# initc3/HoneyBadgerMPC

Measured on AMD Instinct MI355X. Metric: shares reconstructed/sec (batch open, n=64 t=21), higher is better.
Workload: dtype u256 (integer mod p): exact int8 x int8 -> int32 byte-split GEMM on the matrix cores; the high half of every sum folded mod p on the matrix cores too, one-word Barrett quotient

## Files before the change

honeybadgermpc_amd/csrc/gen_mm8.py:

```python
#!/usr/bin/env python3
import os

NC = 47
MAXKB = 4
XB = 180
ABUF = [[196, 200], [204, 208]]
F_SETS = [212, 234]
F_KMIN = -2
CLOBBER_LO, CLOBBER_HI = 180, 255
HALF_RHOS = [(0, 1), (2, 3)]


def f(s, k, e):
    assert -2 <= k <= 8 and e in (0, 1)
    return F_SETS[s] + 2 * (k - F_KMIN) + e


def windows(rho):
    return [q for q in range(-2, 8) if -7 <= 4 * q + rho <= 31]


def cols_of(rho):
    return sorted({4 * q + rho + 7 + 8 * g for q in windows(rho) for g in (0, 1)})


def half_columns(half):
    return sorted(c for rho in HALF_RHOS[half] for c in cols_of(rho))


NCP = 39


def packed_columns(half):
    return sorted(4 * q + rho + 7 for rho in HALF_RHOS[half] for q in windows(rho))


def lds_loads(kb, xs_op, as_op, packed=False):
    a0, a1 = ABUF[kb & 1]
    out = []
    for e in (0, 1):
        for h in (0, 1):
            out.append(f"ds_read_b128 v[{XB + 8 * e + 4 * h}:{XB + 8 * e + 4 * h + 3}], {xs_op} offset:{((kb * 2 + e) * 2 + h) * 1024}")
    out.append(f"ds_read_b128 v[{a0}:{a0 + 3}], {as_op} offset:{(kb * 2) * 1024}")
    if not packed:
        out.append(f"ds_read_b128 v[{a1}:{a1 + 3}], {as_op} offset:{(kb * 2 + 1) * 1024}")
    return out


def interleave(mfmas, ops):
    out = []
    if not mfmas:
        return list(ops)
    n = len(mfmas)
    per = (len(ops) + max(n - 1, 1) - 1) // max(n - 1, 1)
    pi = 0
    for i, m in enumerate(mfmas):
        if i == n - 1:
            out += ops[pi:]
            pi = len(ops)
        out.append(m)
        if i < n - 1:
            out += ops[pi:pi + per]
            pi += per
    return out


def asm_half(half, nkb, skip=False, packed=False):
    assert not skip or nkb >= 2
    assert not (skip and packed)
    cols = packed_columns(half) if packed else half_columns(half)
    pos = {c: i for i, c in enumerate(cols)}
    ncol = len(cols)
    xs_op, as_op, bias = f"%{ncol}", f"%{ncol + 1}", f"%{ncol + 2}"
    L = []
    for s in range(2):
        for k in (-2, 8):
            for e in (0, 1):
                L.append(f"v_mov_b32 v{f(s, k, e)}, 0")
    L += lds_loads(0, xs_op, as_op, packed)[:(5 if skip else 6)]
    groups = [(kb, rho) for kb in range(nkb) for rho in HALF_RHOS[half]]

    def prep(gi):
        kb, rho = groups[gi]
        s = gi & 1
        ops = []
        if rho == HALF_RHOS[half][0]:
            ops.append("s_waitcnt lgkmcnt(0)")
            for e in (0, 1):
                for k in range(8):
                    ops.append(f"v_xor_b32 v{f(s, k, e)}, 0x80808080, v{XB + 8 * e + k}")
                ops.append(f"v_mov_b32 v{f(s, -1, e)}, 0")
            if rho != 0:
                for e in (0, 1):
                    for k in range(-1, 8):
                        ops.append(f"v_alignbyte_b32 v{f(s, k, e)}, v{f(s, k + 1, e)}, v{f(s, k, e)}, {rho}")
        else:
            for e in (0, 1):
                for k in range(-1, 8):
                    ops.append(f"v_alignbyte_b32 v{f(s, k, e)}, v{f(1 - s, k + 1, e)}, v{f(1 - s, k, e)}, 1")
        return ops

    started = set()

    def mfmas(gi):
        kb, rho = groups[gi]
        s = gi & 1
        out = []
        for q in windows(rho):
            r = f(s, q, 0)
            assert r % 2 == 0
            for grp in ((0,) if packed else (0, 1)):
                if skip and kb == 0 and grp == 1:
                    continue
                c = 4 * q + rho + 7 + 8 * grp
                ab = ABUF[kb & 1][grp]
                cin = f"%{pos[c]}"
                if c not in started:
                    assert kb == 0 or (skip and kb == 1)
                    cin = bias
                    started.add(c)
                out.append(f"v_mfma_i32_16x16x64_i8 %{pos[c]}, v[{ab}:{ab + 3}], v[{r}:{r + 3}], {cin}")
        return out

    L += prep(0) + ["s_nop 1"]
    for gi in range(len(groups)):
        nxt = gi + 1 < len(groups)
        kb, rho = groups[gi]
        if rho == HALF_RHOS[half][0] and kb + 1 < nkb:
            L += lds_loads(kb + 1, xs_op, as_op, packed)
        L += interleave(mfmas(gi), prep(gi + 1) if nxt else [])
        if nxt:
            L.append("s_nop 0")
    assert started == set(cols)
    L += ["s_nop 7", "s_nop 7"]
    return L, ncol


def emit():
    out = ["// GENERATED by gen_mm8.py -- do not edit", ""]
    out.append("// column held by accumulator i of each half (half 0: rho in {0,1}; half 1: rho in {2,3})")
    for half in range(2):
        cols = half_columns(half)
        out.append(f"// half {half}: {cols}")
    assert half_columns(0) == [c for c in range(NC) if c % 4 in (0, 3)] and half_columns(1) == [c for c in range(NC) if c % 4 in (1, 2)]
    out.append("template <int NKB, int HALF, bool SKIP = false> struct Mm8Phase;")
    clob = ", ".join(f'"v{r}"' for r in range(CLOBBER_LO, CLOBBER_HI + 1))
    for nkb, skip in [(k, False) for k in range(1, MAXKB + 1)] + [(k, True) for k in range(2, MAXKB + 1)]:
        for half in range(2):
            lines, ncol = asm_half(half, nkb, skip)
            out.append(f"template <> struct Mm8Phase<{nkb}, {half}, {'true' if skip else 'false'}> {{")
            out.append("    static __device__ __forceinline__ void run(v4i (&acc)[24], uint32_t xs_addr, uint32_t as_addr, v4i biasv) {")
            out.append("        asm volatile(")
            for ln in lines:
                out.append(f'            "{ln}\\n\\t"')
            outs = ", ".join(f'"=&v"(acc[{i}])' for i in range(ncol))
            out.append(f"            : {outs}")
            out.append('            : "v"(xs_addr), "v"(as_addr), "v"(biasv)')
            out.append(f'            : {clob}, "memory");')
            out.append("    }")
            out.append("};")
    assert packed_columns(0) == [c for c in range(NCP) if c % 4 in (0, 3)] and packed_columns(1) == [c for c in range(NCP) if c % 4 in (1, 2)]
    out.append("// packed phases: accumulator i of a half is the virtual column (one per window) of the same two lists cut at 38")
    out.append("template <int NKB, int HALF> struct Mm8PhasePacked;")
    for nkb in range(1, MAXKB + 1):
        for half in range(2):
            lines, ncol = asm_half(half, nkb, packed=True)
            assert sum("v_mfma" in ln for ln in lines) == len(windows(HALF_RHOS[half][0]) + windows(HALF_RHOS[half][1])) * nkb
            out.append(f"template <> struct Mm8PhasePacked<{nkb}, {half}> {{")
            out.append("    static __device__ __forceinline__ void run(v4i (&acc)[20], uint32_t xs_addr, uint32_t as_addr, v4i biasv) {")
            out.append("        asm volatile(")
            for ln in lines:
                out.append(f'            "{ln}\\n\\t"')
            outs = ", ".join(f'"=&v"(acc[{i}])' for i in range(ncol))
            out.append(f"            : {outs}")
            out.append('            : "v"(xs_addr), "v"(as_addr), "v"(biasv)')
            out.append(f'            : {clob}, "memory");')
            out.append("    }")
            out.append("};")
    return "\n".join(out) + "\n"


if __name__ == "__main__":
    here = os.path.dirname(os.path.abspath(__file__))
    text = emit()
    path = os.path.join(here, "hb_mm8_body.inc")
    old = open(path).read() if os.path.exists(path) else None
    if old != text:
        open(path, "w").write(text)
    print(path)
```

honeybadgermpc_amd/csrc/hb_common.hpp:

```cpp
#pragma once
#include <hip/hip_runtime.h>
#include <stdint.h>
#include <stdio.h>
#include <string.h>

#include <functional>
#include <map>
#include <mutex>
#include <string>
#include <vector>

#include "../../include/hbmpc_hip.h"
#include "fp29.hpp"

namespace hb {
struct FastMatrix;
struct Mm8Matrix;
struct Mm8wMatrix;
}
namespace hb {

struct Wide { static constexpr int NL = 9, NW = 8; };
struct Narrow { static constexpr int NL = 3, NW = 2; };

constexpr int OT = 4;

template <int NL, int NW>
__device__ __forceinline__ void eval_at_point_128(uint32_t (&r)[NL], const uint32_t *__restrict__ x_packed, const uint32_t *__restrict__ poly, int d,
                                                  const FpParams<NL> &P, uint32_t (*red)[NL]) {
    const int tid = threadIdx.x;
    uint32_t xd[NL], xm[NL], acc[NL];
    load_digits<NL, NW>(xd, x_packed);
    to_mont(xm, xd, P);
#pragma unroll
    for (int q = 0; q < NL; q++) acc[q] = 0;
    for (int l = tid; l < d; l += 128) {
        uint32_t pw[NL], cd[NL], m[NL];
        fp_pow_u32(pw, xm, (uint32_t)l, P);
        load_digits<NL, NW>(cd, poly + (size_t)l * NW);
        mont_mul(m, cd, pw, P);
        fp_add(acc, acc, m, P);
    }
#pragma unroll
    for (int q = 0; q < NL; q++) red[tid][q] = acc[q];
    __syncthreads();
    for (int w = 64; w >= 1; w >>= 1) {
        if (tid < w) {
            uint32_t a[NL], b[NL], t[NL];
#pragma unroll
            for (int q = 0; q < NL; q++) { a[q] = red[tid][q]; b[q] = red[tid + w][q]; }
            fp_add(t, a, b, P);
#pragma unroll
            for (int q = 0; q < NL; q++) red[tid][q] = t[q];
        }
        __syncthreads();
    }
#pragma unroll
    for (int q = 0; q < NL; q++) r[q] = red[0][q];
}

__host__ __device__ inline size_t m_index(int i, int l, int n_in, int nl, int q) {
    return (((size_t)((i / OT) * n_in + l) * (size_t)nl + (size_t)q) * OT) + (size_t)(i % OT);
}
inline int m_tiles(int n_out) { return (n_out + OT - 1) / OT; }

}

struct hb_matrix {
    hb_ctx *ctx;
    int n_out, n_in;
    uint32_t *dev;
    size_t words;
    bool cached;
    int refs;
    hb::Mm8wMatrix *wide;
    bool wide_tried;
};

namespace hb {
struct TlsError {
    static std::string &slot() { static thread_local std::string s; return s; }
    TlsError &operator=(const std::string &m) { slot() = m; return *this; }
    TlsError &operator=(const char *m) { slot() = m ? m : ""; return *this; }
    const char *c_str() const { return slot().c_str(); }
    void clear() { slot().clear(); }
    bool empty() const { return slot().empty(); }
};
struct PrescaleParams {
    uint32_t pbar[9];
    uint32_t pneg[8];
    uint32_t m0, m1;
};
}
namespace hb {
enum EnvHook {
    ENV_CACHE_CAP,
    ENV_GAO_PAIR,
    ENV_MM8W_FLAT,
    ENV_MM8W_RQ,
    ENV_MM8W_TILE16,
    ENV_MM8_NO_SKIP,
    ENV_NO_EVAL_FEW,
    ENV_NO_FUSED_MSCALE,
    ENV_NO_FUSED_PACK,
    ENV_NO_FUSED_SMALL,
    ENV_NO_FUSED_VALIDATE,
    ENV_NO_MFMA,
    ENV_NO_MFMA_DECODE,
    ENV_NO_MFMA_WIDE,
    ENV_NO_NARROW_FAST,
    ENV_NO_QUICK,
    ENV_NO_QUICK_PLAN,
    ENV_NTT_STAGE_LOOP,
    ENV_PROBE_WGS,
    ENV_QUICK_NO_CAND,
    ENV_UPLOAD_MODE,
    ENV_WB_NO_GAO,
    ENV_WB_NO_UNIFORM,
    ENV_COUNT
};
const char *env_hook(EnvHook h);
void env_reload();
}
struct hb_ctx {
    int device;
    int n_limbs;
    hb::FpParams<9> pw;
    hb::FpParams<3> pn;
    uint64_t p_limbs[4];
    std::recursive_mutex mu;
    int api_depth = 0;
    hb::TlsError err;
    std::map<std::string, hb_matrix *> mcache;
    std::map<std::vector<int32_t>, int32_t *> icache;
    std::map<std::string, void *> dcache;
    std::map<std::string, hb::FastMatrix *> fcache;
    std::map<std::string, hb::Mm8Matrix *> m8cache;
    struct CacheSlot { uint64_t tick; bool pinned; std::function<void()> drop; };
    std::map<std::string, CacheSlot> lru;
    uint64_t lru_clock = 0;
    size_t cache_cap = 192;
    int32_t *flag_dev;
    hb::PrescaleParams psc;
    int psc_state = 0;
    std::map<std::string, void *> ptcache;
    struct QuickSlot { void *buf = nullptr; size_t cap = 0; void *ev = nullptr; };
    std::vector<QuickSlot> qslots;
    unsigned qnext = 0;
    std::vector<void *> probe_pool, probe_host_pool;
    void *side_stream = nullptr;
    std::map<std::string, std::pair<void *, size_t>> scratch;
    void *fetch_host = nullptr, *fetch_dev = nullptr;
    int fetch_seq = 0;
    void *cand_host = nullptr, *cand_dev = nullptr;
    int32_t *cand_ticket = nullptr;
    int cand_seq = 0;
    void *after_event = nullptr;
    std::map<int, void *> wide_shared;
    std::map<std::string, std::vector<int>> wide_shapes;
    void *mm8_shared = nullptr;
    int elem_words() const { return n_limbs == 4 ? 8 : 2; }
    int nl() const { return n_limbs == 4 ? 9 : 3; }
};

struct hb_api_guard {
    hb_ctx *c;
    explicit hb_api_guard(hb_ctx *ctx) : c(ctx) { if (c) { c->mu.lock(); c->api_depth++; } }
    ~hb_api_guard() { if (c) { c->api_depth--; c->mu.unlock(); } }
    hb_api_guard(const hb_api_guard &) = delete;
    hb_api_guard &operator=(const hb_api_guard &) = delete;
};
#define HB_API_GUARD(ctxexpr) hb_api_guard hb_api_guard__(ctxexpr)

inline int ctx_scratch(hb_ctx *ctx, const char *slot, size_t bytes, void **out) {
    auto &e = ctx->scratch[slot];
    if (e.second < bytes || !e.first) {
        if (e.first) { (void)hipFree(e.first); e.first = nullptr; e.second = 0; }
        const size_t want = bytes ? bytes : 4;
        const hipError_t err = hipMalloc(&e.first, want);
        if (err != hipSuccess) { e.first = nullptr; ctx->err = std::string("scratch ") + slot + ": " + hipGetErrorString(err); return HB_ERR_HIP; }
        e.second = want;
    }
    *out = e.first;
    return HB_OK;
}
inline void ctx_scratch_free(hb_ctx *ctx) {
    for (auto &kv : ctx->scratch) if (kv.second.first) (void)hipFree(kv.second.first);
    ctx->scratch.clear();
}

#define HB_HIP(ctx, call)                                                                         \
    do {                                                                                          \
        hipError_t e__ = (call);                                                                  \
        if (e__ != hipSuccess) {                                                                  \
            (ctx)->err = std::string(#call) + ": " + hipGetErrorString(e__);                      \
            return HB_ERR_HIP;                                                                    \
        }                                                                                         \
    } while (0)

#define HB_LAUNCH_CHECK(ctx)                                                                      \
    do {                                                                                          \
        hipError_t e__ = hipGetLastError();                                                       \
        if (e__ != hipSuccess) {                                                                  \
            (ctx)->err = std::string("kernel launch: ") + hipGetErrorString(e__);                 \
            return HB_ERR_HIP;                                                                    \
        }                                                                                         \
    } while (0)

namespace hb {

inline int fail(hb_ctx *ctx, int code, const char *msg) {
    if (ctx) ctx->err = msg;
    return code;
}
inline int nsub_for(int d, int nl, int nw) {
    int shift = 29 * nl - 32 * nw;
    long per = 1L << shift;
    long n = (d + per - 1) / per;
    return n < 1 ? 1 : (int)n;
}
void fp_params_from_limbs(FpParams<9> &P, const uint64_t *p_limbs);
void fp_params_from_limbs(FpParams<3> &P, const uint64_t *p_limbs);
int get_int_array(hb_ctx *ctx, const int32_t *host, int n, int32_t **dev, hipStream_t s);
int own_int_array(hb_ctx *ctx, const int32_t *host, int n, int32_t **dev, hipStream_t s);
void cache_note(hb_ctx *ctx, const std::string &rk, std::function<void()> drop, bool pinned = false);
void cache_touch(hb_ctx *ctx, const std::string &rk);
void cache_trim(hb_ctx *ctx);
void matrix_unref(hb_matrix *m);
int alloc_matrix(hb_ctx *ctx, int n_out, int n_in, hb_matrix **out);
int upload_elems(hb_ctx *ctx, const uint64_t *host, size_t count, uint32_t **dev, hipStream_t s);
int upload_table(hb_ctx *ctx, void *dst_dev, const void *src_host, size_t bytes, hipStream_t s);
std::string table_key(const char *kind, hb_ctx *ctx, const uint64_t *x, int n, int d);
int pow_points_dev(hb_ctx *ctx, const uint64_t *base_host, const int32_t *exps_dev, int count, uint32_t **out_dev, hipStream_t s);
int vand_matrix_from_dev(hb_ctx *ctx, const std::string &key, const uint32_t *x_dev, int n, int d, hb_matrix **out, hipStream_t s);
int vinv_from_dev(hb_ctx *ctx, const std::string &key, const uint32_t *x_dev, int k, hb_matrix **out, hipStream_t s);
int gao_decode(hb_ctx *ctx, const uint64_t *x_host, int npts, int k, const uint64_t *ys_dev, int64_t C,
               uint64_t *coeffs_dev, uint64_t *errloc_dev, int32_t *errloc_len_dev, uint8_t *ok_dev, void *stream, int ys_stride = 0, const int32_t *sel_host = nullptr);
int launch_matvec(hb_ctx *ctx, const hb_matrix *m, const uint32_t *in, hb_view iv, const int32_t *in_rows_dev, int64_t in_count,
                  uint32_t *out, hb_view ov, int64_t out_count, const int32_t *check_mask_dev, int32_t *mismatch_dev,
                  int64_t C, hipStream_t s);
int launch_copy_view(hb_ctx *ctx, const uint32_t *src, hb_view sv, uint32_t *dst, hb_view dv, int64_t C, int L, int64_t dst_count, hipStream_t s);

int get_twiddles(hb_ctx *ctx, const uint64_t *omega_host, int n, uint32_t **tw, hipStream_t s);
int launch_ntt_lds(hb_ctx *ctx, const uint32_t *tw, int n, const uint32_t *in, hb_view iv, int64_t in_count, int d, int k,
                   uint32_t *out, hb_view ov, int64_t out_count, const int32_t *check_mask_dev, int32_t *mismatch_dev,
                   int64_t C, hipStream_t s, uint32_t *copy_dst = nullptr, hb_view cpv = hb_view{0, 0}, int64_t copy_count = 0, int copy_rows = 0);

struct FastMatrix {
    int n_out, n_in;
    int ot;
    uint32_t *M;
    int32_t *nd;
    int32_t *negrow;
    uint32_t *K;
    uint32_t *K2;
    uint32_t *K1;
    uint32_t *KT;
};
__host__ __device__ inline size_t mf_index(int i, int l, int n_in, int nl, int q, int ot) {
    return (((size_t)((i / ot) * n_in + l) * (size_t)nl + (size_t)q) * ot) + (size_t)(i % ot);
}
void fast_matrix_free(FastMatrix *m);
int fast_vand_create(hb_ctx *ctx, const uint32_t *x_dev, int n, int d, FastMatrix **out, hipStream_t s);
int fast_vinv_create(hb_ctx *ctx, const uint32_t *x_dev, int k, FastMatrix **out, hipStream_t s);
int launch_prescale(hb_ctx *ctx, const FastMatrix *m, const uint32_t *in, hb_view iv, const int32_t *rows_dev, int64_t in_count,
                    uint32_t *out_dg, int64_t C, hipStream_t s);
int launch_prescale_pk(hb_ctx *ctx, const FastMatrix *m, const uint32_t *in, hb_view iv, const int32_t *rows_dev, int64_t in_count,
                       uint32_t *out_pk, int64_t C, hipStream_t s);
int launch_matvec2(hb_ctx *ctx, const FastMatrix *m, const uint32_t *in_dg,
                   const uint32_t *in_pk, hb_view iv, const int32_t *in_rows_dev, int64_t in_count, uint32_t *scratch_dg,
                   uint32_t *out_pk, hb_view ov, int64_t out_count,
                   int pk_rows, int pk_from_mont, uint32_t *out_dg, const int32_t *check_mask_dev, int32_t *mismatch_dev,
                   int64_t C, hipStream_t s, int check_skip = 0, const uint32_t *K_override = nullptr);

int launch_decode_check(hb_ctx *ctx, const FastMatrix *dec, const FastMatrix *enc, const uint32_t *cols, hb_view cv,
                        const int32_t *z_dev, uint32_t *pk_dst, hb_view pv, int64_t pk_count, int pk_rows, uint32_t *coef_dg,
                        const int32_t *mask_dev, int32_t *mismatch_dev, int64_t C, hipStream_t s, int check_skip);

bool prescale_params(hb_ctx *ctx);
int mm8_from_fast(hb_ctx *ctx, const FastMatrix *f, Mm8Matrix **out, hipStream_t s, const int32_t *rows = nullptr, int n_rows = 0);
void mm8_free(Mm8Matrix *m);
int launch_mm8(hb_ctx *ctx, const Mm8Matrix *m, const uint32_t *in, hb_view iv, const int32_t *in_rows_dev, int64_t in_count,
               uint32_t *out, hb_view ov, int64_t out_count, const int32_t *check_mask_dev, int32_t *mismatch_dev,
               int64_t C, hipStream_t s, uint32_t *copy_dst = nullptr, hb_view cpv = hb_view{0, 0}, int64_t copy_count = 0,
               int copy_rows = 0, const int32_t *check_rows_dev = nullptr);

int mm8w_from_host(hb_ctx *ctx, const uint64_t *m_host, int n_out, int n_in, Mm8wMatrix **out, hipStream_t s);
void mm8w_free(Mm8wMatrix *m);
int mm8w_route(hb_ctx *ctx, const Mm8wMatrix *m, int64_t C, int32_t *out);
int launch_mm8w(hb_ctx *ctx, const Mm8wMatrix *m, const uint32_t *in, hb_view iv, const int32_t *in_rows_dev, int64_t in_count,
                uint32_t *out, hb_view ov, int64_t out_count, const int32_t *check_mask_dev, int32_t *mismatch_dev,
                int64_t C, hipStream_t s, const uint32_t *cmp = nullptr, hb_view cv = hb_view{0, 0}, int n_store = 0);
bool fold_tables(hb_ctx *ctx, int n_bytes, uint8_t *fold, uint32_t *top8, uint32_t *mu, uint32_t *shift8);
struct FsVerdict { unsigned long long word; unsigned long long pad; };
struct FsDone { int32_t *counter; FsVerdict *host; int32_t seq; };
constexpr int32_t FS_VERDICT_NONE = 0x3fffffff;
#ifdef __HIPCC__
__device__ __forceinline__ void fs_publish_verdict(int32_t *mismatch, int32_t *first_bad, int32_t *counter, FsVerdict *host, int32_t seq) {
    const int32_t fl = mismatch ? __hip_atomic_load(mismatch, __ATOMIC_RELAXED, __HIP_MEMORY_SCOPE_AGENT) : 0;
    const int32_t fb = first_bad ? __hip_atomic_load(first_bad, __ATOMIC_RELAXED, __HIP_MEMORY_SCOPE_AGENT) : INT32_MAX;
    const uint32_t low = ((fl & 1) ? 0x80000000u : 0u) | ((fl & 0x40000000) ? 0x40000000u : 0u) | (uint32_t)((fb < 0 || fb > FS_VERDICT_NONE) ? FS_VERDICT_NONE : fb);
    __hip_atomic_store(&host->word, ((unsigned long long)(uint32_t)seq << 32) | low, __ATOMIC_RELAXED, __HIP_MEMORY_SCOPE_SYSTEM);
    if (mismatch) __hip_atomic_store(mismatch, 0, __ATOMIC_RELAXED, __HIP_MEMORY_SCOPE_AGENT);
    if (first_bad) __hip_atomic_store(first_bad, INT32_MAX, __ATOMIC_RELAXED, __HIP_MEMORY_SCOPE_AGENT);
    if (counter) __hip_atomic_store(counter, 0, __ATOMIC_RELAXED, __HIP_MEMORY_SCOPE_AGENT);
}
__device__ __forceinline__ void fs_workgroup_done(const FsDone &done, int32_t *mismatch, int32_t *first_bad) {
    if (!done.counter) return;
    asm volatile("s_waitcnt vmcnt(0)" ::: "memory");
    __syncthreads();
    if (threadIdx.x == 0 && atomicAdd(done.counter, 1) == (int)gridDim.x - 1) fs_publish_verdict(mismatch, first_bad, done.counter, done.host, done.seq);
}
#endif
inline bool fs_verdict_is(const FsVerdict *host, int32_t seq) { return (int32_t)(*reinterpret_cast<const volatile unsigned long long *>(&host->word) >> 32) == seq; }
inline void fs_verdict_read(const FsVerdict *host, int32_t *flag, int32_t *first) {
    const uint32_t low = (uint32_t)*reinterpret_cast<const volatile unsigned long long *>(&host->word);
    *flag = ((low >> 31) ? 1 : 0) | ((low & 0x40000000u) ? 0x40000000 : 0);
    const int32_t f = (int32_t)(low & 0x3fffffffu);
    *first = f == FS_VERDICT_NONE ? INT32_MAX : f;
}
struct Mm8wShared { uint32_t bias; uint32_t c80r[9], biasmod[9]; void *wp; uint32_t *zero; };
int mm8w_geometry(int n_out, int d, int *tile_rows, int *n_rt, int *nkb, size_t *a8_bytes, size_t *crow_words);
int mm8w_shared(hb_ctx *ctx, int d, const Mm8wShared **out, hipStream_t s);
void mm8w_shared_free(hb_ctx *ctx);
int launch_mm8w_raw(hb_ctx *ctx, int n_out, int d, int tile_rows, const void *a8, const uint32_t *crow, const Mm8wShared *sh,
                    const uint32_t *in, hb_view iv, const int32_t *in_rows_dev, int64_t in_count, uint32_t *out, hb_view ov, int64_t out_count,
                    const int32_t *check_mask_dev, int32_t *mismatch_dev, int64_t C, hipStream_t s, const uint32_t *cmp, hb_view cv, int n_store,
                    int32_t *first_bad_dev, uint32_t *bad_map_dev = nullptr, const FsDone *done = nullptr);
void point_tables_free(hb_ctx *ctx);
void mm8_shared_free(hb_ctx *ctx);
struct PointTable {
    int n, S;
    uint32_t *xm, *inv, *pw;
    bool usable;
    int refs;
    bool small;
    std::vector<uint16_t> xs;
    uint16_t *xs_dev;
};
int point_table(hb_ctx *ctx, const uint64_t *x_host, int n, PointTable **out, hipStream_t s);
struct QuickLayout {
    int n, d, nc, n_coef, n_out, tile_rows, nkb;
    size_t o_a8, o_crow, o_wj, o_full, o_nraw, o_mcan, o_z, o_map, o_sync, need;
    size_t o_cand, o_cand_crow;
};
int quick_layout(hb_ctx *ctx, int n, int d, int nc, int n_coef, QuickLayout *L);
int quick_build(hb_ctx *ctx, const uint64_t *x_host, const int32_t *z, const int32_t *zc, const QuickLayout &L, uint8_t *base, const Mm8wShared **shared, hipStream_t s,
                int flags = 3 );
int quick_layout_cand(hb_ctx *ctx, QuickLayout *L);
int quick_launch(hb_ctx *ctx, const QuickLayout &L, const uint8_t *base, const Mm8wShared *sh, const uint32_t *cols, hb_view cv, uint32_t *out, hb_view ov,
                 int64_t out_count, int n_store, int32_t *mismatch_dev, int32_t *first_bad_dev, int64_t C, hipStream_t s, uint32_t *bad_map_dev = nullptr,
                 const FsDone *done = nullptr);
struct FsLayout {
    int n, d, nc, n_coef, n_out, n_rt, nkb;
    size_t o_a8, o_crow, o_kt, o_mode, o_z, o_cand, o_cand_crow, need;
    int pk_nm, pk_ns;
    uint8_t pk_single[8];
    size_t o_ms;
    int mscale;
};
constexpr int FS_BUILD_Z = 1, FS_BUILD_ZC = 2;
int fs_layout(hb_ctx *ctx, const PointTable *pt, int d, int nc, int n_coef, FsLayout *L);
int fs_build(hb_ctx *ctx, const PointTable *pt, const int32_t *z, const int32_t *zc, const FsLayout &L, uint8_t *base, int flags, int32_t *status_dev, hipStream_t s);
bool fs_pack(const PointTable *pt, const int32_t *z, FsLayout *L);
bool fs_mscale(FsLayout *L);
int fs_launch(hb_ctx *ctx, const FsLayout &L, const uint8_t *base, const uint32_t *cols, hb_view cv, uint32_t *out, hb_view ov, int64_t out_count,
              int32_t *mismatch_dev, int32_t *first_bad_dev, uint32_t *bad_map_dev, int64_t C, hipStream_t s, const FsDone *done = nullptr,
              const int32_t *pick_zc = nullptr);
int fs_build_cand(hb_ctx *ctx, PointTable *pt, const int32_t *z, const FsLayout &L, uint8_t *base, int32_t *status_dev, hipStream_t s, bool with_z = false);
struct Mv64Matrix;
int points_on_device(hb_ctx *ctx, const uint64_t *x_host, int n, uint32_t **out, hipStream_t s);
bool mv64_applies(const hb_ctx *ctx, int d);
bool mv64_matrix_cores(const hb_ctx *ctx, int d);
int mv64_from_host(hb_ctx *ctx, const uint64_t *m_host, int n_out, int d, const int32_t *mode_host, Mv64Matrix **out, hipStream_t s);
void mv64_free(Mv64Matrix *m);
int launch_mv64(hb_ctx *ctx, const Mv64Matrix *m, const uint64_t *in, hb_view iv, const int32_t *in_rows_dev, int64_t in_count, uint64_t *out, hb_view ov,
                int64_t out_count, int32_t *mismatch_dev, int32_t *first_bad_dev, int64_t C, hipStream_t s);
int mv64_plan_tables(hb_ctx *ctx, const uint64_t *x, int n, int d, const int32_t *z, const int32_t *zc, int nc, std::vector<uint64_t> &V, std::vector<uint64_t> &Vinv,
                     std::vector<uint64_t> &P);
int quick_dec_supported(hb_quick_dec *qd, int d, int nc, int n_coef);
const Mm8wMatrix *matrix_wide(hb_ctx *ctx, const hb_matrix *m, hipStream_t s);

#define HB_DISPATCH(ctx, EXPR_W, EXPR_N)                                                          \
    do {                                                                                          \
        if ((ctx)->n_limbs == 4) { EXPR_W; } else { EXPR_N; }                                     \
    } while (0)

}
```

honeybadgermpc_amd/csrc/hb_core.hip:

```cpp
#include <algorithm>

#include <mutex>
#include <string>

#include "hb_common.hpp"

using namespace hb;

namespace {

struct U320 { uint64_t l[5]; };
inline bool ge(const U320 &a, const U320 &b) {
    for (int i = 4; i >= 0; i--) if (a.l[i] != b.l[i]) return a.l[i] > b.l[i];
    return true;
}
inline void sub(U320 &a, const U320 &b) {
    unsigned __int128 br = 0;
    for (int i = 0; i < 5; i++) {
        unsigned __int128 d = (unsigned __int128)a.l[i] - b.l[i] - (uint64_t)br;
        a.l[i] = (uint64_t)d; br = (d >> 64) & 1;
    }
}
inline void dbl_mod(U320 &a, const U320 &p) {
    for (int i = 4; i > 0; i--) a.l[i] = (a.l[i] << 1) | (a.l[i - 1] >> 63);
// ... 122 lines not shown
    uint32_t d[NL], m[NL];
    load_digits<NL, NW>(d, src + (size_t)idx * NW);
    to_mont(m, d, P);
#pragma unroll
    for (int q = 0; q < NL; q++) M[m_index(i, l, n_in, NL, q)] = m[q];
}
template <int NL, int NW>
__global__ void k_matrix_export(const FpParams<NL> P, const uint32_t *__restrict__ M, int n_out, int n_in, uint32_t *__restrict__ dst) {
    int idx = blockIdx.x * blockDim.x + threadIdx.x;
    if (idx >= n_out * n_in) return;
    int i = idx / n_in, l = idx % n_in;
    uint32_t m[NL], d[NL];
#pragma unroll
    for (int q = 0; q < NL; q++) m[q] = M[m_index(i, l, n_in, NL, q)];
    from_mont(d, m, P);
    store_digits<NL, NW>(dst + (size_t)idx * NW, d);
}

template <int NL, int NW, bool CHECK>
__global__ void __launch_bounds__(256) k_matvec(const FpParams<NL> P, const uint32_t *__restrict__ M, int n_out, int n_in, int nsub,
                                                const uint32_t *__restrict__ in, int64_t in_sc, int64_t in_sl,
                                                const int32_t *__restrict__ in_rows, int64_t in_count,
                                                uint32_t *__restrict__ out, int64_t out_sc, int64_t out_sl, int64_t out_count,
                                                const int32_t *__restrict__ check_mask, int32_t *__restrict__ mismatch,
                                                int64_t C, int tiles, int64_t n_waves) {
    static_assert(OT == 4, "matrix tile is loaded as uint4 per digit");
    const int lane = threadIdx.x & 63;
    const int wib = __builtin_amdgcn_readfirstlane(threadIdx.x >> 6);
    const int64_t nb8 = gridDim.x >> 3;
    const int64_t vb = (int64_t)(blockIdx.x & 7) * nb8 + (blockIdx.x >> 3);
    const int64_t wave = vb * 4 + wib;
    if (wave >= n_waves) return;
    const int tile = (int)(wave % tiles);
    const int64_t g = wave / tiles;
    const int64_t c = g * 64 + lane;
    const bool active = c < C;
    const int64_t cc = active ? c : (C - 1);
    const int nv = min(OT, n_out - tile * OT);
    const uint4 *mt = reinterpret_cast<const uint4 *>(M) + (size_t)tile * n_in * NL;
    constexpr int GROUP = Lazy<NL>::GROUP;

    uint64_t col[OT][2 * NL];
#pragma unroll
    for (int o = 0; o < OT; o++) col_zero(col[o]);

#define HB_ROW_OF(l_) (in_rows ? in_rows[((l_) < n_in) ? (l_) : (n_in - 1)] : (((l_) < n_in) ? (l_) : (n_in - 1)))
#define HB_LOAD_M(dst_, l_)                                                              \
    _Pragma("unroll") for (int q = 0; q < NL; q++) dst_[q] = mt[(size_t)(l_) * NL + q];
#define HB_LOAD_X(w_, valid_, row_)                                                      \
    {                                                                                    \
        const int64_t idx_ = cc * in_sc + (int64_t)(row_) * in_sl;                       \
        valid_ = idx_ < in_count;                                                        \
        load_words<NW>(w_, in + (valid_ ? idx_ : 0) * NW);                               \
    }
#define HB_UNPACK_X(d_, w_, valid_)                                                      \
    {                                                                                    \
        unpack<NL, NW>(d_, w_);                                                          \
        _Pragma("unroll") for (int q = 0; q < NL; q++) d_[q] = valid_ ? d_[q] : 0u;      \
    }
    uint4 mc[NL], mn[NL];
    uint32_t wn[NW], xd[NL];
    bool vn;
    HB_LOAD_M(mc, 0)
    HB_LOAD_X(wn, vn, HB_ROW_OF(0))
    HB_UNPACK_X(xd, wn, vn)
    int row_n = HB_ROW_OF(1);
    int gcnt = 0;
    for (int l = 0; l < n_in; l++) {
        const int ln = (l + 1 < n_in) ? l + 1 : l;
        HB_LOAD_M(mn, ln)
        const int row_nn = HB_ROW_OF(l + 2);
        HB_LOAD_X(wn, vn, row_n)
        __builtin_amdgcn_sched_barrier(0);
        uint32_t xu[NL];
#pragma unroll
        for (int q = 0; q < NL; q++) { xu[q] = xd[q]; asm volatile("" : "+v"(xu[q])); }
#pragma unroll
        for (int o = 0; o < OT; o++) {
            if (o < nv) {
                uint32_t md[NL];
#pragma unroll
                for (int q = 0; q < NL; q++) md[q] = (o == 0) ? mc[q].x : (o == 1) ? mc[q].y : (o == 2) ? mc[q].z : mc[q].w;
                mac<NL>(col[o], md, xu);
            }
        }
        if (++gcnt == GROUP) {
            gcnt = 0;
#pragma unroll
            for (int o = 0; o < OT; o++) carry(col[o]);
        }
        __builtin_amdgcn_sched_barrier(0);
        HB_UNPACK_X(xd, wn, vn)
        row_n = row_nn;
#pragma unroll
        for (int q = 0; q < NL; q++) mc[q] = mn[q];
    }
#undef HB_ROW_OF
#undef HB_LOAD_M
#undef HB_LOAD_X
#undef HB_UNPACK_X
#pragma unroll
    for (int o = 0; o < OT; o++) {
        if (o < nv) {
            const int i = tile * OT + o;
            uint32_t r[NL];
            carry(col[o]);
            redc(r, col[o], P);
            for (int s = 0; s < nsub; s++) cond_sub_p(r, P);
            uint32_t w[NW];
            pack<NL, NW>(w, r);
            const int64_t oidx = cc * out_sc + (int64_t)i * out_sl;
            if constexpr (CHECK) {
                if (check_mask[i] && active) {
                    uint32_t e[NW];
                    load_words<NW>(e, out + oidx * NW);
                    uint32_t diff = 0;
#pragma unroll
                    for (int q = 0; q < NW; q++) diff |= e[q] ^ w[q];
                    if (diff) atomicOr(mismatch, 1);
                }
            } else {
                if (active && oidx < out_count) store_words<NW>(out + oidx * NW, w);
            }
        }
    }
}

template <int NW>
__global__ void k_copy_view(const uint32_t *__restrict__ src, int64_t s_sc, int64_t s_sl, uint32_t *__restrict__ dst, int64_t d_sc, int64_t d_sl,
                            int64_t C, int L, int64_t dst_count) {
    int64_t idx = (int64_t)blockIdx.x * blockDim.x + threadIdx.x;
    if (idx >= C * L) return;
    int64_t c = idx / L; int l = (int)(idx % L);
    int64_t di = c * d_sc + (int64_t)l * d_sl;
    if (di >= dst_count) return;
    uint32_t w[NW];
    load_words<NW>(w, src + (c * s_sc + (int64_t)l * s_sl) * NW);
    store_words<NW>(dst + di * NW, w);
}

template <int NL, int NW>
__global__ void k_reduce(const FpParams<NL> P, const uint32_t *__restrict__ src, uint32_t *__restrict__ dst, int64_t count,
                         int32_t *__restrict__ changed) {
    const int64_t i = (int64_t)blockIdx.x * blockDim.x + threadIdx.x;
    if (i >= count) return;
    uint32_t w[NW], d[NL], m[NL], o[NW];
    load_words<NW>(w, src + i * NW);
    unpack<NL, NW>(d, w);
    to_mont<NL>(m, d, P);
    from_mont<NL>(d, m, P);
    pack<NL, NW>(o, d);
    bool diff = false;
#pragma unroll
    for (int q = 0; q < NW; q++) diff |= o[q] != w[q];
    if (diff) {
        store_words<NW>(dst + i * NW, o);
        if (changed) atomicAdd(changed, 1);
    } else if (dst != src) {
        store_words<NW>(dst + i * NW, w);
    }
}

namespace hb {

void cache_note(hb_ctx *ctx, const std::string &rk, std::function<void()> drop, bool pinned) {
    ctx->lru[rk] = hb_ctx::CacheSlot{++ctx->lru_clock, pinned, std::move(drop)};
}
void cache_touch(hb_ctx *ctx, const std::string &rk) {
    auto it = ctx->lru.find(rk);
    if (it != ctx->lru.end()) it->second.tick = ++ctx->lru_clock;
}
static void cache_drop_down_to(hb_ctx *ctx, size_t keep) {
    std::vector<std::pair<uint64_t, std::string>> order;
    for (auto &kv : ctx->lru) if (!kv.second.pinned) order.emplace_back(kv.second.tick, kv.first);
    if (order.size() <= keep) return;
    std::sort(order.begin(), order.end());
    (void)hipDeviceSynchronize();
    for (size_t i = 0; i + keep < order.size(); i++) {
        auto it = ctx->lru.find(order[i].second);
        if (it == ctx->lru.end()) continue;
        auto drop = std::move(it->second.drop);
        ctx->lru.erase(it);
        drop();
    }
}
void cache_trim(hb_ctx *ctx) {
    if (ctx->api_depth > 1) return;
    size_t unpinned = 0;
    for (auto &kv : ctx->lru) if (!kv.second.pinned) unpinned++;
    if (unpinned > ctx->cache_cap) cache_drop_down_to(ctx, ctx->cache_cap / 2);
}
void matrix_unref(hb_matrix *m) {
    if (!m) return;
    if (--m->refs > 0) return;
    (void)hipFree(m->dev);
    mm8w_free(m->wide);
    delete m;
}

static std::string int_key(const int32_t *host, int n) {
    return std::string("i|") + std::string(reinterpret_cast<const char *>(host), (size_t)(n > 0 ? n : 0) * 4);
}
int own_int_array(hb_ctx *ctx, const int32_t *host, int n, int32_t **dev, hipStream_t s) {
    int32_t *d = nullptr;
    HB_HIP(ctx, hipMalloc(&d, sizeof(int32_t) * (size_t)(n > 0 ? n : 1)));
    const int rc = upload_table(ctx, d, host, sizeof(int32_t) * (size_t)(n > 0 ? n : 0), s);
    if (rc) { (void)hipFree(d); return rc; }
    *dev = d;
    return HB_OK;
}
int get_int_array(hb_ctx *ctx, const int32_t *host, int n, int32_t **dev, hipStream_t s) {
    std::vector<int32_t> key(host, host + n);
    const std::string rk = int_key(host, n);
    auto it = ctx->icache.find(key);
    if (it != ctx->icache.end()) { cache_touch(ctx, rk); *dev = it->second; return HB_OK; }
    int32_t *d = nullptr;
    int rc = own_int_array(ctx, host, n, &d, s); if (rc) return rc;
    ctx->icache[key] = d;
    cache_note(ctx, rk, [ctx, key]() { auto f = ctx->icache.find(key); if (f != ctx->icache.end()) { (void)hipFree(f->second); ctx->icache.erase(f); } });
    *dev = d;
    return HB_OK;
}

int alloc_matrix(hb_ctx *ctx, int n_out, int n_in, hb_matrix **out) {
    hb_matrix *m = new hb_matrix();
    m->ctx = ctx; m->n_out = n_out; m->n_in = n_in; m->cached = false; m->refs = 1; m->wide = nullptr; m->wide_tried = false;
    m->words = (size_t)m_tiles(n_out) * (size_t)n_in * OT * (size_t)ctx->nl();
    if (m->words == 0) m->words = 1;
    hipError_t e = hipMalloc(&m->dev, m->words * sizeof(uint32_t));
    if (e != hipSuccess) { delete m; ctx->err = std::string("hipMalloc: ") + hipGetErrorString(e); return HB_ERR_HIP; }
    *out = m;
    return HB_OK;
}

__global__ void k_upload_copy(const uint4 *__restrict__ src, uint4 *__restrict__ dst, size_t n16) {
    const size_t i = (size_t)blockIdx.x * blockDim.x + threadIdx.x;
    if (i < n16) dst[i] = src[i];
}
int upload_table(hb_ctx *ctx, void *dst_dev, const void *src_host, size_t bytes, hipStream_t s) {
    if (bytes == 0) return HB_OK;
    static const int legacy = [] { const char *e = env_hook(ENV_UPLOAD_MODE); return e && !strcmp(e, "memcpy") ? 1 : 0; }();
    if (legacy) {
        hipError_t e = hipMemcpyAsync(dst_dev, src_host, bytes, hipMemcpyHostToDevice, s);
        if (e == hipSuccess) e = hipStreamSynchronize(s);
        if (e != hipSuccess) { ctx->err = std::string("table upload: ") + hipGetErrorString(e); return HB_ERR_HIP; }
        return HB_OK;
    }
    const size_t n16 = (bytes + 15) / 16;
    void *stage = nullptr;
    HB_HIP(ctx, hipMalloc(&stage, n16 * 16));
    hipError_t e = hipMemcpy(stage, src_host, bytes, hipMemcpyHostToDevice);
    if (e == hipSuccess) {
        if (bytes % 16 == 0) k_upload_copy<<<(unsigned)((n16 + 255) / 256), 256, 0, s>>>((const uint4 *)stage, (uint4 *)dst_dev, n16);
        else e = hipMemcpyAsync(dst_dev, stage, bytes, hipMemcpyDeviceToDevice, s);
    }
    if (e == hipSuccess) e = hipGetLastError();
    if (e == hipSuccess) e = hipStreamSynchronize(s);
    (void)hipFree(stage);
    if (e != hipSuccess) { ctx->err = std::string("table upload: ") + hipGetErrorString(e); return HB_ERR_HIP; }
    return HB_OK;
}

int upload_elems(hb_ctx *ctx, const uint64_t *host, size_t count, uint32_t **dev, hipStream_t s) {
    size_t bytes = count * (size_t)ctx->elem_words() * 4;
    HB_HIP(ctx, hipMalloc(dev, bytes ? bytes : 4));
    const int rc = upload_table(ctx, *dev, host, bytes, s);
    if (rc) { (void)hipFree(*dev); *dev = nullptr; }
    return rc;
}

int points_on_device(hb_ctx *ctx, const uint64_t *x_host, int n, uint32_t **out, hipStream_t s) {
    std::string key = table_key("xs", ctx, x_host, n, 0);
    auto it = ctx->dcache.find(key);
    if (it != ctx->dcache.end()) { *out = (uint32_t *)it->second; cache_touch(ctx, "d|" + key); return HB_OK; }
    uint32_t *xd = nullptr;
    const int rc = upload_elems(ctx, x_host, (size_t)n, &xd, s); if (rc) return rc;
    ctx->dcache[key] = xd;
    cache_note(ctx, "d|" + key, [ctx, key]() { auto f = ctx->dcache.find(key); if (f != ctx->dcache.end()) { (void)hipFree(f->second); ctx->dcache.erase(f); } });
    *out = xd;
    return HB_OK;
}

std::string table_key(const char *kind, hb_ctx *ctx, const uint64_t *x, int n, int d) {
    std::string k(kind);
    k += ":" + std::to_string(n) + ":" + std::to_string(d) + ":";
    k.append(reinterpret_cast<const char *>(x), (size_t)n * ctx->n_limbs * 8);
    return k;
}

}

template <int NL, int NW>
__global__ void __launch_bounds__(128) k_eval_few(const FpParams<NL> P, const uint32_t *__restrict__ x, int n, const uint32_t *__restrict__ polys, int d,
                                                  uint32_t *__restrict__ out) {
    __shared__ uint32_t red[128][NL];
    const int c = blockIdx.x / n, i = blockIdx.x - c * n;
    uint32_t r[NL];
    eval_at_point_128<NL, NW>(r, x + (size_t)i * NW, polys + (size_t)c * d * NW, d, P, red);
    if (threadIdx.x == 0) store_digits<NL, NW>(out + ((size_t)c * n + i) * NW, r);
}


namespace hb {
static const char *const ENV_NAMES[ENV_COUNT] = {"HB_CACHE_CAP", "HB_GAO_PAIR", "HB_MM8W_FLAT", "HB_MM8W_RQ", "HB_MM8W_TILE16", "HB_MM8_NO_SKIP", "HB_NO_EVAL_FEW", "HB_NO_FUSED_MSCALE", "HB_NO_FUSED_PACK", "HB_NO_FUSED_SMALL", "HB_NO_FUSED_VALIDATE", "HB_NO_MFMA", "HB_NO_MFMA_DECODE", "HB_NO_MFMA_WIDE", "HB_NO_NARROW_FAST", "HB_NO_QUICK", "HB_NO_QUICK_PLAN", "HB_NTT_STAGE_LOOP", "HB_PROBE_WGS", "HB_QUICK_NO_CAND", "HB_UPLOAD_MODE", "HB_WB_NO_GAO", "HB_WB_NO_UNIFORM"};
static std::string g_env_val[ENV_COUNT];
static bool g_env_set[ENV_COUNT];
static std::once_flag g_env_once;
static std::mutex g_env_mu;
static void env_read() {
    for (int i = 0; i < ENV_COUNT; i++) {
        const char *e = ::getenv(ENV_NAMES[i]);
        g_env_set[i] = e != nullptr;
        g_env_val[i] = e ? e : "";
    }
}
const char *env_hook(EnvHook h) {
    std::call_once(g_env_once, env_read);
    return g_env_set[h] ? g_env_val[h].c_str() : nullptr;
}
void env_reload() {
    std::call_once(g_env_once, env_read);
    std::lock_guard<std::mutex> lk(g_env_mu);
    env_read();
}
}
extern "C" void hb_debug_reload_env() { hb::env_reload(); }

extern "C" {

int hb_version(void) { return 100; }

int hb_device_count(void) {
    int n = 0;
    if (hipGetDeviceCount(&n) != hipSuccess) return 0;
    return n;
}

int hb_ctx_create(hb_ctx **out, const uint64_t *p_limbs, int n_limbs, int device) {
    if (!out || !p_limbs) return HB_ERR_BAD_ARG;
    *out = nullptr;
    if (n_limbs != 1 && n_limbs != 4) return HB_ERR_BAD_ARG;
    if ((p_limbs[0] & 1) == 0) return HB_ERR_UNSUPPORTED;
    bool small = true; for (int i = 1; i < n_limbs; i++) if (p_limbs[i]) small = false;
    if (small && p_limbs[0] < 3) return HB_ERR_UNSUPPORTED;
    int ndev = 0;
    if (hipGetDeviceCount(&ndev) != hipSuccess || ndev == 0) return HB_ERR_NO_DEVICE;
    if (device < 0 || device >= ndev) return HB_ERR_NO_DEVICE;
    if (hipSetDevice(device) != hipSuccess) return HB_ERR_NO_DEVICE;
    hb_ctx *ctx = new hb_ctx();
    ctx->device = device; ctx->n_limbs = n_limbs;
    memset(ctx->p_limbs, 0, sizeof ctx->p_limbs);
    memcpy(ctx->p_limbs, p_limbs, (size_t)n_limbs * 8);
    if (n_limbs == 4) make_params<9>(ctx->pw, p_limbs, 4); else make_params<3>(ctx->pn, p_limbs, 1);
    if (const char *e = env_hook(ENV_CACHE_CAP)) { long v = atol(e); if (v >= 1) ctx->cache_cap = (size_t)v; }
    ctx->flag_dev = nullptr;
    if (hipMalloc(&ctx->flag_dev, 64 * sizeof(int32_t)) != hipSuccess) { delete ctx; return HB_ERR_HIP; }
    (void)hipMemset(ctx->flag_dev, 0, 64 * sizeof(int32_t));
    *out = ctx;
    return HB_OK;
}

void hb_ctx_destroy(hb_ctx *ctx) {
    if (!ctx) return;
    (void)hipSetDevice(ctx->device);
    ctx->lru.clear();
    for (auto &kv : ctx->mcache) matrix_unref(kv.second);
    for (auto &kv : ctx->icache) (void)hipFree(kv.second);
    for (auto &kv : ctx->dcache) (void)hipFree(kv.second);
    for (auto &kv : ctx->fcache) fast_matrix_free(kv.second);
    for (auto &kv : ctx->m8cache) mm8_free(kv.second);
    if (ctx->flag_dev) (void)hipFree(ctx->flag_dev);
    if (ctx->side_stream) (void)hipStreamDestroy((hipStream_t)ctx->side_stream);
    point_tables_free(ctx);
    mm8w_shared_free(ctx);
    mm8_shared_free(ctx);
    ctx_scratch_free(ctx);
    delete ctx;
}

const char *hb_last_error(const hb_ctx *ctx) { return ctx ? ctx->err.c_str() : "no context"; }
int hb_elem_bytes(const hb_ctx *ctx) { return ctx ? ctx->n_limbs * 8 : 0; }

int hb_malloc(hb_ctx *ctx, void **dptr, size_t bytes) { HB_API_GUARD(ctx); HB_HIP(ctx, hipMalloc(dptr, bytes ? bytes : 4)); return HB_OK; }
int hb_free(hb_ctx *ctx, void *dptr) { HB_API_GUARD(ctx); HB_HIP(ctx, hipFree(dptr)); return HB_OK; }
int hb_memcpy_h2d(hb_ctx *ctx, void *dst, const void *src, size_t bytes, void *stream) { HB_API_GUARD(ctx);
    HB_HIP(ctx, hipMemcpyAsync(dst, src, bytes, hipMemcpyHostToDevice, (hipStream_t)stream)); return HB_OK;
}
int hb_memcpy_d2h(hb_ctx *ctx, void *dst, const void *src, size_t bytes, void *stream) { HB_API_GUARD(ctx);
    HB_HIP(ctx, hipMemcpyAsync(dst, src, bytes, hipMemcpyDeviceToHost, (hipStream_t)stream));
    HB_HIP(ctx, hipStreamSynchronize((hipStream_t)stream)); return HB_OK;
}
int hb_stream_sync(hb_ctx *ctx, void *stream) { HB_API_GUARD(ctx); HB_HIP(ctx, hipStreamSynchronize((hipStream_t)stream)); return HB_OK; }

}

namespace hb {

template <int NL, int NW>
__global__ void k_pow_points(const FpParams<NL> P, const uint32_t *__restrict__ base, const int32_t *__restrict__ exps, int count,
                             uint32_t *__restrict__ out) {
    int i = blockIdx.x * blockDim.x + threadIdx.x;
    if (i >= count) return;
    uint32_t bd[NL], bm[NL], r[NL], c[NL];
    load_digits<NL, NW>(bd, base);
    to_mont(bm, bd, P);
    fp_pow_u32(r, bm, (uint32_t)(exps ? exps[i] : i), P);
    from_mont(c, r, P);
    store_digits<NL, NW>(out + (size_t)i * NW, c);
}

int pow_points_dev(hb_ctx *ctx, const uint64_t *base_host, const int32_t *exps_dev, int count, uint32_t **out_dev, hipStream_t s) {
    uint32_t *bd = nullptr;
    int rc = upload_elems(ctx, base_host, 1, &bd, s); if (rc) return rc;
    HB_HIP(ctx, hipMalloc(out_dev, (size_t)(count > 0 ? count : 1) * ctx->elem_words() * 4));
    if (count > 0) {
        HB_DISPATCH(ctx,
            (k_pow_points<9, 8><<<(count + 63) / 64, 64, 0, s>>>(ctx->pw, bd, exps_dev, count, *out_dev)),
            (k_pow_points<3, 2><<<(count + 63) / 64, 64, 0, s>>>(ctx->pn, bd, exps_dev, count, *out_dev)));
        HB_LAUNCH_CHECK(ctx);
    }
    HB_HIP(ctx, hipStreamSynchronize(s));
    HB_HIP(ctx, hipFree(bd));
    return HB_OK;
}

int vand_matrix_from_dev(hb_ctx *ctx, const std::string &key, const uint32_t *x_dev, int n, int d, hb_matrix **out, hipStream_t s) {
    hb_matrix *m = nullptr;
    int rc = alloc_matrix(ctx, n, d, &m); if (rc) return rc;
    HB_HIP(ctx, hipMemsetAsync(m->dev, 0, m->words * 4, s));
    if (n > 0 && d > 0) {
        HB_DISPATCH(ctx,
            (k_vand_table<9, 8><<<(n + 63) / 64, 64, 0, s>>>(ctx->pw, x_dev, n, d, m->dev)),
            (k_vand_table<3, 2><<<(n + 63) / 64, 64, 0, s>>>(ctx->pn, x_dev, n, d, m->dev)));
        HB_LAUNCH_CHECK(ctx);
        HB_HIP(ctx, hipStreamSynchronize(s));
    }
    m->cached = true; ctx->mcache[key] = m; *out = m;
    cache_note(ctx, "m|" + key, [ctx, key]() { auto f = ctx->mcache.find(key); if (f != ctx->mcache.end()) { hb_matrix *mm = f->second; ctx->mcache.erase(f); matrix_unref(mm); } });
    return HB_OK;
}

int vinv_from_dev(hb_ctx *ctx, const std::string &key, const uint32_t *x_dev, int k, hb_matrix **out, hipStream_t s) {
    if (k > 1023) return fail(ctx, HB_ERR_UNSUPPORTED, "vandermonde inverse: k > 1023");
    hb_matrix *m = nullptr;
    int rc = alloc_matrix(ctx, k, k, &m); if (rc) return rc;
    HB_HIP(ctx, hipMemsetAsync(m->dev, 0, m->words * 4, s));
    int singular = 0;
    if (k > 0) {
        HB_HIP(ctx, hipMemsetAsync(ctx->flag_dev, 0, sizeof(int32_t), s));
        int threads = ((k + 1 + 63) / 64) * 64;
        size_t lds = (size_t)(k + 2 * (k + 1)) * ctx->nl() * 4;
        if (ctx->n_limbs == 4) {
            HB_HIP(ctx, hipFuncSetAttribute(reinterpret_cast<const void *>(k_vinv_table<9, 8>), hipFuncAttributeMaxDynamicSharedMemorySize, (int)lds));
            k_vinv_table<9, 8><<<1, threads, lds, s>>>(ctx->pw, x_dev, k, m->dev, ctx->flag_dev);
        } else {
            HB_HIP(ctx, hipFuncSetAttribute(reinterpret_cast<const void *>(k_vinv_table<3, 2>), hipFuncAttributeMaxDynamicSharedMemorySize, (int)lds));
            k_vinv_table<3, 2><<<1, threads, lds, s>>>(ctx->pn, x_dev, k, m->dev, ctx->flag_dev);
        }
        HB_LAUNCH_CHECK(ctx);
        HB_HIP(ctx, hipMemcpyAsync(&singular, ctx->flag_dev, sizeof(int), hipMemcpyDeviceToHost, s));
        HB_HIP(ctx, hipStreamSynchronize(s));
    }
    if (singular) { m->refs = 1; matrix_unref(m); return fail(ctx, HB_ERR_SINGULAR, "Interpolation failed"); }
    m->cached = true; ctx->mcache[key] = m; *out = m;
    cache_note(ctx, "m|" + key, [ctx, key]() { auto f = ctx->mcache.find(key); if (f != ctx->mcache.end()) { hb_matrix *mm = f->second; ctx->mcache.erase(f); matrix_unref(mm); } });
    return HB_OK;
}

}

extern "C" {

int hb_vand_matrix_create(hb_ctx *ctx, const uint64_t *x_host, int n, int d, hb_matrix **out, void *stream) { HB_API_GUARD(ctx);
    if (!ctx || !out || n < 0 || d < 0) return HB_ERR_BAD_ARG;
    hipStream_t s = (hipStream_t)stream;
    cache_trim(ctx);
    std::string key = table_key("V", ctx, x_host, n, d);
    auto it = ctx->mcache.find(key);
    if (it != ctx->mcache.end()) { cache_touch(ctx, "m|" + key); it->second->refs++; *out = it->second; return HB_OK; }
    uint32_t *xd = nullptr;
    int rc = upload_elems(ctx, x_host, (size_t)n, &xd, s); if (rc) return rc;
    rc = vand_matrix_from_dev(ctx, key, xd, n, d, out, s);
    (void)hipStreamSynchronize(s);
    (void)hipFree(xd);
    if (!rc) (*out)->refs++;
    return rc;
}

int hb_vand_inverse_create(hb_ctx *ctx, const uint64_t *x_host, int k, hb_matrix **out, void *stream) { HB_API_GUARD(ctx);
    if (!ctx || !out || k < 0) return HB_ERR_BAD_ARG;
    hipStream_t s = (hipStream_t)stream;
    cache_trim(ctx);
    std::string key = table_key("Vinv", ctx, x_host, k, k);
    auto it = ctx->mcache.find(key);
    if (it != ctx->mcache.end()) { cache_touch(ctx, "m|" + key); it->second->refs++; *out = it->second; return HB_OK; }
    uint32_t *xd = nullptr;
    int rc = upload_elems(ctx, x_host, (size_t)k, &xd, s); if (rc) return rc;
    rc = vinv_from_dev(ctx, key, xd, k, out, s);
    (void)hipStreamSynchronize(s);
    (void)hipFree(xd);
    if (!rc) (*out)->refs++;
    return rc;
}

int hb_matrix_from_host(hb_ctx *ctx, const uint64_t *m_host, int n_out, int n_in, hb_matrix **out, void *stream) { HB_API_GUARD(ctx);
    if (!ctx || !out || n_out < 0 || n_in < 0) return HB_ERR_BAD_ARG;
    hipStream_t s = (hipStream_t)stream;
    hb_matrix *m = nullptr;
    int rc = alloc_matrix(ctx, n_out, n_in, &m); if (rc) return rc;
    HB_HIP(ctx, hipMemsetAsync(m->dev, 0, m->words * 4, s));
    if (n_out * n_in > 0) {
        uint32_t *src = nullptr;
        rc = upload_elems(ctx, m_host, (size_t)n_out * n_in, &src, s); if (rc) return rc;
        int tot = n_out * n_in;
        HB_DISPATCH(ctx,
            (k_matrix_import<9, 8><<<(tot + 127) / 128, 128, 0, s>>>(ctx->pw, src, n_out, n_in, m->dev)),
            (k_matrix_import<3, 2><<<(tot + 127) / 128, 128, 0, s>>>(ctx->pn, src, n_out, n_in, m->dev)));
        HB_LAUNCH_CHECK(ctx);
        HB_HIP(ctx, hipStreamSynchronize(s));
        HB_HIP(ctx, hipFree(src));
    }
    *out = m;
    return HB_OK;
}

int hb_matrix_to_host(hb_ctx *ctx, const hb_matrix *m, uint64_t *m_host, void *stream) { HB_API_GUARD(ctx);
    if (!ctx || !m || !m_host) return HB_ERR_BAD_ARG;
    hipStream_t s = (hipStream_t)stream;
    int tot = m->n_out * m->n_in;
    if (tot == 0) return HB_OK;
    uint32_t *dst = nullptr;
    size_t bytes = (size_t)tot * ctx->elem_words() * 4;
    HB_HIP(ctx, hipMalloc(&dst, bytes));
    HB_DISPATCH(ctx,
        (k_matrix_export<9, 8><<<(tot + 127) / 128, 128, 0, s>>>(ctx->pw, m->dev, m->n_out, m->n_in, dst)),
        (k_matrix_export<3, 2><<<(tot + 127) / 128, 128, 0, s>>>(ctx->pn, m->dev, m->n_out, m->n_in, dst)));
    HB_LAUNCH_CHECK(ctx);
    HB_HIP(ctx, hipMemcpyAsync(m_host, dst, bytes, hipMemcpyDeviceToHost, s));
    HB_HIP(ctx, hipStreamSynchronize(s));
    HB_HIP(ctx, hipFree(dst));
    return HB_OK;
}

void hb_matrix_destroy(hb_matrix *m) { HB_API_GUARD((m ? m->ctx : nullptr)); matrix_unref(m); }

}

namespace hb {

static const Mm8wMatrix *matvec_wide(hb_ctx *ctx, const hb_matrix *m, int64_t C, hipStream_t s) {
    return C >= 256 && m->n_in >= 4 && m->n_out >= 4 ? matrix_wide(ctx, m, s) : nullptr;
}

int launch_matvec(hb_ctx *ctx, const hb_matrix *m, const uint32_t *in, hb_view iv, const int32_t *in_rows_dev, int64_t in_count,
                  uint32_t *out, hb_view ov, int64_t out_count, const int32_t *check_mask_dev, int32_t *mismatch_dev,
                  int64_t C, hipStream_t s) {
    if (C <= 0 || m->n_out == 0) return HB_OK;
    if (const Mm8wMatrix *w = matvec_wide(ctx, m, C, s)) return launch_mm8w(ctx, w, in, iv, in_rows_dev, in_count, out, ov, out_count, check_mask_dev, mismatch_dev, C, s);
    const int tiles = m_tiles(m->n_out);
    const int64_t groups = (C + 63) / 64;
    const int64_t n_waves = groups * tiles;
    int64_t blocks = (n_waves + 3) / 4;
    blocks = ((blocks + 7) / 8) * 8;
    if (blocks > 0x7fffffffLL) return fail(ctx, HB_ERR_UNSUPPORTED, "matvec: batch too large for one launch");
    const int nsub = nsub_for(m->n_in, ctx->nl(), ctx->elem_words());
    if (nsub > 64) return fail(ctx, HB_ERR_UNSUPPORTED, "matvec: inner dimension too large");
    const bool check = check_mask_dev != nullptr;
    if (ctx->n_limbs == 4) {
        if (check) k_matvec<9, 8, true><<<(unsigned)blocks, 256, 0, s>>>(ctx->pw, m->dev, m->n_out, m->n_in, nsub, in, iv.stride_c, iv.stride_l, in_rows_dev, in_count, out, ov.stride_c, ov.stride_l, out_count, check_mask_dev, mismatch_dev, C, tiles, n_waves);
        else k_matvec<9, 8, false><<<(unsigned)blocks, 256, 0, s>>>(ctx->pw, m->dev, m->n_out, m->n_in, nsub, in, iv.stride_c, iv.stride_l, in_rows_dev, in_count, out, ov.stride_c, ov.stride_l, out_count, nullptr, nullptr, C, tiles, n_waves);
    } else {
        if (check) k_matvec<3, 2, true><<<(unsigned)blocks, 256, 0, s>>>(ctx->pn, m->dev, m->n_out, m->n_in, nsub, in, iv.stride_c, iv.stride_l, in_rows_dev, in_count, out, ov.stride_c, ov.stride_l, out_count, check_mask_dev, mismatch_dev, C, tiles, n_waves);
        else k_matvec<3, 2, false><<<(unsigned)blocks, 256, 0, s>>>(ctx->pn, m->dev, m->n_out, m->n_in, nsub, in, iv.stride_c, iv.stride_l, in_rows_dev, in_count, out, ov.stride_c, ov.stride_l, out_count, nullptr, nullptr, C, tiles, n_waves);
    }
    HB_LAUNCH_CHECK(ctx);
    return HB_OK;
}

const Mm8wMatrix *matrix_wide(hb_ctx *ctx, const hb_matrix *cm, hipStream_t s) {
    hb_matrix *m = const_cast<hb_matrix *>(cm);
    if (m->wide_tried) return m->wide;
    m->wide_tried = true;
    if (ctx->n_limbs != 4 || env_hook(ENV_NO_MFMA) || env_hook(ENV_NO_MFMA_WIDE)) return nullptr;
    std::vector<uint64_t> host((size_t)m->n_out * m->n_in * 4);
    if (hb_matrix_to_host(ctx, m, host.data(), (void *)s) != HB_OK) return nullptr;
    Mm8wMatrix *w = nullptr;
    if (mm8w_from_host(ctx, host.data(), m->n_out, m->n_in, &w, s) != HB_OK) return nullptr;
    m->wide = w;
    return w;
}

int launch_copy_view(hb_ctx *ctx, const uint32_t *src, hb_view sv, uint32_t *dst, hb_view dv, int64_t C, int L, int64_t dst_count, hipStream_t s) {
    int64_t tot = C * L;
    if (tot <= 0) return HB_OK;
    int64_t blocks = (tot + 255) / 256;
    if (ctx->n_limbs == 4) k_copy_view<8><<<(unsigned)blocks, 256, 0, s>>>(src, sv.stride_c, sv.stride_l, dst, dv.stride_c, dv.stride_l, C, L, dst_count);
    else k_copy_view<2><<<(unsigned)blocks, 256, 0, s>>>(src, sv.stride_c, sv.stride_l, dst, dv.stride_c, dv.stride_l, C, L, dst_count);
    HB_LAUNCH_CHECK(ctx);
    return HB_OK;
}

}

extern "C" int hb_debug_matvec_route(hb_ctx *ctx, const hb_matrix *m, int64_t C, int32_t *out) { HB_API_GUARD(ctx);
    if (!ctx || !m || !out) return HB_ERR_BAD_ARG;
    for (int j = 0; j < 8; j++) out[j] = 0;
    if (C <= 0 || m->n_out == 0) return HB_OK;
// ... 219 lines not shown
```

honeybadgermpc_amd/csrc/hb_mfma.hip:

```cpp
#include <atomic>

#include "hb_mm8.hpp"

namespace hb {

#include "hb_mm8_body.inc"

#ifdef HB_MM8_TIMING
__device__ unsigned long long g_mm8_t[2048 * 8];
#define MM8_T(k) do { const unsigned long long tn_ = __builtin_amdgcn_s_memtime(); tacc[k] += tn_ - tlast; tlast = tn_; } while (0)
#else
#define MM8_T(k) do { } while (0)
#endif
template <int NKB, bool CHECK, bool RAGGED, bool SKIP>
__global__ __launch_bounds__(256, 2) void k_mm8(const int4 *__restrict__ a8, const uint32_t *__restrict__ crowd,
                                                const uint32_t *__restrict__ zero_src,
                                                const uint32_t *__restrict__ in_pk, int64_t in_sc, int64_t in_sl,
                                                const int32_t *__restrict__ in_rows, int64_t in_count, int d,
                                                uint32_t *__restrict__ out_pk, int64_t out_sc, int64_t out_sl, int64_t out_count,
                                                const int32_t *__restrict__ check_mask, const int32_t *__restrict__ check_rows, int32_t *__restrict__ mismatch,
                                                uint32_t *__restrict__ copy_dst, int64_t copy_sc, int64_t copy_sl, int64_t copy_count, int copy_rows,
                                                int n_out, int n_rt, int tpw, int64_t n_chunks, int64_t n_units, BarrettParams bp) {
    extern __shared__ uint4 mm8_lds[];
    const int lane = threadIdx.x & 63, wave = __builtin_amdgcn_readfirstlane(threadIdx.x >> 6);
    const int n = lane & 15, g = lane >> 4;
    uint32_t *crl = reinterpret_cast<uint32_t *>(mm8_lds);
    int4 *abuf = reinterpret_cast<int4 *>(mm8_lds + n_rt * 64);
    uint4 *xbuf = mm8_lds + n_rt * 64 + n_rt * NKB * 2 * 64;
    const int bufsz = tpw * NKB * 4 * 64;

    const int n_pairs = tpw * n_rt;

    int32_t *rowl = reinterpret_cast<int32_t *>(xbuf + 2 * bufsz);
    uint32_t *rowoff = reinterpret_cast<uint32_t *>(rowl + 32);
    v4i *foldl = reinterpret_cast<v4i *>(rowl + 96 + 16 * n_rt);
    if (threadIdx.x < 32) {
        const int lc = (int)threadIdx.x < d ? (int)threadIdx.x : d - 1;
        const int row = in_rows ? in_rows[lc] : lc;
        rowl[threadIdx.x] = row;
        rowoff[threadIdx.x] = (uint32_t)((int64_t)row * in_sl * 32);
        int m = row;
        for (int o = 16; o > 0; o >>= 1) m = max(m, __shfl_xor(m, o, 32));
        if (threadIdx.x == 0) rowl[64] = m;
    }
    int32_t *maskl = rowl + 96;
    if constexpr (CHECK) {
        for (int i = threadIdx.x; i < n_rt * 16; i += 256) maskl[i] = (i < n_out && check_mask[i]) ? (check_rows ? check_rows[i] + 1 : i + 1) : 0;
    }
    __syncthreads();
    const int rowmax = __builtin_amdgcn_readfirstlane(rowl[64]);
    const bool fast_dma = in_sc >= 0 && in_sl >= 0 && in_count < (1ll << 27);
    const uint32_t lane_off = (uint32_t)((int64_t)n * in_sc * 32);
    const int n_slots = tpw * NKB * 4;
    auto issue_loads = [&](int64_t unit, int buf) {
        const int64_t c_last = (unit * tpw + tpw) * 16 - 1;
        if (fast_dma && c_last < n_chunks && c_last * in_sc + (int64_t)rowmax * in_sl < in_count) {
            for (int s = wave; s < n_slots; s += 4) {
                const int h = s & 1, e = (s >> 1) & 1, q = s >> 2, t = q / NKB, kb = q - t * NKB;
                const uint64_t sbase = (uint64_t)(uintptr_t)in_pk + (uint64_t)((unit * tpw + t) * 16 * in_sc) * 32 + h * 16;
                const uint32_t voff = lane_off + rowoff[8 * kb + 2 * g + e];
                const uint32_t lds_dst = __builtin_amdgcn_readfirstlane(
                    (uint32_t)(uintptr_t)(__attribute__((address_space(3))) void *)(xbuf + (size_t)buf * bufsz + s * 64));
                uint32_t keep;
                asm volatile("s_mov_b32 %0, m0\n\ts_mov_b32 m0, %3\n\ts_nop 0\n\tglobal_load_lds_dwordx4 %1, %2\n\ts_mov_b32 m0, %0"
                             : "=&s"(keep) : "v"(voff), "s"(sbase), "s"(lds_dst) : "memory");
            }
            return;
        }
        for (int s = wave; s < n_slots; s += 4) {
            const int h = s & 1, e = (s >> 1) & 1, q = s >> 2, t = q / NKB, kb = q - t * NKB;
            int64_t chunk = (unit * tpw + t) * 16 + n;
            if (chunk >= n_chunks) chunk = n_chunks - 1;
            const int64_t idx = chunk * in_sc + (int64_t)rowl[8 * kb + 2 * g + e] * in_sl;
            const uint4 *src = (idx < in_count) ? reinterpret_cast<const uint4 *>(in_pk) + idx * 2 + h
                                                : reinterpret_cast<const uint4 *>(zero_src) + h;
            const uint32_t lds_dst = __builtin_amdgcn_readfirstlane(
                (uint32_t)(uintptr_t)(__attribute__((address_space(3))) void *)(xbuf + (size_t)buf * bufsz + s * 64));
            uint32_t keep;
            asm volatile("s_mov_b32 %0, m0\n\ts_mov_b32 m0, %2\n\ts_nop 0\n\tglobal_load_lds_dwordx4 %1, off\n\ts_mov_b32 m0, %0"
                         : "=&s"(keep) : "v"(src), "s"(lds_dst) : "memory");
        }
    };
    const v4i biasv = v4i{MM8_BIAS, MM8_BIAS, MM8_BIAS, MM8_BIAS};
    uint32_t k256 = 256u, k16m = 1u << 24;
    int32_t s1 = 1, s256 = 256, s64k = 1 << 16, s16m = 1 << 24;
    uint32_t u1 = 1u;
    asm volatile("" : "+s"(k256), "+s"(k16m), "+s"(s1), "+s"(s256), "+s"(s64k), "+s"(s16m), "+s"(u1));

    int buf = 0;
    int64_t unit = blockIdx.x;
#ifdef HB_MM8_TIMING
    unsigned long long tacc[8] = {0, 0, 0, 0, 0, 0, 0, 0}, tlast = __builtin_amdgcn_s_memtime();
#endif
    if (unit < n_units) issue_loads(unit, 0);
    {
        const int n_cr = n_rt, n_blk = n_rt * (1 + 2 * NKB);
        for (int blk = wave; blk < n_blk; blk += 4) {
            const uint4 *src = (blk < n_cr ? reinterpret_cast<const uint4 *>(crowd) + blk * 64
                                           : reinterpret_cast<const uint4 *>(a8) + (blk - n_cr) * 64) + lane;
            const uint32_t lds_dst = __builtin_amdgcn_readfirstlane((uint32_t)(uintptr_t)(__attribute__((address_space(3))) void *)(mm8_lds + blk * 64));
            uint32_t keep;
            asm volatile("s_mov_b32 %0, m0\n\ts_mov_b32 m0, %2\n\ts_nop 0\n\tglobal_load_lds_dwordx4 %1, off\n\ts_mov_b32 m0, %0"
                         : "=&s"(keep) : "v"(src), "s"(lds_dst) : "memory");
        }
    }
    if (threadIdx.x < MM8_FOLD_Q) foldl[threadIdx.x] = reinterpret_cast<const v4i *>(crowd + (size_t)n_rt * 256)[threadIdx.x];
    asm volatile("s_waitcnt vmcnt(0) lgkmcnt(0)" ::: "memory");
    const v4i *fold_lane = reinterpret_cast<const v4i *>(reinterpret_cast<const char *>(foldl) + (g == (n >> 2) ? 16 * n : 256));
    MM8_T(0);
    for (; unit < n_units; unit += gridDim.x, buf ^= 1) {
        __builtin_amdgcn_s_barrier();
        MM8_T(1);
        if (unit + gridDim.x < n_units) issue_loads(unit + gridDim.x, buf ^ 1);
        MM8_T(2);
        if constexpr (CHECK) {
            if (copy_dst) {
                for (int e = wave; e < tpw * NKB * 2; e += 4) {
                    const int t = e / (NKB * 2), kb = (e >> 1) - t * NKB, l = 8 * kb + 2 * g + (e & 1);
                    const int64_t ch = (unit * tpw + t) * 16 + n;
                    const int64_t idx = ch * copy_sc + (int64_t)l * copy_sl;
                    if (l < copy_rows && l < d && ch < n_chunks && idx < copy_count) {
                        const uint4 *src = xbuf + (size_t)buf * bufsz + (size_t)e * 2 * 64 + lane;
                        uint4 *dst = reinterpret_cast<uint4 *>(copy_dst) + idx * 2;
                        dst[0] = src[0];
                        dst[1] = src[64];
                    }
                }
            }
        }
        if (wave >= n_pairs) asm volatile("s_waitcnt vmcnt(0)" ::: "memory");
        for (int pidx = wave; pidx < n_pairs; pidx += 4) {
            const int tl = pidx / n_rt, rt = pidx - tl * n_rt;
            const int64_t chunk = (unit * tpw + tl) * 16 + n;
            const uint4 *xs = xbuf + (size_t)buf * bufsz + (size_t)tl * NKB * 4 * 64 + lane;
            const int4 *as = abuf + (size_t)rt * NKB * 2 * 64 + lane;
            uint32_t eap[4][11], c0p[4];
            const int64_t obase = chunk * out_sc + (int64_t)(16 * rt + g) * out_sl, ostep = 4 * out_sl;
            const bool pair1 = !RAGGED || 16 * rt + 8 < n_out;
            const uint32_t xs_addr = (uint32_t)(uintptr_t)(__attribute__((address_space(3))) const void *)xs;
            const uint32_t as_addr = (uint32_t)(uintptr_t)(__attribute__((address_space(3))) const void *)as;
            {
                v4i acc[24];
                asm volatile("" ::: "memory");
                __builtin_amdgcn_sched_barrier(0);
                __builtin_amdgcn_s_setprio(0);
                Mm8Phase<NKB, 0, SKIP>::run(acc, xs_addr, as_addr, biasv);
                __builtin_amdgcn_s_setprio(2);
                __builtin_amdgcn_sched_barrier(0);
                MM8_T(3);
#pragma unroll
                for (int reg = 0; reg < 4; reg++) {
                    if (reg == 2 && !pair1) break;
                    c0p[reg] = (uint32_t)acc[0][reg];
#pragma unroll
                    for (int j = 0; j < 11; j++) eap[reg][j] = (uint32_t)acc[1 + 2 * j][reg] + ((uint32_t)acc[2 + 2 * j][reg] << 8);
                    asm volatile("" ::"v"(c0p[reg]), "v"(eap[reg][0]), "v"(eap[reg][1]), "v"(eap[reg][2]), "v"(eap[reg][3]), "v"(eap[reg][4]),
                                 "v"(eap[reg][5]), "v"(eap[reg][6]), "v"(eap[reg][7]), "v"(eap[reg][8]), "v"(eap[reg][9]), "v"(eap[reg][10]));
                    __builtin_amdgcn_sched_barrier(0);
                }
            }
            {
                v4i acc[24];
                asm volatile("" ::: "memory");
                __builtin_amdgcn_sched_barrier(0);
                MM8_T(4);
                __builtin_amdgcn_s_setprio(0);
                Mm8Phase<NKB, 1, SKIP>::run(acc, xs_addr, as_addr, biasv);
                __builtin_amdgcn_s_setprio(2);
                __builtin_amdgcn_sched_barrier(0);
                MM8_T(5);
                if (pidx + 4 >= n_pairs) asm volatile("s_waitcnt vmcnt(0)" ::: "memory");
                MM8_T(6);
#pragma unroll
                for (int reg = 0; reg < 4; reg++) {
                    if (reg == 2 && !pair1) break;
                    const int i = 16 * rt + 4 * reg + g;
                    uint32_t ew[8];
                    bool cmp = false;
                    if constexpr (CHECK) {
                        const int erow = maskl[i];
                        cmp = (chunk < n_chunks) && erow;
                        load_words<8>(ew, out_pk + (cmp ? (chunk * out_sc + (int64_t)(erow - 1) * out_sl) * 8 : 0));
                    }
                    (void)ew; (void)cmp;
                    uint64_t pw[8];
                    {
                        const uint4 *cr = reinterpret_cast<const uint4 *>(crl + (size_t)i * 16);
#pragma unroll
                        for (int k = 0; k < 4; k++) {
                            const uint4 c = cr[k];
                            pw[2 * k] = (uint64_t)c.x | ((uint64_t)c.y << 32);
                            pw[2 * k + 1] = (uint64_t)c.z | ((uint64_t)c.w << 32);
                        }
                    }
                    uint32_t glo[5], ghi[5];
#pragma unroll
                    for (int k = 0; k < 12; k++) {
                        const uint32_t f = (uint32_t)acc[2 * k][reg] + ((uint32_t)acc[2 * k + 1][reg] << 8);
                        uint64_t gk = (uint64_t)f * k256 + (k < 7 ? pw[k] : 0ull);
                        if (k < 11) gk += (uint64_t)eap[reg][k] * k16m;
                        if (k < 7) pw[k] = gk;
                        else { glo[k - 7] = (uint32_t)gk; ghi[k - 7] = (uint32_t)(gk >> 32); }
                    }
                    pw[0] += (uint64_t)c0p[reg] * u1;
                    pw[7] += (uint64_t)glo[0] * u1;
                    uint32_t hw[5];
                    {
                        unsigned cyw = 0;
#pragma unroll
                        for (int k = 0; k < 4; k++) hw[k] = __builtin_addc(glo[k + 1], ghi[k], cyw, &cyw);
                        hw[4] = ghi[4] + cyw;
                    }
                    v4i hb;
#pragma unroll
                    for (int k = 0; k < 4; k++) hb[k] = (int)(hw[k] ^ 0x80808080u);
                    v4i dcol[8];
#pragma unroll
                    for (int eb = 0; eb < 8; eb++)
                        dcol[eb] = __builtin_amdgcn_mfma_i32_16x16x64_i8(fold_lane[eb * (MM8_FOLD_ROW / 16)], hb, v4i{0, 0, 0, 0}, 0, 0, 0);
#pragma unroll
                    for (int k = 0; k < 8; k++) pw[k] += (uint64_t)hw[4] * bp.c384[k];
#pragma unroll
                    for (int k = 0; k < 8; k++) {
                        int64_t t = (int64_t)pw[k] + (int64_t)dcol[k][0] * s1;
                        t += (int64_t)dcol[k][1] * s256;
                        t += (int64_t)dcol[k][2] * s64k;
                        t += (int64_t)dcol[k][3] * s16m;
                        pw[k] = (uint64_t)t;
                    }
                    const uint64_t tq = pw[7] + (pw[6] >> 32);
                    const uint32_t qh = (uint32_t)(((uint64_t)(uint32_t)(tq >> 16) * bp.mu) >> 46);
#pragma unroll
                    for (int k = 0; k < 8; k++) pw[k] += (uint64_t)qh * bp.pneg[k];
                    uint32_t ow[8];
                    uint32_t top;
                    {
                        unsigned cy = 0;
                        ow[0] = (uint32_t)pw[0];
#pragma unroll
                        for (int k = 1; k < 8; k++) ow[k] = __builtin_addc((uint32_t)pw[k], (uint32_t)(pw[k - 1] >> 32), cy, &cy);
                        top = (uint32_t)(pw[7] >> 32) + cy - qh;
                    }
                    if (__builtin_amdgcn_ballot_w64(top != 0 || ow[7] >= ~bp.pneg[7]) != 0) {
                        uint32_t u[8];
                        unsigned cy2 = 0;
#pragma unroll
                        for (int k = 0; k < 8; k++) u[k] = __builtin_addc(ow[k], bp.pneg[k], cy2, &cy2);
                        const bool take = cy2 || top;
#pragma unroll
                        for (int k = 0; k < 8; k++) ow[k] = take ? u[k] : ow[k];
                    }
                    const int64_t oidx = obase + reg * ostep;
                    if constexpr (CHECK) {
                        uint32_t diff = 0;
#pragma unroll
                        for (int k = 0; k < 8; k++) diff |= ew[k] ^ ow[k];
                        asm volatile("" : "+v"(diff));
                        if (__builtin_amdgcn_ballot_w64(cmp && diff) != 0 && lane == 0 && *reinterpret_cast<volatile int32_t *>(mismatch) == 0) atomicOr(mismatch, 1);
                    } else {
                        asm volatile("" ::"v"(ow[0]), "v"(ow[1]), "v"(ow[2]), "v"(ow[3]), "v"(ow[4]), "v"(ow[5]), "v"(ow[6]), "v"(ow[7]));
                        if (chunk < n_chunks && i < n_out && oidx < out_count) {
                            bool stream_out = false;
                            if constexpr (SKIP && !RAGGED) stream_out = out_sc == 1;
                            if (stream_out) store_words_nt<8>(out_pk + oidx * 8, ow);
                            else store_words<8>(out_pk + oidx * 8, ow);
                        }
                    }
                    if (reg & 1) __builtin_amdgcn_sched_barrier(0);
                }
            }
            MM8_T(7);
        }
    }
#ifdef HB_MM8_TIMING
    if (lane == 0 && blockIdx.x < 512) for (int k = 0; k < 8; k++) g_mm8_t[(blockIdx.x * 4 + wave) * 8 + k] = tacc[k];
#endif
}

int64_t mm8_trimmed_grid(int64_t n_units, int64_t blocks) {
    if (blocks < 1 || n_units < 1) return blocks;
    const int64_t rounds = (n_units + blocks - 1) / blocks;
    return (n_units + rounds - 1) / rounds;
}

}

using namespace hb;

namespace {

constexpr size_t MM8_LDS_LIMIT = 78 * 1024;
size_t mm8_lds_bytes(int n_rt, int nkb, int tpw);
int mm8_tpw(int n_rt, int nkb) {
    int tpw = (n_rt == 1) ? 4 : (n_rt == 2) ? 2 : 1;
    return tpw;
}
size_t mm8_lds_bytes(int n_rt, int nkb, int tpw) {
    return ((size_t)n_rt * 64 + (size_t)n_rt * nkb * 2 * 64 + (size_t)2 * tpw * nkb * 4 * 64 + MM8_FOLD_Q) * 16 + 96 * 4 + (size_t)n_rt * 16 * 4;
}

int mm8_num_cus() {
    static int n = 0;
    if (!n) {
        int dev = 0;
        (void)hipGetDevice(&dev);
        if (hipDeviceGetAttribute(&n, hipDeviceAttributeMultiprocessorCount, dev) != hipSuccess || n <= 0) n = 256;
    }
    return n;
}

typedef std::vector<uint32_t> Big;
Big big_mul(const Big &a, const Big &b) {
    Big r(a.size() + b.size(), 0);
    for (size_t i = 0; i < a.size(); i++) {
        uint64_t cy = 0;
        for (size_t j = 0; j < b.size(); j++) {
            uint64_t t = (uint64_t)a[i] * b[j] + r[i + j] + cy;
            r[i + j] = (uint32_t)t; cy = t >> 32;
        }
        r[i + b.size()] = (uint32_t)cy;
    }
    return r;
}
bool big_ge(const Big &a, const Big &b) {
    for (size_t i = a.size(); i-- > 0;) if (a[i] != b[i]) return a[i] > b[i];
    return true;
}
void big_sub(Big &a, const Big &b) {
    int64_t br = 0;
    for (size_t i = 0; i < a.size(); i++) {
        int64_t t = (int64_t)a[i] - (i < b.size() ? b[i] : 0) + br;
        a[i] = (uint32_t)t; br = t >> 32;
    }
}
void big_add(Big &a, const Big &b) {
    uint64_t cy = 0;
    for (size_t i = 0; i < a.size(); i++) {
        uint64_t t = (uint64_t)a[i] + (i < b.size() ? b[i] : 0) + cy;
        a[i] = (uint32_t)t; cy = t >> 32;
    }
}
Big big_divmod(const Big &x, const Big &p, Big *q) {
    Big r(p.size() + 1, 0), pp(p); pp.push_back(0);
    if (q) q->assign(x.size(), 0);
    for (int bit = (int)x.size() * 32 - 1; bit >= 0; bit--) {
        uint32_t in = (x[bit >> 5] >> (bit & 31)) & 1u;
        for (size_t i = r.size(); i-- > 0;) r[i] = (r[i] << 1) | (i ? r[i - 1] >> 31 : in);
        if (big_ge(r, pp)) { big_sub(r, pp); if (q) (*q)[bit >> 5] |= 1u << (bit & 31); }
    }
    r.pop_back();
    return r;
}
Big big_shl(const Big &a, int bits, size_t words) {
    Big r(words, 0);
    for (size_t i = 0; i < a.size(); i++) {
        const size_t w = i + bits / 32; const int s = bits % 32;
        if (w < words) r[w] |= a[i] << s;
        if (s && w + 1 < words) r[w + 1] |= a[i] >> (32 - s);
    }
    return r;
}

}

namespace hb {

bool prescale_params(hb_ctx *ctx) {
    if (ctx->psc_state) return ctx->psc_state > 0;
    ctx->psc_state = -1;
    if (ctx->n_limbs != 4 || (ctx->p_limbs[3] >> 62) == 0) return false;
    Big p(8);
    for (int i = 0; i < 4; i++) { p[2 * i] = (uint32_t)ctx->p_limbs[i]; p[2 * i + 1] = (uint32_t)(ctx->p_limbs[i] >> 32); }
    Big pw9(p); pw9.push_back(0);
    Big pb(9, 0); pb[8] = 1u << 5;
    big_sub(pb, pw9);
    for (int k = 0; k < 9; k++) {
        const int bit = 29 * k, j = bit >> 5, sft = bit & 31;
        const uint64_t v = pb[j] | ((uint64_t)(j + 1 < 9 ? pb[j + 1] : 0) << 32);
        ctx->psc.pbar[k] = (uint32_t)(v >> sft) & DMASK;
    }
    Big pn(9, 0); pn[8] = 1;
    big_sub(pn, pw9);
    for (int k = 0; k < 8; k++) ctx->psc.pneg[k] = pn[k];
    Big two290(10, 0); two290[9] = 1u << 2;
    Big mu; big_divmod(two290, p, &mu);
    const uint64_t muv = mu[0] | ((uint64_t)mu[1] << 32);
    ctx->psc.m0 = (uint32_t)muv & DMASK;
    ctx->psc.m1 = (uint32_t)(muv >> LB);
    ctx->psc_state = 1;
    return true;
}

void mm8_free(Mm8Matrix *m) {
    if (!m) return;
    (void)hipFree(m->a8); (void)hipFree(m->crow); (void)hipFree(m->zero);
    delete m;
}

int mm8_shared(hb_ctx *ctx, const Mm8Shared **out, hipStream_t s) {
    if (ctx->mm8_shared) { *out = static_cast<const Mm8Shared *>(ctx->mm8_shared); return HB_OK; }
    if (ctx->n_limbs != 4 || (ctx->p_limbs[3] >> 62) == 0 || !prescale_params(ctx)) return fail(ctx, HB_ERR_UNSUPPORTED, "mm8: modulus");
    Mm8Shared *sh = new Mm8Shared();
    memset(sh, 0, sizeof *sh);
    Big p(8);
    for (int k = 0; k < 4; k++) { p[2 * k] = (uint32_t)ctx->p_limbs[k]; p[2 * k + 1] = (uint32_t)(ctx->p_limbs[k] >> 32); }
    uint32_t shift8[8];
    if (!fold_tables(ctx, 16, sh->fold_host, sh->bp.c384, &sh->bp.mu, shift8)) { delete sh; return fail(ctx, HB_ERR_UNSUPPORTED, "mm8: fold table"); }
    {
        Big pn(9, 0); pn[8] = 1;
        Big pw9(p); pw9.push_back(0);
        big_sub(pn, pw9);
        for (int k = 0; k < 8; k++) sh->bp.pneg[k] = pn[k];
    }
    auto digits9 = [](const Big &v, uint32_t *dg) {
        for (int k = 0; k < 9; k++) {
            const int bit = 29 * k, j = bit >> 5, sft = bit & 31;
            const uint64_t w = (uint64_t)(j < (int)v.size() ? v[j] : 0) | ((uint64_t)(j + 1 < (int)v.size() ? v[j + 1] : 0) << 32);
            dg[k] = (uint32_t)(w >> sft) & DMASK;
        }
    };
    Big biasmod;
    { Big bt(14, 0); for (int c = 0; c < MM8_NC; c++) { Big t(1, (uint32_t)MM8_BIAS); big_add(bt, big_shl(t, 8 * c, 14)); } biasmod = big_divmod(bt, p, nullptr); }
    { Big sft(shift8, shift8 + 8); if (!big_ge(biasmod, sft)) big_add(biasmod, p); big_sub(biasmod, sft); }
    digits9(biasmod, sh->biasmod);
    for (int merged = 0; merged < 2; merged++) {
        Big bt(14, 0);
        for (int c = 0; c < MM8_NCP; c++) {
            Big t(1, (uint32_t)MM8_BIAS_PACK);
            big_add(bt, big_shl(t, 8 * c, 14));
            if (merged) big_add(bt, big_shl(t, 8 * (c + 8), 14));
        }
        Big bm = big_divmod(bt, p, nullptr);
        Big sft(shift8, shift8 + 8);
        if (!big_ge(bm, sft)) big_add(bm, p);
        big_sub(bm, sft);
        digits9(bm, merged ? sh->biasmod_pm : sh->biasmod_ps);
    }
    {
        Big c80(8, 0x80808080u);
        Big r261(9, 0); r261[8] = 1u << 5;
        digits9(big_divmod(big_mul(c80, r261), p, nullptr), sh->c80r);
    }
    {
        digits9(big_divmod(Big(8, 0x80808080u), p, nullptr), sh->ms_c80);
        Big bt(10, 0);
        for (int c = 0; c < 32; c++) { Big t(1, 1u << 20); big_add(bt, big_shl(t, 8 * c, 10)); }
        digits9(big_divmod(bt, p, nullptr), sh->ms_bias);
    }
    if (hipMalloc(&sh->fold_dev, sizeof sh->fold_host) != hipSuccess) { delete sh; return fail(ctx, HB_ERR_HIP, "mm8: hipMalloc(fold table)"); }
    if (int rc = upload_table(ctx, sh->fold_dev, sh->fold_host, sizeof sh->fold_host, s)) { (void)hipFree(sh->fold_dev); delete sh; return rc; }
    ctx->mm8_shared = sh;
    *out = sh;
    return HB_OK;
}

void mm8_shared_free(hb_ctx *ctx) {
    Mm8Shared *sh = static_cast<Mm8Shared *>(ctx->mm8_shared);
    if (!sh) return;
    (void)hipFree(sh->fold_dev);
    delete sh;
    ctx->mm8_shared = nullptr;
}

int mm8_from_fast(hb_ctx *ctx, const FastMatrix *f, Mm8Matrix **out, hipStream_t s, const int32_t *rows, int n_rows) {
    *out = nullptr;
    if (env_hook(ENV_NO_MFMA)) return HB_ERR_UNSUPPORTED;
    if (ctx->n_limbs != 4 || f->n_in < 1 || f->n_in > 32 || f->n_out < 1) return HB_ERR_UNSUPPORTED;
    if ((ctx->p_limbs[3] >> 62) == 0) return HB_ERR_UNSUPPORTED;
    const int n_out = rows ? n_rows : f->n_out, d = f->n_in, nkb = (d + 7) / 8, n_rt = (n_out + 15) / 16;
    if (n_out < 1) return HB_ERR_UNSUPPORTED;
    if (mm8_lds_bytes(n_rt, nkb, (n_rt == 1) ? 4 : (n_rt == 2) ? 2 : 1) > MM8_LDS_LIMIT) return HB_ERR_UNSUPPORTED;
    const int tiles = (f->n_out + f->ot - 1) / f->ot;
    std::vector<uint32_t> Mh((size_t)tiles * d * f->ot * 9);
    std::vector<int32_t> neg((size_t)f->n_out, 0);
    HB_HIP(ctx, hipMemcpyAsync(Mh.data(), f->M, Mh.size() * 4, hipMemcpyDeviceToHost, s));
    if (f->negrow) HB_HIP(ctx, hipMemcpyAsync(neg.data(), f->negrow, neg.size() * 4, hipMemcpyDeviceToHost, s));
    HB_HIP(ctx, hipStreamSynchronize(s));

    Big p(8);
    for (int k = 0; k < 4; k++) { p[2 * k] = (uint32_t)ctx->p_limbs[k]; p[2 * k + 1] = (uint32_t)(ctx->p_limbs[k] >> 32); }
    Big c80(8, 0x80808080u);
    c80 = big_divmod(c80, p, nullptr);
    Big biasmod;
    { Big bt(14, 0); for (int c = 0; c < MM8_NC; c++) { Big t(1, (uint32_t)MM8_BIAS); big_add(bt, big_shl(t, 8 * c, 14)); } biasmod = big_divmod(bt, p, nullptr); }
    std::vector<uint8_t> foldtab((size_t)MM8_FOLD_Q * 16, 0);
    BarrettParams bpar;
    {
        uint32_t shift8[8];
        if (!fold_tables(ctx, 16, foldtab.data(), bpar.c384, &bpar.mu, shift8)) return HB_ERR_UNSUPPORTED;
        Big sh(shift8, shift8 + 8);
        if (!big_ge(biasmod, sh)) big_add(biasmod, p);
        big_sub(biasmod, sh);
    }

    std::vector<int8_t> a((size_t)n_rt * nkb * 2 * 64 * 16, 0);
    bool skip01 = nkb >= 2 && !env_hook(ENV_MM8_NO_SKIP);
    std::vector<uint32_t> cr((size_t)n_rt * 16 * 16 + (size_t)MM8_FOLD_Q * 4, 0);
    memcpy(&cr[(size_t)n_rt * 16 * 16], foldtab.data(), foldtab.size());
    for (size_t i = 0; i < (size_t)n_rt * 16; i++) for (int k = 0; k < 8; k++) { cr[i * 16 + 2 * k] = 0x10100000u; cr[i * 16 + 2 * k + 1] = 0x1010u; }
    for (int i = 0; i < n_out; i++) {
        Big pos(5, 0), ngs(5, 0);
        int64_t colsum = 0;
        const int src = rows ? rows[i] : i;
        if (src < 0 || src >= f->n_out) return HB_ERR_BAD_ARG;
        for (int l = 0; l < d; l++) {
            uint32_t dg[9], w8[8];
            for (int q = 0; q < 9; q++) dg[q] = Mh[mf_index(src, l, d, 9, q, f->ot)];
            pack<9, 8>(w8, dg);
            if (w8[4] | w8[5] | w8[6] | w8[7]) return HB_ERR_UNSUPPORTED;
            const int sgn = neg[src] ? -1 : 1;
            int carry = 0;
            const int lane_ = (4 * ((i % 16) % 4) + (i % 16) / 4) + 16 * ((l % 8) / 2), el = l & 1;
            for (int b = 0; b < 16; b++) {
                int t = sgn * (int)((w8[b >> 2] >> (8 * (b & 3))) & 0xffu) + carry;
                if (t > 127) { t -= 256; carry = 1; } else if (t < -128) { t += 256; carry = -1; } else carry = 0;
                const int grp = b >> 3, r7 = 7 - (b & 7), hi = r7 >> 2, bi = r7 & 3;
                a[((((size_t)(i / 16) * nkb + l / 8) * 2 + grp) * 64 + (size_t)lane_) * 16 + 4 * (2 * hi + el) + bi] = (int8_t)t;
                if (t != 0 && grp == 1 && l < 8) skip01 = false;
                colsum += (t < 0) ? -t : t;
            }
            if (carry) return HB_ERR_UNSUPPORTED;
            Big e(w8, w8 + 4);
            big_add(neg[src] ? ngs : pos, e);
        }
        if (colsum * 128 > MM8_BIAS) return HB_ERR_UNSUPPORTED;
        Big cp = big_divmod(big_mul(c80, pos), p, nullptr), cn = big_divmod(big_mul(c80, ngs), p, nullptr);
        if (!big_ge(cp, cn)) big_add(cp, p);
        big_sub(cp, cn);
        if (!big_ge(cp, biasmod)) big_add(cp, p);
        big_sub(cp, biasmod);
        for (int k = 0; k < 8; k++) {
            const uint64_t pair = (uint64_t)cp[k] + ((0x1010ull << 32) | 0x10100000ull);
            cr[(size_t)i * 16 + 2 * k] = (uint32_t)pair;
            cr[(size_t)i * 16 + 2 * k + 1] = (uint32_t)(pair >> 32);
        }
    }
    Mm8Matrix *m = new Mm8Matrix();
    m->n_out = n_out; m->d = d; m->nkb = nkb; m->n_rt = n_rt; m->skip01 = skip01; m->a8 = nullptr; m->crow = nullptr; m->zero = nullptr;
    m->bp = bpar;
    {
        Big pn(9, 0); pn[8] = 1;
        Big pw9(p); pw9.push_back(0);
        big_sub(pn, pw9);
        for (int k = 0; k < 8; k++) m->bp.pneg[k] = pn[k];
    }
    HB_HIP(ctx, hipMalloc(&m->a8, a.size()));
    HB_HIP(ctx, hipMalloc(&m->crow, cr.size() * 4));
    HB_HIP(ctx, hipMalloc(&m->zero, 64));
    {
        std::vector<uint8_t> zero64(64, 0);
        int rc = upload_table(ctx, m->a8, a.data(), a.size(), s);
        if (!rc) rc = upload_table(ctx, m->crow, cr.data(), cr.size() * 4, s);
        if (!rc) rc = upload_table(ctx, m->zero, zero64.data(), 64, s);
        if (rc) { mm8_free(m); return rc; }
    }
    *out = m;
    return HB_OK;
}

int launch_mm8(hb_ctx *ctx, const Mm8Matrix *m, const uint32_t *in, hb_view iv, const int32_t *in_rows_dev, int64_t in_count,
               uint32_t *out, hb_view ov, int64_t out_count, const int32_t *check_mask_dev, int32_t *mismatch_dev,
               int64_t C, hipStream_t s, uint32_t *copy_dst, hb_view cpv, int64_t copy_count, int copy_rows,
               const int32_t *check_rows_dev) {
    if (C <= 0) return HB_OK;
    const int tpw = mm8_tpw(m->n_rt, m->nkb);
    const int64_t n_tiles = (C + 15) / 16;
    const int64_t n_units = (n_tiles + tpw - 1) / tpw;
    int64_t blocks = 2 * (int64_t)mm8_num_cus();
    if (blocks > n_units) blocks = n_units;
    blocks = mm8_trimmed_grid(n_units, blocks);
    const size_t lds = mm8_lds_bytes(m->n_rt, m->nkb, tpw);
    const bool check = check_mask_dev != nullptr;
    const bool ragged = !check && (m->n_out % 16) >= 1 && (m->n_out % 16) <= 8;
#define MM8_LAUNCH_(NKB, CHK, RG, SK)                                                                                 \
    do {                                                                                                          \
        static std::atomic<unsigned long long> attr_done{0};                                                                               \
        if (!((attr_done.load() >> (ctx->device & 63)) & 1ull)) {                                                                                         \
            HB_HIP(ctx, hipFuncSetAttribute(reinterpret_cast<const void *>(k_mm8<NKB, CHK, RG, SK>), hipFuncAttributeMaxDynamicSharedMemorySize, 80 * 1024)); \
            attr_done.fetch_or(1ull << (ctx->device & 63));                                                                                     \
        }                                                                                                         \
        hipLaunchKernelGGL((k_mm8<NKB, CHK, RG, SK>), dim3((unsigned)blocks), dim3(256), lds, s, m->a8, m->crow, m->zero, in, iv.stride_c, \
                           iv.stride_l, in_rows_dev, in_count, m->d, out, ov.stride_c, ov.stride_l, out_count,   \
                           check_mask_dev, check_rows_dev, mismatch_dev, copy_dst, cpv.stride_c, cpv.stride_l, copy_count, copy_rows,         \
                           m->n_out, m->n_rt, tpw, C, n_units, m->bp);             \
    } while (0)
#define MM8_LAUNCH(NKB) do { if (check) MM8_LAUNCH_(NKB, true, false, false); else if (ragged) MM8_LAUNCH_(NKB, false, true, false); else MM8_LAUNCH_(NKB, false, false, false); } while (0)
#define MM8_LAUNCH_SK(NKB) do { if (check) MM8_LAUNCH_(NKB, true, false, true); else if (ragged) MM8_LAUNCH_(NKB, false, true, false); else MM8_LAUNCH_(NKB, false, false, true); } while (0)
    switch (m->nkb) {
        case 1: MM8_LAUNCH(1); break;
        case 2: if (m->skip01) MM8_LAUNCH_SK(2); else MM8_LAUNCH(2); break;
        case 3: if (m->skip01) MM8_LAUNCH_SK(3); else MM8_LAUNCH(3); break;
        case 4: if (m->skip01) MM8_LAUNCH_SK(4); else MM8_LAUNCH(4); break;
        default: return fail(ctx, HB_ERR_UNSUPPORTED, "mm8: more than 32 terms");
    }
#undef MM8_LAUNCH
#undef MM8_LAUNCH_SK
#undef MM8_LAUNCH_
    HB_LAUNCH_CHECK(ctx);
    return HB_OK;
}

}

extern "C" int hb_debug_mm8_create(hb_ctx *ctx, const uint64_t *x_host, int n, int d, void **out) { HB_API_GUARD(ctx);
    uint32_t *xd = nullptr;
    int rc = upload_elems(ctx, x_host, (size_t)n, &xd, 0);
    if (rc) return rc;
    FastMatrix *V = nullptr;
    rc = fast_vand_create(ctx, xd, n, d, &V, 0);
    (void)hipFree(xd);
    if (rc) return rc;
    Mm8Matrix *m = nullptr;
    rc = mm8_from_fast(ctx, V, &m, 0);
    fast_matrix_free(V);
    *out = m;
    return rc;
}
extern "C" int hb_debug_mm8_apply(hb_ctx *ctx, void *mat, const void *in_dev, int64_t in_sc, int64_t in_sl, int64_t in_count,
                                  void *out_dev, int64_t out_sc, int64_t out_sl, int64_t out_count, int64_t n_chunks,
                                  const int32_t *check_mask_dev, int32_t *mismatch_dev) { HB_API_GUARD(ctx);
    hb_view iv{in_sc, in_sl}, ov{out_sc, out_sl};
    return launch_mm8(ctx, (const Mm8Matrix *)mat, (const uint32_t *)in_dev, iv, nullptr, in_count, (uint32_t *)out_dev, ov, out_count,
                      check_mask_dev, mismatch_dev, n_chunks, 0, nullptr, hb_view{0, 0}, 0, 0, nullptr);
}

#ifdef HB_MM8_TIMING
extern "C" int hb_debug_mm8_timing(unsigned long long *out, int count) {
    return hipMemcpyFromSymbol(out, HIP_SYMBOL(hb::g_mm8_t), sizeof(unsigned long long) * (size_t)count) == hipSuccess ? 0 : 1;
}
#endif
```

honeybadgermpc_amd/csrc/hb_mfma_fused.hip:

```cpp
#include <math.h>

#include <algorithm>
#include <atomic>
#include <type_traits>

#include "hb_mm8.hpp"

namespace hb {

#include "hb_mm8_body.inc"

constexpr int FS_WAVES = 8, FS_TPW = 4;
#ifdef HB_MM8_TIMING
__device__ unsigned long long g_fs_t[256 * 8 * 8];
#define FS_T(k) do { const unsigned long long tn_ = __builtin_amdgcn_s_memtime(); tacc[k] += tn_ - tlast; tlast = tn_; } while (0)
#else
#define FS_T(k) do { } while (0)
#endif
constexpr int FS_MAXD = 24, FS_MAXC = 104;
constexpr size_t FS_LDS_LIMIT = 156 * 1024;

struct FsIdx { uint16_t z[FS_MAXD], xz[FS_MAXD], zc[FS_MAXC], xzc[FS_MAXC]; };
struct FsPick { const uint4 *cand; const uint32_t *cand_crow; int n_coef, nc; uint16_t zc[FS_MAXC]; };
struct FsSplit { uint32_t terms[FS_WAVES]; };
struct FsPack { int nm, ns; uint8_t single[8]; };
__host__ __device__ inline int fs_slot(const FsPack &pk, int i, int n_out, int &kind) {
    kind = 0;
    if (!(pk.nm | pk.ns)) return i;
    const int base = 16 * ((n_out + 15) / 16 - 1);
    int before = 0;
    for (int k = 0; k < pk.ns; k++) {
        if (pk.single[k] == i) { kind = 2; return base + 4 + (k & 3) + 8 * (k >> 2); }
        before += pk.single[k] < i;
    }
    const int pos = i - before;
    if (pos >= base) kind = 1;
    return pos;
}
static bool fs_pack_decide(int d, int n_coef, int nc, const uint8_t *small, FsPack *pk) {
    memset(pk, 0, sizeof *pk);
    const int n_out = n_coef + nc, rem = n_out - 16 * ((n_out + 15) / 16 - 1);
    if ((int64_t)d * 8 * 128 * 128 > MM8_BIAS_PACK) return false;
    if (rem <= 8) { pk->nm = rem; return true; }
    if (rem == 16) return false;
    int ns = 0;
    for (int i = n_coef - 1; i >= 0 && ns < 8; i--)
        if (small[i]) pk->single[ns++] = (uint8_t)i;
    std::reverse(pk->single, pk->single + ns);
    if (rem - ns > 4) { memset(pk, 0, sizeof *pk); return false; }
    pk->nm = rem - ns; pk->ns = ns;
    return true;
}
constexpr int FS_CAND_MAXN = 128;

__host__ __device__ inline int fs_ms_q(int d) { return d * 64 + d * 8; }
__host__ __device__ inline size_t fs_lds_bytes(int n_rt, int nkb, int ms_d = 0) {
    return ((size_t)n_rt * 64 + (size_t)n_rt * nkb * 2 * 64 + (size_t)2 * FS_TPW * nkb * 4 * 64 + MM8_FOLD_Q + (ms_d ? fs_ms_q(ms_d) : 0)) * 16 +
           (size_t)(32 + 16 * n_rt) * 4;
}

#define FS_REDUCE(I_, F_, E_, C0_) \
    do { \
        const int i = (I_); \
        const int md = maskl[i]; \
        const bool live = chunk < n_chunks; \
        const bool cmp = live && md > 0, st = live && md < 0; \
        uint32_t ew[8]; \
        load_words<8>(ew, in_pk + (cmp ? (chunk * in_sc + (int64_t)(md - 1) * in_sl) * 8 : 0)); \
        uint64_t pw[8]; \
        { \
            const uint4 *cr = reinterpret_cast<const uint4 *>(crl + (size_t)i * 16); \
        _Pragma("unroll") \
            for (int k = 0; k < 4; k++) { \
                const uint4 c = cr[k]; \
                pw[2 * k] = (uint64_t)c.x | ((uint64_t)c.y << 32); \
                pw[2 * k + 1] = (uint64_t)c.z | ((uint64_t)c.w << 32); \
            } \
        } \
        uint32_t glo[5], ghi[5]; \
        _Pragma("unroll") \
        for (int k = 0; k < 12; k++) { \
            uint64_t gk = (uint64_t)F_(k) * k256 + (k < 7 ? pw[k] : 0ull); \
            if (k < 11) gk += (uint64_t)E_(k) * k16m; \
            if (k < 7) pw[k] = gk; \
            else { glo[k - 7] = (uint32_t)gk; ghi[k - 7] = (uint32_t)(gk >> 32); } \
        } \
        pw[0] += (uint64_t)(C0_) * u1; \
        pw[7] += (uint64_t)glo[0] * u1; \
        uint32_t hw[5]; \
        { \
            unsigned cyw = 0; \
        _Pragma("unroll") \
            for (int k = 0; k < 4; k++) hw[k] = __builtin_addc(glo[k + 1], ghi[k], cyw, &cyw); \
            hw[4] = ghi[4] + cyw; \
        } \
        v4i hb; \
        _Pragma("unroll") \
        for (int k = 0; k < 4; k++) hb[k] = (int)(hw[k] ^ 0x80808080u); \
        v4i dcol[8]; \
        _Pragma("unroll") \
        for (int eb = 0; eb < 8; eb++) \
            dcol[eb] = __builtin_amdgcn_mfma_i32_16x16x64_i8(fold_lane[eb * (MM8_FOLD_ROW / 16)], hb, v4i{0, 0, 0, 0}, 0, 0, 0); \
        _Pragma("unroll") \
        for (int k = 0; k < 8; k++) pw[k] += (uint64_t)hw[4] * bp.c384[k]; \
        _Pragma("unroll") \
        for (int k = 0; k < 8; k++) { \
            int64_t tt = (int64_t)pw[k] + (int64_t)dcol[k][0] * s1; \
            tt += (int64_t)dcol[k][1] * s256; \
            tt += (int64_t)dcol[k][2] * s64k; \
            tt += (int64_t)dcol[k][3] * s16m; \
            pw[k] = (uint64_t)tt; \
        } \
        const uint64_t tq = pw[7] + (pw[6] >> 32); \
        const uint32_t qh = (uint32_t)(((uint64_t)(uint32_t)(tq >> 16) * bp.mu) >> 46); \
        _Pragma("unroll") \
        for (int k = 0; k < 8; k++) pw[k] += (uint64_t)qh * bp.pneg[k]; \
        uint32_t ow[8]; \
        uint32_t top; \
        { \
            unsigned cy = 0; \
            ow[0] = (uint32_t)pw[0]; \
        _Pragma("unroll") \
            for (int k = 1; k < 8; k++) ow[k] = __builtin_addc((uint32_t)pw[k], (uint32_t)(pw[k - 1] >> 32), cy, &cy); \
            top = (uint32_t)(pw[7] >> 32) + cy - qh; \
        } \
        if (__builtin_amdgcn_ballot_w64(top != 0 || ow[7] >= ~bp.pneg[7]) != 0) { \
            uint32_t u[8]; \
            unsigned cy2 = 0; \
        _Pragma("unroll") \
            for (int k = 0; k < 8; k++) u[k] = __builtin_addc(ow[k], bp.pneg[k], cy2, &cy2); \
            const bool take = cy2 || top; \
        _Pragma("unroll") \
            for (int k = 0; k < 8; k++) ow[k] = take ? u[k] : ow[k]; \
        } \
        uint32_t diff = 0; \
        _Pragma("unroll") \
        for (int k = 0; k < 8; k++) diff |= ew[k] ^ ow[k]; \
        asm volatile("" : "+v"(diff), "+v"(ow[0]), "+v"(ow[1]), "+v"(ow[2]), "+v"(ow[3]), "+v"(ow[4]), "+v"(ow[5]), "+v"(ow[6]), "+v"(ow[7])); \
        const unsigned long long bad_lanes = __builtin_amdgcn_ballot_w64(cmp && diff); \
        if (bad_lanes) { \
            const uint32_t bits16 = (uint32_t)((bad_lanes | (bad_lanes >> 16) | (bad_lanes >> 32) | (bad_lanes >> 48)) & 0xffffull); \
            if (lane == 0) { \
                const int64_t tile_base = chunk - n; \
                const int32_t cmin = (int32_t)tile_base + __builtin_ctz(bits16); \
                if (*reinterpret_cast<volatile int32_t *>(mismatch) == 0) atomicOr(mismatch, 1); \
                if (first_bad && *reinterpret_cast<volatile int32_t *>(first_bad) > cmin) atomicMin(first_bad, cmin); \
                if (bad_map) atomicOr(bad_map + (tile_base >> 5), bits16 << (tile_base & 31)); \
            } \
        } \
        const int64_t oidx = chunk * out_sc + (int64_t)(-md - 1) * out_sl; \
        if (st && oidx < out_count) store_words<8>(out_pk + oidx * 8, ow); \
    } while (0)

template <int NKB, int PK, bool MSC>
__global__ __launch_bounds__(64 * FS_WAVES, 2) void k_mm8f(const int4 *__restrict__ a8, const uint32_t *__restrict__ crowd, const v4i *__restrict__ foldg,
                                                          const uint32_t *__restrict__ KT, const PrescaleParams PP,
                                                          const uint32_t *__restrict__ in_pk, int64_t in_sc, int64_t in_sl, const int32_t *__restrict__ in_rows,
                                                          int64_t in_count, int d, const int32_t *__restrict__ rowmode,
                                                          uint32_t *__restrict__ out_pk, int64_t out_sc, int64_t out_sl, int64_t out_count,
                                                          int32_t *__restrict__ mismatch, int32_t *__restrict__ first_bad, uint32_t *__restrict__ bad_map,
                                                          int n_out, int n_rt, int64_t n_chunks, int64_t n_units, BarrettParams bp, const FsDone done, const FsPick pick,
                                                          const FsSplit split, const v4i *__restrict__ MS) {
    constexpr bool PACKED = PK != 0;
    const int n_slots = PACKED ? 16 * n_rt : n_out;
    constexpr int NT = 64 * FS_WAVES, NL = 9, NW = 8;
    extern __shared__ uint4 fs_lds[];
    const int lane = threadIdx.x & 63, wave = __builtin_amdgcn_readfirstlane(threadIdx.x >> 6);
    const int n = lane & 15, g = lane >> 4;
    uint32_t *crl = reinterpret_cast<uint32_t *>(fs_lds);
    int4 *abuf = reinterpret_cast<int4 *>(fs_lds + n_rt * 64);
    uint4 *xbuf = fs_lds + n_rt * 64 + n_rt * NKB * 2 * 64;
    constexpr int bufsz = FS_TPW * NKB * 4 * 64;
    int32_t *rowl = reinterpret_cast<int32_t *>(xbuf + 2 * bufsz);
    int32_t *maskl = rowl + 32;
    v4i *foldl = reinterpret_cast<v4i *>(maskl + 16 * n_rt);
    v4i *msl = foldl + MM8_FOLD_Q;

#ifdef HB_MM8_TIMING
    unsigned long long tacc[8] = {0, 0, 0, 0, 0, 0, 0, 0}, tlast = __builtin_amdgcn_s_memtime();
#endif
    auto unit_chunk = [&](int64_t unit) {
        const int64_t chunk = unit * 64 + lane;
        return chunk >= n_chunks ? n_chunks - 1 : chunk;
    };
    auto fetch_halves = [&](int64_t unit, int row, uint32_t (&w)[NW], bool &okk) {
        const int r = lane & 31, h = lane >> 5;
        bool oks[2];
#pragma unroll
        for (int s = 0; s < 2; s++) {
            int64_t chunk = unit * 64 + 32 * s + r;
            chunk = chunk >= n_chunks ? n_chunks - 1 : chunk;
            const int64_t idx = chunk * in_sc + (int64_t)row * in_sl;
            oks[s] = idx < in_count;
            const uint4 v = *reinterpret_cast<const uint4 *>(in_pk + (oks[s] ? idx : 0) * NW + 4 * h);
            w[4 * s] = v.x; w[4 * s + 1] = v.y; w[4 * s + 2] = v.z; w[4 * s + 3] = v.w;
        }
        okk = h ? oks[1] : oks[0];
    };
    auto fetch_row = [&](int64_t chunk, int row, uint32_t (&w)[NW], bool &okk) {
        const int64_t idx = chunk * in_sc + (int64_t)row * in_sl;
        okk = idx < in_count;
        load_words<NW>(w, in_pk + (okk ? idx : 0) * NW);
    };
    const uint32_t first_terms = (0x01010101u << wave) & (d < 32 ? (1u << d) - 1u : ~0u);
    uint32_t x_first[NW] = {0, 0, 0, 0, 0, 0, 0, 0};
    bool ok_first = false;
    uint32_t xf[MSC ? NKB : 1][NW];
    bool okf[MSC ? NKB : 1];
    if (!MSC && first_terms) {
        const int l0 = __builtin_ctz(first_terms);
        fetch_row(unit_chunk(blockIdx.x), in_rows ? in_rows[l0] : l0, x_first, ok_first);
    }
    uint4 pk_piece = make_uint4(0, 0, 0, 0), pk_crow = make_uint4(0, 0, 0, 0);
    const int pk_e = threadIdx.x;
    const bool pk_has_piece = !PACKED && pick.cand && pk_e < pick.nc * NKB * 8, pk_has_crow = !PACKED && pick.cand && pk_e < pick.nc * 4;
    if (pk_has_piece) {
        const int j = pk_e / (NKB * 8), pc = pk_e - j * (NKB * 8);
        pk_piece = pick.cand[(size_t)pick.zc[j] * (NKB * 8) + pc];
    }
    if (pk_has_crow) pk_crow = reinterpret_cast<const uint4 *>(pick.cand_crow)[(size_t)pick.zc[pk_e >> 2] * 4 + (pk_e & 3)];
    {
        const int tid = threadIdx.x, n_mask = n_rt * 16, n_crow = n_rt * 64, n_img = n_rt * NKB * 2 * 64;
        const int lc = tid < d ? tid : d - 1;
        int32_t rw = in_rows ? in_rows[lc] : lc;
        int32_t mk = rowmode[tid < n_slots ? tid : 0];
        v4i cr = reinterpret_cast<const v4i *>(crowd)[tid < n_crow ? tid : 0];
        v4i fo = foldg[tid < MM8_FOLD_Q ? tid : 0];
        v4i img[3];
#pragma unroll
        for (int k = 0; k < 3; k++) img[k] = reinterpret_cast<const v4i *>(a8)[tid + k * NT < n_img ? tid + k * NT : 0];
        const int ms_lj = wave + 8 * (lane >> 3), ms_cq = d * 64 + (ms_lj < d ? ms_lj : d - 1) * 8 + (lane & 7);
        v4i msv[MSC ? NKB + 1 : 1];
        if constexpr (MSC) {
#pragma unroll
            for (int j = 0; j < NKB; j++) {
                const int l = wave + 8 * j, lc = l < d ? l : d - 1;
                msv[j] = MS[lc * 64 + lane];
            }
            msv[NKB] = MS[ms_cq];
#pragma unroll
            for (int j = 0; j < NKB; j++) {
                const int l = wave + 8 * j, lc = l < d ? l : d - 1;
                fetch_halves(blockIdx.x, in_rows ? in_rows[lc] : lc, xf[j], okf[j]);
                okf[j] = okf[j] && l < d;
            }
        }
        asm volatile("" : "+v"(rw), "+v"(mk), "+v"(cr), "+v"(fo), "+v"(img[0]), "+v"(img[1]), "+v"(img[2]));
        if constexpr (MSC) {
#pragma unroll
            for (int j = 0; j <= NKB; j++) asm volatile("" : "+v"(msv[j]));
        }
        if (tid < 32) rowl[tid] = rw;
        if (tid < n_mask) maskl[tid] = tid < n_slots ? mk : 0;
        if (tid < n_crow) reinterpret_cast<v4i *>(fs_lds)[tid] = cr;
        if (tid < MM8_FOLD_Q) foldl[tid] = fo;
#pragma unroll
        for (int k = 0; k < 3; k++)
            if (tid + k * NT < n_img) reinterpret_cast<v4i *>(abuf)[tid + k * NT] = img[k];
        if constexpr (MSC) {
#pragma unroll
            for (int j = 0; j < NKB; j++) {
                const int l = wave + 8 * j, lc = l < d ? l : d - 1;
                msl[lc * 64 + lane] = msv[j];
            }
            if (lane < 8 * NKB) msl[ms_cq] = msv[NKB];
        }
        for (int i = tid + NT; i < n_mask; i += NT) maskl[i] = i < n_slots ? rowmode[i] : 0;
        for (int i = tid + NT; i < n_crow; i += NT) fs_lds[i] = reinterpret_cast<const uint4 *>(crowd)[i];
        for (int i = tid + 3 * NT; i < n_img; i += NT) abuf[i] = a8[i];
    }
    for (int i = threadIdx.x; i < (8 * NKB - d) * 256; i += NT) {
        const int l = d + (i >> 8), b = (i >> 7) & 1, t = (i >> 5) & 3, h = (i >> 4) & 1, c = i & 15;
        const int kb = l >> 3, gg = (l & 7) >> 1, e = l & 1;
        xbuf[(size_t)b * bufsz + (size_t)((((t * NKB + kb) * 2 + e) * 2 + h) * 64) + (c + 16 * gg)] = make_uint4(0, 0, 0, 0);
    }
    const int n_pairs = FS_TPW * n_rt;
    const uint32_t my_terms = (uint32_t)__builtin_amdgcn_readfirstlane((int)split.terms[wave]);

    uint32_t ms64k = 1u << 16;
    if constexpr (MSC) asm volatile("" : "+s"(ms64k));
    typedef int v16i __attribute__((ext_vector_type(16)));
    const v4i *ms_al = msl + lane, *ms_cl = msl + d * 64 + 4 * (lane >> 5);
    auto ms_products = [&](int l, const uint32_t (&x)[NW], v16i &acc0, v16i &acc1) __attribute__((always_inline)) {
        const v4i a = ms_al[l * 64];
        const v4i *cl = ms_cl + l * 8;
        v16i c;
#pragma unroll
        for (int q = 0; q < 4; q++) {
            const v4i cq = cl[q];
#pragma unroll
            for (int k = 0; k < 4; k++) c[4 * q + k] = cq[k];
        }
        const v4i b0 = v4i{(int)(x[0] ^ 0x80808080u), (int)(x[1] ^ 0x80808080u), (int)(x[2] ^ 0x80808080u), (int)(x[3] ^ 0x80808080u)};
        const v4i b1 = v4i{(int)(x[4] ^ 0x80808080u), (int)(x[5] ^ 0x80808080u), (int)(x[6] ^ 0x80808080u), (int)(x[7] ^ 0x80808080u)};
        acc0 = __builtin_amdgcn_mfma_i32_32x32x32_i8(a, b0, c, 0, 0, 0);
        acc1 = __builtin_amdgcn_mfma_i32_32x32x32_i8(a, b1, c, 0, 0, 0);
    };
    auto ms_words = [&](const v16i &acc0, const v16i &acc1, uint64_t (&mw)[8]) __attribute__((always_inline)) {
#pragma unroll
        for (int q = 0; q < 4; q++) {
            uint64_t ad[2];
#pragma unroll
            for (int s = 0; s < 2; s++) {
                const v16i &m = s ? acc1 : acc0;
                const uint32_t lo = (uint32_t)m[4 * q] + ((uint32_t)m[4 * q + 1] << 8), hi = (uint32_t)m[4 * q + 2] + ((uint32_t)m[4 * q + 3] << 8);
                ad[s] = (uint64_t)hi * ms64k + lo;
            }
            const auto slo = __builtin_amdgcn_permlane32_swap((uint32_t)ad[0], (uint32_t)ad[1], false, false);
            const auto shi = __builtin_amdgcn_permlane32_swap((uint32_t)(ad[0] >> 32), (uint32_t)(ad[1] >> 32), false, false);
            mw[2 * q] = (uint64_t)slo[0] | ((uint64_t)shi[0] << 32);
            mw[2 * q + 1] = (uint64_t)slo[1] | ((uint64_t)shi[1] << 32);
        }
    };
    auto scale_unit = [&](auto first, int64_t unit, uint4 *dst, uint32_t terms) {
        constexpr bool FIRST = decltype(first)::value;
        const int64_t chunk = unit_chunk(unit);
        const int t = lane >> 4;
        uint32_t xw[NW];
        bool ok = false;
        auto fetch = [&](int l, uint32_t (&w)[NW], bool &okk) {
            if constexpr (MSC) fetch_halves(unit, rowl[l], w, okk);
            else fetch_row(chunk, FIRST ? (in_rows ? in_rows[l] : l) : rowl[l], w, okk);
        };
        terms &= d < 32 ? (1u << d) - 1u : ~0u;
        int l = terms ? __builtin_ctz(terms) : d;
        if constexpr (FIRST) {
#pragma unroll
            for (int k = 0; k < NW; k++) xw[k] = x_first[k];
            ok = ok_first;
        } else if (l < d) fetch(l, xw, ok);
        while (l < d) {
            terms &= terms - 1u;
            const int ln = terms ? __builtin_ctz(terms) : d;
            uint32_t xn[NW];
            bool okn = false;
            fetch(ln < d ? ln : l, xn, okn);
            uint32_t w[NW];
            bool over;
            if constexpr (MSC) {
                static_assert(!FIRST, "the first unit's matrix-core tasks are the block at the call site");
                v16i acc0, acc1;
                ms_products(l, xw, acc0, acc1);
                uint64_t mw[8];
                ms_words(acc0, acc1, mw);
                const uint64_t tq = mw[7] + (mw[6] >> 32);
                const uint32_t mq = (uint32_t)(((uint64_t)(uint32_t)(tq >> 16) * bp.mu) >> 46);
#pragma unroll
                for (int k = 0; k < 8; k++) mw[k] += (uint64_t)mq * bp.pneg[k];
                unsigned cyw = 0;
                w[0] = (uint32_t)mw[0];
#pragma unroll
                for (int k = 1; k < 8; k++) w[k] = __builtin_addc((uint32_t)mw[k], (uint32_t)(mw[k - 1] >> 32), cyw, &cyw);
                over = (uint32_t)(mw[7] >> 32) + cyw != mq;
            } else {
                const uint32_t *__restrict__ T = KT + (size_t)l * (NL * NL);
                uint32_t xd[NL];
                unpack<NL, NW>(xd, xw);
                uint64_t col[NL + 1];
#pragma unroll
                for (int j = 0; j <= NL; j++) col[j] = 0;
#pragma unroll
                for (int q = 0; q < NL; q++)
#pragma unroll
                    for (int j = 0; j < NL; j++) col[j] += (uint64_t)xd[q] * T[q * NL + j];
                uint32_t v[NL + 1];
#pragma unroll
                for (int k = 0; k < NL; k++) { v[k] = (uint32_t)col[k] & DMASK; col[k + 1] += col[k] >> LB; }
                v[NL] = (uint32_t)col[NL];
                const uint64_t mid = (uint64_t)v[9] * PP.m0 + (uint64_t)v[8] * PP.m1 + (((uint64_t)v[8] * PP.m0) >> LB);
                const uint64_t qh = (uint64_t)v[9] * PP.m1 + (mid >> LB);
                const uint32_t q0 = (uint32_t)qh & DMASK, q1 = (uint32_t)(qh >> LB);
                uint64_t dc[NL];
#pragma unroll
                for (int k = 0; k < NL; k++) {
                    dc[k] = v[k] + (uint64_t)q0 * PP.pbar[k];
                    if (k > 0) dc[k] += (uint64_t)q1 * PP.pbar[k - 1];
                }
                uint32_t r[NL];
#pragma unroll
                for (int k = 0; k < NL; k++) {
                    r[k] = (uint32_t)dc[k] & DMASK;
                    if (k < NL - 1) dc[k + 1] += dc[k] >> LB;
                }
                pack<NL, NW>(w, r);
                over = (r[NL - 1] >> 24) != 0;
            }
            const uint32_t *pneg = MSC ? bp.pneg : PP.pneg;
            if (pneg[NW - 1] >> 31) {
#pragma unroll
                for (int k = 0; k < NW; k++) w[k] = ok ? w[k] : 0u;
            } else {
                uint32_t u[NW];
                unsigned cy = 0;
#pragma unroll
                for (int k = 0; k < NW; k++) u[k] = __builtin_addc(w[k], pneg[k], cy, &cy);
                const bool take = cy || over;
#pragma unroll
                for (int k = 0; k < NW; k++) w[k] = ok ? (take ? u[k] : w[k]) : 0u;
            }
            const int kb = l >> 3, gg = (l & 7) >> 1, e = l & 1;
            uint4 *slot = dst + (size_t)(((t * NKB + kb) * 2 + e) * 2) * 64 + (n + 16 * gg);
            slot[0] = make_uint4(w[0], w[1], w[2], w[3]);
            slot[64] = make_uint4(w[4], w[5], w[6], w[7]);
#pragma unroll
            for (int k = 0; k < NW; k++) xw[k] = xn[k];
            ok = okn;
            l = ln;
        }
    };

    if constexpr (MSC) {
        const int t = lane >> 4;
        auto first_block = [&](auto canon_c) __attribute__((always_inline)) {
            constexpr bool CANON = decltype(canon_c)::value;
            v16i mc[NKB][2];
#pragma unroll
            for (int s = 0; s <= NKB; s++) {
                if (s < NKB) {
                    const int j = s, l = wave + 8 * j, lc = l < d ? l : d - 1;
                    ms_products(lc, xf[j], mc[j][0], mc[j][1]);
                }
                if (s > 0) {
                    const int j = s - 1, l = wave + 8 * j;
                    uint64_t mw[8];
                    ms_words(mc[j][0], mc[j][1], mw);
                    const uint64_t tq = mw[7] + (mw[6] >> 32);
                    const uint32_t mq = (uint32_t)(((uint64_t)(uint32_t)(tq >> 16) * bp.mu) >> 46);
#pragma unroll
                    for (int k = 0; k < 8; k++) mw[k] += (uint64_t)mq * bp.pneg[k];
                    uint32_t w[NW];
                    unsigned cyw = 0;
                    w[0] = (uint32_t)mw[0];
#pragma unroll
                    for (int k = 1; k < 8; k++) w[k] = __builtin_addc((uint32_t)mw[k], (uint32_t)(mw[k - 1] >> 32), cyw, &cyw);
                    if constexpr (CANON) {
                        const bool over = (uint32_t)(mw[7] >> 32) + cyw != mq;
                        uint32_t u[NW];
                        unsigned cy = 0;
#pragma unroll
                        for (int k = 0; k < NW; k++) u[k] = __builtin_addc(w[k], bp.pneg[k], cy, &cy);
                        const bool take = cy || over;
#pragma unroll
                        for (int k = 0; k < NW; k++) w[k] = okf[j] ? (take ? u[k] : w[k]) : 0u;
                    } else {
#pragma unroll
                        for (int k = 0; k < NW; k++) w[k] = okf[j] ? w[k] : 0u;
                    }
                    const int gg = (l & 7) >> 1, e = l & 1;
                    uint4 *slot = xbuf + (size_t)(((t * NKB + j) * 2 + e) * 2) * 64 + (n + 16 * gg);
                    slot[0] = make_uint4(w[0], w[1], w[2], w[3]);
                    slot[64] = make_uint4(w[4], w[5], w[6], w[7]);
                }
                __builtin_amdgcn_sched_barrier(0);
            }
        };
        if (bp.pneg[NW - 1] >> 31) first_block(std::false_type{});
        else first_block(std::true_type{});
    } else
        scale_unit(std::true_type{}, blockIdx.x, xbuf, first_terms);
    if (!PACKED && pick.cand) {
        __syncthreads();
        auto put = [&](int e, const uint4 &v) {
            const int j = e / (NKB * 8), pc = e - j * (NKB * 8);
            const int ri = pick.n_coef + j, rt = ri >> 4, r16 = ri & 15, r = 4 * (r16 & 3) + (r16 >> 2);
            const int kb = pc >> 3, grp = (pc >> 2) & 1, gg = pc & 3;
            reinterpret_cast<uint4 *>(abuf)[((rt * NKB + kb) * 2 + grp) * 64 + r + 16 * gg] = v;
        };
        if (pk_has_piece) put(pk_e, pk_piece);
        for (int e = pk_e + NT; e < pick.nc * NKB * 8; e += NT) {
            const int j = e / (NKB * 8), pc = e - j * (NKB * 8);
            put(e, pick.cand[(size_t)pick.zc[j] * (NKB * 8) + pc]);
        }
        if (pk_has_crow) fs_lds[(pick.n_coef + (pk_e >> 2)) * 4 + (pk_e & 3)] = pk_crow;
        for (int j = threadIdx.x; j < pick.nc; j += NT) maskl[pick.n_coef + j] = (int32_t)pick.zc[j] + 1;
    }

    const v4i biasv = v4i{MM8_BIAS, MM8_BIAS, MM8_BIAS, MM8_BIAS};
    uint32_t k256 = 256u, k16m = 1u << 24;
    int32_t s1 = 1, s256 = 256, s64k = 1 << 16, s16m = 1 << 24;
    uint32_t u1 = 1u;
    asm volatile("" : "+s"(k256), "+s"(k16m), "+s"(s1), "+s"(s256), "+s"(s64k), "+s"(s16m), "+s"(u1));
    const v4i *fold_lane = reinterpret_cast<const v4i *>(reinterpret_cast<const char *>(foldl) + (g == (n >> 2) ? 16 * n : 256));

    int buf = 0;
    int64_t unit = blockIdx.x;
    FS_T(0);
    for (; unit < n_units; unit += gridDim.x, buf ^= 1) {
        asm volatile("s_waitcnt lgkmcnt(0)" ::: "memory");
        FS_T(7);
        __builtin_amdgcn_s_barrier();
        FS_T(1);
        if (my_terms && unit + gridDim.x < n_units) scale_unit(std::false_type{}, unit + gridDim.x, xbuf + (size_t)(buf ^ 1) * bufsz, my_terms);
        FS_T(2);
        for (int pidx = wave; pidx < n_pairs; pidx += FS_WAVES) {
            const int tl = n_rt == 2 ? (pidx >> 1) : pidx / n_rt;
            const int rt = n_rt == 2 ? ((pidx ^ (pidx >> 2)) & 1) : pidx - tl * n_rt;
            const int64_t chunk = (unit * FS_TPW + tl) * 16 + n;
            const uint4 *xs = xbuf + (size_t)buf * bufsz + (size_t)tl * NKB * 4 * 64 + lane;
            const int4 *as = abuf + (size_t)rt * NKB * 2 * 64 + lane;
            uint32_t eap[4][11], c0p[4];
            const int rows_here = n_out - 16 * rt < 16 ? n_out - 16 * rt : 16;
            const int nreg = PACKED ? 4 : (rows_here + 3) >> 2;
            const uint32_t xs_addr = (uint32_t)(uintptr_t)(__attribute__((address_space(3))) const void *)xs;
            const uint32_t as_addr = (uint32_t)(uintptr_t)(__attribute__((address_space(3))) const void *)as;
            if (PACKED && rt == n_rt - 1) {
                const v4i biaspv = v4i{MM8_BIAS_PACK, MM8_BIAS_PACK, MM8_BIAS_PACK, MM8_BIAS_PACK};
                auto park_merged = [&](auto rc, const v4i (&acc)[20]) __attribute__((always_inline)) {
                    constexpr int r = decltype(rc)::value;
                    c0p[r] = (uint32_t)acc[0][r];
#pragma unroll
                    for (int j = 0; j < 11; j++) {
                        uint32_t lo = 0, hi = 0;
                        if (j < 9) { lo = (uint32_t)acc[1 + 2 * j][r]; hi = (uint32_t)acc[2 + 2 * j][r]; }
                        if (j >= 2) { lo += (uint32_t)acc[2 * j - 3][r + 2]; hi += (uint32_t)acc[2 * j - 2][r + 2]; }
                        if (j == 1) hi += (uint32_t)acc[0][r + 2];
                        eap[r][j] = lo + (hi << 8);
                    }
                };
                auto park_single = [&](auto rc, const v4i (&acc)[20]) __attribute__((always_inline)) {
                    constexpr int r = decltype(rc)::value;
                    c0p[r] = (uint32_t)acc[0][r];
#pragma unroll
                    for (int j = 0; j < 11; j++) eap[r][j] = j < 9 ? (uint32_t)acc[1 + 2 * j][r] + ((uint32_t)acc[2 + 2 * j][r] << 8) : 0u;
                };
                auto keep = [&](auto rc) __attribute__((always_inline)) {
                    constexpr int r = decltype(rc)::value;
                    asm volatile("" ::"v"(c0p[r]), "v"(eap[r][0]), "v"(eap[r][1]), "v"(eap[r][2]), "v"(eap[r][3]), "v"(eap[r][4]), "v"(eap[r][5]),
                                 "v"(eap[r][6]), "v"(eap[r][7]), "v"(eap[r][8]), "v"(eap[r][9]), "v"(eap[r][10]));
                    __builtin_amdgcn_sched_barrier(0);
                };
                {
                    v4i acc[20];
                    asm volatile("" ::: "memory");
                    __builtin_amdgcn_sched_barrier(0);
                    __builtin_amdgcn_s_setprio(0);
                    Mm8PhasePacked<NKB, 0>::run(acc, xs_addr, as_addr, biaspv);
                    __builtin_amdgcn_s_setprio(2);
                    __builtin_amdgcn_sched_barrier(0);
                    FS_T(3);
                    park_merged(std::integral_constant<int, 0>{}, acc);
                    keep(std::integral_constant<int, 0>{});
                    if constexpr (PK == 1) park_merged(std::integral_constant<int, 1>{}, acc);
                    else park_single(std::integral_constant<int, 1>{}, acc);
                    keep(std::integral_constant<int, 1>{});
                    if constexpr (PK == 2) {
                        park_single(std::integral_constant<int, 3>{}, acc);
                        keep(std::integral_constant<int, 3>{});
                    }
                }
                {
                    v4i acc[20];
                    asm volatile("" ::: "memory");
                    __builtin_amdgcn_sched_barrier(0);
                    FS_T(4);
                    __builtin_amdgcn_s_setprio(0);
                    Mm8PhasePacked<NKB, 1>::run(acc, xs_addr, as_addr, biaspv);
                    __builtin_amdgcn_s_setprio(2);
                    __builtin_amdgcn_sched_barrier(0);
                    FS_T(5);
                    auto pair_merged = [&](auto rc, int k) __attribute__((always_inline)) {
                        constexpr int r = decltype(rc)::value;
                        uint32_t lo = 0, hi = 0;
                        if (k < 10) { lo = (uint32_t)acc[2 * k][r]; hi = (uint32_t)acc[2 * k + 1][r]; }
                        if (k >= 2) { lo += (uint32_t)acc[2 * k - 4][r + 2]; hi += (uint32_t)acc[2 * k - 3][r + 2]; }
                        return lo + (hi << 8);
                    };
                    auto pair_single = [&](auto rc, int k) __attribute__((always_inline)) {
                        constexpr int r = decltype(rc)::value;
                        return k < 10 ? (uint32_t)acc[2 * k][r] + ((uint32_t)acc[2 * k + 1][r] << 8) : 0u;
                    };
#define FS_FM0(k) pair_merged(std::integral_constant<int, 0>{}, k)
#define FS_FM1(k) pair_merged(std::integral_constant<int, 1>{}, k)
#define FS_FS1(k) pair_single(std::integral_constant<int, 1>{}, k)
#define FS_FS3(k) pair_single(std::integral_constant<int, 3>{}, k)
#define FS_E0(k) eap[0][k]
#define FS_E1(k) eap[1][k]
#define FS_E3(k) eap[3][k]
                    if constexpr (PK == 2) { FS_REDUCE(16 * rt + 12 + g, FS_FS3, FS_E3, c0p[3]); __builtin_amdgcn_sched_barrier(0); }
                    FS_REDUCE(16 * rt + g, FS_FM0, FS_E0, c0p[0]);
                    if constexpr (PK == 1) FS_REDUCE(16 * rt + 4 + g, FS_FM1, FS_E1, c0p[1]);
                    else FS_REDUCE(16 * rt + 4 + g, FS_FS1, FS_E1, c0p[1]);
#undef FS_FM0
#undef FS_FM1
#undef FS_FS1
#undef FS_FS3
#undef FS_E0
#undef FS_E1
#undef FS_E3
                }
                FS_T(6);
                continue;
            }
            {
                v4i acc[24];
                asm volatile("" ::: "memory");
                __builtin_amdgcn_sched_barrier(0);
                __builtin_amdgcn_s_setprio(0);
                Mm8Phase<NKB, 0, false>::run(acc, xs_addr, as_addr, biasv);
                __builtin_amdgcn_s_setprio(2);
                __builtin_amdgcn_sched_barrier(0);
                FS_T(3);
#pragma unroll
                for (int reg = 0; reg < 4; reg++) {
                    if (reg >= 2 && reg >= nreg) break;
                    c0p[reg] = (uint32_t)acc[0][reg];
#pragma unroll
                    for (int j = 0; j < 11; j++) eap[reg][j] = (uint32_t)acc[1 + 2 * j][reg] + ((uint32_t)acc[2 + 2 * j][reg] << 8);
                    asm volatile("" ::"v"(c0p[reg]), "v"(eap[reg][0]), "v"(eap[reg][1]), "v"(eap[reg][2]), "v"(eap[reg][3]), "v"(eap[reg][4]),
                                 "v"(eap[reg][5]), "v"(eap[reg][6]), "v"(eap[reg][7]), "v"(eap[reg][8]), "v"(eap[reg][9]), "v"(eap[reg][10]));
                    __builtin_amdgcn_sched_barrier(0);
                }
            }
            {
                v4i acc[24];
                asm volatile("" ::: "memory");
                __builtin_amdgcn_sched_barrier(0);
                FS_T(4);
                __builtin_amdgcn_s_setprio(0);
                Mm8Phase<NKB, 1, false>::run(acc, xs_addr, as_addr, biasv);
                __builtin_amdgcn_s_setprio(2);
                __builtin_amdgcn_sched_barrier(0);
                FS_T(5);
#pragma unroll
                for (int reg = 0; reg < 4; reg++) {
                    if (reg >= 2 && reg >= nreg) break;
#define FS_F(k) ((uint32_t)acc[2 * (k)][reg] + ((uint32_t)acc[2 * (k) + 1][reg] << 8))
#define FS_E(k) eap[reg][k]
                    FS_REDUCE(16 * rt + 4 * reg + g, FS_F, FS_E, c0p[reg]);
#undef FS_F
#undef FS_E
                    if (reg & 1) __builtin_amdgcn_sched_barrier(0);
                }
            }
            FS_T(6);
        }
    }
#ifdef HB_MM8_TIMING
    if (lane == 0 && blockIdx.x < 256) for (int k = 0; k < 8; k++) g_fs_t[(blockIdx.x * 8 + wave) * 8 + k] = tacc[k];
#endif
    fs_workgroup_done(done, mismatch, first_bad);
}

typedef __int128 i128;

struct FsConsts {
    uint32_t c80r[9], biasmod[9], biasmod_pm[9], biasmod_ps[9];
    uint32_t ms_c80[9], ms_bias[9], pneg[8];
};
constexpr int FS_MS_BIAS = 1 << 20;
constexpr int32_t FS_OVERFLOW = 0x40000000;

__device__ __forceinline__ size_t fs_digit_addr(int i, int l, int b, int nkb) {
    const int lane_ = (4 * ((i % 16) % 4) + (i % 16) / 4) + 16 * ((l % 8) / 2), el = l & 1;
    const int grp = b >> 3, r7 = 7 - (b & 7), hi = r7 >> 2, bi = r7 & 3;
    return ((((size_t)(i / 16) * nkb + l / 8) * 2 + grp) * 64 + (size_t)lane_) * 16 + 4 * (2 * hi + el) + bi;
}

__device__ __forceinline__ void fs_row_constant(const FpParams<9> &P, const FsConsts &cs, const i128 *row, int d, uint32_t *dst16, int kind = 0) {
    constexpr int NL = 9, NW = 8;
    uint32_t s5[5] = {0, 0, 0, 0, 0};
    for (int l = 0; l < d; l++) {
        const i128 v = row[l];
        const uint32_t vw[5] = {(uint32_t)v, (uint32_t)(v >> 32), (uint32_t)(v >> 64), (uint32_t)(v >> 96), (uint32_t)(v >> 127 >> 1)};
        unsigned cy = 0;
#pragma unroll
        for (int k = 0; k < 5; k++) s5[k] = __builtin_addc(s5[k], vw[k], cy, &cy);
    }
    const bool negs = (s5[4] >> 31) != 0;
    if (negs) {
        unsigned cy = 1;
#pragma unroll
        for (int k = 0; k < 5; k++) s5[k] = __builtin_addc(~s5[k], 0u, cy, &cy);
    }
    uint32_t w8[NW] = {s5[0], s5[1], s5[2], s5[3], s5[4], 0, 0, 0}, fe[NL], prod[NL], corr[NL], k80[NL], bm[NL];
    unpack<NL, NW>(fe, w8);
    if (negs) fp_neg(fe, fe, P);
#pragma unroll
    for (int k = 0; k < NL; k++) { k80[k] = cs.c80r[k]; bm[k] = kind == 0 ? cs.biasmod[k] : kind == 1 ? cs.biasmod_pm[k] : cs.biasmod_ps[k]; }
    mont_mul(prod, fe, k80, P);
    fp_sub(corr, prod, bm, P);
    uint32_t cw[NW];
    pack<NL, NW>(cw, corr);
#pragma unroll
    for (int k = 0; k < 8; k++) {
        const uint64_t pair = (uint64_t)cw[k] + ((0x1010ull << 32) | 0x10100000ull);
        dst16[2 * k] = (uint32_t)pair;
        dst16[2 * k + 1] = (uint32_t)(pair >> 32);
    }
}

__device__ __forceinline__ void fs_build_body(uint8_t *fb_lds, const FpParams<9> &P, const uint32_t *__restrict__ inv, int n, const FsIdx &ix, int d, int nc, int n_coef,
                                              int flags, const FsConsts &cs, uint8_t *__restrict__ a8, uint32_t *__restrict__ crow, uint32_t *__restrict__ KT,
                                              int32_t *__restrict__ rowmode, int32_t *__restrict__ z_dev, int32_t *__restrict__ status, const FsPack &pk,
                                              uint8_t *__restrict__ ms = nullptr) {
    constexpr int NL = 9, NW = 8;
    const int n_out = n_coef + nc, nkb = (d + 7) / 8, n_rt = (n_out + 15) / 16;
    i128 *ent = reinterpret_cast<i128 *>(fb_lds);
    i128 *Ac = ent + (size_t)n_out * d;
    uint32_t *wj = reinterpret_cast<uint32_t *>(Ac + (d + 1));
    uint32_t *part = wj + (size_t)d * NL;
    const int tid = threadIdx.x;
    const bool do_z = flags & FS_BUILD_Z, do_zc = flags & FS_BUILD_ZC;
    if (do_z) {
        const size_t img = (size_t)n_rt * nkb * 2 * 64 * 16;
        for (size_t i = tid; i < img / 16; i += 1024) reinterpret_cast<uint4 *>(a8)[i] = make_uint4(0, 0, 0, 0);
        for (int i = tid; i < n_rt * 16 * 8; i += 1024) { crow[2 * i] = 0x10100000u; crow[2 * i + 1] = 0x1010u; }
        for (int i = tid; i < n_rt * 16; i += 1024) rowmode[i] = 0;
        if (tid < d) z_dev[tid] = ix.z[tid];
    }
    if (do_z && tid < 64) {
        if (tid <= d) Ac[tid] = tid == 0 ? 1 : 0;
        __builtin_amdgcn_fence(__ATOMIC_RELEASE, "wavefront");
        __builtin_amdgcn_wave_barrier();
        for (int q = 0; q < d; q++) {
            i128 nv = 0;
            const bool act = tid <= q + 1 && tid <= d;
            if (act) nv = (tid > 0 ? Ac[tid - 1] : (i128)0) - (i128)ix.xz[q] * Ac[tid];
            __builtin_amdgcn_fence(__ATOMIC_ACQ_REL, "wavefront");
            __builtin_amdgcn_wave_barrier();
            if (act) Ac[tid] = nv;
            __builtin_amdgcn_fence(__ATOMIC_ACQ_REL, "wavefront");
            __builtin_amdgcn_wave_barrier();
        }
        if (tid < d) {
            const i128 xj = ix.xz[tid];
            i128 cur = 1;
            for (int m = d - 1; m >= 0; m--) {
                if (m < n_coef) ent[(size_t)m * d + tid] = cur;
                if (m > 0) cur = Ac[m] + xj * cur;
            }
        }
    } else if (do_z && tid < 64 + 4 * FS_MAXD + 32) {
        const int j = (tid - 64) >> 2, pq = (tid - 64) & 3;
        if (j < d) {
            uint32_t w[NL];
            fp_set(w, P.one);
            const uint32_t *row = inv + (size_t)ix.z[j] * n * NL;
            for (int q = pq; q < d; q += 4) {
                if (q == j) continue;
                uint32_t f[NL];
#pragma unroll
                for (int k = 0; k < NL; k++) f[k] = row[(size_t)ix.z[q] * NL + k];
                mont_mul(w, w, f, P);
            }
#pragma unroll
            for (int k = 0; k < NL; k++) part[((size_t)j * 4 + pq) * NL + k] = w[k];
        }
    } else if (do_zc && tid >= 256) {
        for (int e = tid - 256; e < nc * d; e += 1024 - 256) {
            const int i = e / d, j = e - i * d;
            const int64_t xi = ix.xzc[i];
            i128 v = 1;
            for (int q = 0; q < d; q++)
                if (q != j) v *= (i128)(xi - (int64_t)ix.xz[q]);
            ent[(size_t)(n_coef + i) * d + j] = v;
        }
    }
    __syncthreads();
    if (do_z && tid < d) {
        uint32_t a[NL], b[NL], c[NL];
#pragma unroll
        for (int k = 0; k < NL; k++) { a[k] = part[((size_t)tid * 4) * NL + k]; b[k] = part[((size_t)tid * 4 + 1) * NL + k]; }
        mont_mul(c, a, b, P);
#pragma unroll
        for (int k = 0; k < NL; k++) { a[k] = part[((size_t)tid * 4 + 2) * NL + k]; b[k] = part[((size_t)tid * 4 + 3) * NL + k]; }
        mont_mul(a, a, b, P);
        mont_mul(c, c, a, P);
#pragma unroll
        for (int k = 0; k < NL; k++) wj[(size_t)tid * NL + k] = c[k];
    }
    __syncthreads();
    const int row_lo = do_z ? 0 : n_coef, row_hi = do_zc ? n_out : n_coef;
    for (int e = tid + row_lo * d; e < row_hi * d; e += 1024) {
        const int i = e / d, l = e - i * d;
        i128 v = ent[e];
        const bool negv = v < 0;
        int carry = 0, kind;
        const int sl = fs_slot(pk, i, n_out, kind);
        bool lost = false;
#pragma unroll
        for (int b = 0; b < 16; b++) {
            int t = (int)((uint32_t)(v >> (8 * b)) & 0xffu) + carry;
            if (t > 127) { t -= 256; carry = 1; } else carry = 0;
            if (kind == 0) a8[fs_digit_addr(sl, l, b, nkb)] = (uint8_t)(int8_t)t;
            else if (b < 8 || kind == 1) a8[fs_digit_addr(sl + (b < 8 ? 0 : 8), l, b & 7, nkb)] = (uint8_t)(int8_t)t;
            else lost |= t != 0;
        }
        if ((lost || carry != (negv ? 1 : 0)) && status) atomicOr(status, FS_OVERFLOW);
    }
    for (int i = tid + row_lo; i < row_hi; i += 1024) {
        int kind;
        const int sl = fs_slot(pk, i, n_out, kind);
        fs_row_constant(P, cs, ent + (size_t)i * d, d, crow + (size_t)sl * 16, kind);
        rowmode[sl] = i < n_coef ? -(i + 1) : (int32_t)ix.zc[i - n_coef] + 1;
    }
    if (do_z) {
        for (int e = tid; e < d * NL; e += 1024) {
            const int l = e / NL, q = e - l * NL;
            uint32_t w[NL], two[NL], tq[NL];
#pragma unroll
            for (int k = 0; k < NL; k++) { w[k] = wj[(size_t)l * NL + k]; two[k] = (k == q) ? 1u : 0u; }
            mont_mul(tq, w, two, P);
#pragma unroll
            for (int k = 0; k < NL; k++) KT[((size_t)l * NL + q) * NL + k] = tq[k];
        }
    }
    if (do_z && ms) {
        for (int e = tid; e < d * 32; e += 1024) {
            const int l = e >> 5, b = e & 31;
            uint32_t w[NL], two[NL], u[NL], uw[NW];
#pragma unroll
            for (int k = 0; k < NL; k++) { w[k] = wj[(size_t)l * NL + k]; two[k] = (k == (8 * b) / LB) ? 1u << ((8 * b) % LB) : 0u; }
            mont_mul(u, w, two, P);
            pack<NL, NW>(uw, u);
            int8_t dg[32];
            int carry = 0;
            for (int pass = 0; pass < 2; pass++) {
                carry = 0;
                for (int c = 0; c < 32; c++) {
                    int t = (int)((uw[c >> 2] >> (8 * (c & 3))) & 0xffu) + carry;
                    if (t > 127) { t -= 256; carry = 1; } else carry = 0;
                    dg[c] = (int8_t)t;
                }
                if (carry == pass) break;
                if (pass == 0) {
                    unsigned cy = 0;
#pragma unroll
                    for (int k = 0; k < NW; k++) uw[k] = __builtin_addc(uw[k], cs.pneg[k], cy, &cy);
                } else if (status) atomicOr(status, FS_OVERFLOW);
            }
            for (int c = 0; c < 32; c++) ms[(size_t)((l * 2 + (b >> 4)) * 32 + c) * 16 + (b & 15)] = (uint8_t)dg[c];
        }
        for (int l = tid; l < d; l += 1024) {
            uint32_t w[NL], c80[NL], bm[NL], prod[NL], kk[NL], kw[NW];
#pragma unroll
            for (int k = 0; k < NL; k++) { w[k] = wj[(size_t)l * NL + k]; c80[k] = cs.ms_c80[k]; bm[k] = cs.ms_bias[k]; }
            mont_mul(prod, w, c80, P);
            fp_sub(kk, prod, bm, P);
            pack<NL, NW>(kw, kk);
            int32_t *ci = reinterpret_cast<int32_t *>(ms + (size_t)d * 1024) + l * 32;
            for (int c = 0; c < 32; c++) ci[16 * ((c >> 2) & 1) + 4 * (c >> 3) + (c & 3)] = FS_MS_BIAS + (int32_t)((kw[c >> 2] >> (8 * (c & 3))) & 0xffu);
        }
    }
}

__device__ __forceinline__ void fs_cand_body(uint8_t *fc_lds, const FpParams<9> &P, int n, const uint16_t *__restrict__ xs, const FsIdx &ix, int d, const FsConsts &cs,
                                             uint8_t *__restrict__ cand, uint32_t *__restrict__ cand_crow, int32_t *__restrict__ status) {
    i128 *ent = reinterpret_cast<i128 *>(fc_lds);
    const int tid = threadIdx.x, nkb = (d + 7) / 8;
    const size_t row_bytes = (size_t)nkb * 8 * 16;
    for (size_t i = tid; i < (size_t)n * row_bytes / 16; i += 1024) reinterpret_cast<uint4 *>(cand)[i] = make_uint4(0, 0, 0, 0);
    for (int e = tid; e < n * d; e += 1024) {
        const int i = e / d, j = e - i * d;
        const int64_t xi = xs[i];
        i128 v = 1;
        for (int q = 0; q < d; q++)
            if (q != j) v *= (i128)(xi - (int64_t)ix.xz[q]);
        ent[e] = v;
    }
    __syncthreads();
    for (int e = tid; e < n * d; e += 1024) {
        const int i = e / d, l = e - i * d;
        const i128 v = ent[e];
        const bool negv = v < 0;
        const int kb = l >> 3, gg = (l & 7) >> 1, el = l & 1;
        int carry = 0;
#pragma unroll
        for (int b = 0; b < 16; b++) {
            int t = (int)((uint32_t)(v >> (8 * b)) & 0xffu) + carry;
            if (t > 127) { t -= 256; carry = 1; } else carry = 0;
            const int grp = b >> 3, r7 = 7 - (b & 7), hi = r7 >> 2, bi = r7 & 3;
            cand[(size_t)i * row_bytes + (size_t)(((kb * 2 + grp) * 4 + gg) * 16) + 4 * (2 * hi + el) + bi] = (uint8_t)(int8_t)t;
        }
        if (carry != (negv ? 1 : 0) && status) atomicOr(status, FS_OVERFLOW);
    }
    for (int i = tid; i < n; i += 1024) fs_row_constant(P, cs, ent + (size_t)i * d, d, cand_crow + (size_t)i * 16);
}

__global__ void __launch_bounds__(1024) k_fs_build(const FpParams<9> P, const uint32_t *__restrict__ inv, int n, const FsIdx ix, int d, int nc, int n_coef,
                                                   int flags, const FsConsts cs, uint8_t *__restrict__ a8, uint32_t *__restrict__ crow, uint32_t *__restrict__ KT,
                                                   int32_t *__restrict__ rowmode, int32_t *__restrict__ z_dev, int32_t *__restrict__ status, const FsPack pk,
                                                   uint8_t *__restrict__ ms) {
    extern __shared__ __attribute__((aligned(16))) uint8_t fs_b_lds[];
    fs_build_body(fs_b_lds, P, inv, n, ix, d, nc, n_coef, flags, cs, a8, crow, KT, rowmode, z_dev, status, pk, ms);
}

__global__ void __launch_bounds__(1024) k_fs_cand(const FpParams<9> P, int n, const uint16_t *__restrict__ xs, const FsIdx ix, int d, const FsConsts cs,
                                                  uint8_t *__restrict__ cand, uint32_t *__restrict__ cand_crow, int32_t *__restrict__ status) {
    extern __shared__ __attribute__((aligned(16))) uint8_t fs_c_lds[];
    fs_cand_body(fs_c_lds, P, n, xs, ix, d, cs, cand, cand_crow, status);
}

__global__ void __launch_bounds__(1024) k_fs_build_z_cand(const FpParams<9> P, const uint32_t *__restrict__ inv, int n, const uint16_t *__restrict__ xs, const FsIdx ix, int d, int nc,
                                                          int n_coef, const FsConsts cs, uint8_t *__restrict__ a8, uint32_t *__restrict__ crow, uint32_t *__restrict__ KT,
                                                          int32_t *__restrict__ rowmode, int32_t *__restrict__ z_dev, uint8_t *__restrict__ cand, uint32_t *__restrict__ cand_crow,
                                                          int32_t *__restrict__ status) {
    extern __shared__ __attribute__((aligned(16))) uint8_t fs_zc_lds[];
    if (blockIdx.x == 0) fs_build_body(fs_zc_lds, P, inv, n, ix, d, nc, n_coef, FS_BUILD_Z, cs, a8, crow, KT, rowmode, z_dev, status, FsPack{});
    else fs_cand_body(fs_zc_lds, P, n, xs, ix, d, cs, cand, cand_crow, status);
}

static int fs_num_cus() {
    static int n = 0;
    if (!n) {
        int dev = 0;
        (void)hipGetDevice(&dev);
        if (hipDeviceGetAttribute(&n, hipDeviceAttributeMultiprocessorCount, dev) != hipSuccess || n <= 0) n = 256;
    }
    return n;
}

int fs_layout(hb_ctx *ctx, const PointTable *pt, int d, int nc, int n_coef, FsLayout *L) {
    if (ctx->n_limbs != 4 || !pt || !pt->usable || !pt->small) return HB_ERR_UNSUPPORTED;
    if (d < 4 || d > 22 || nc < 0 || nc > FS_MAXC || n_coef < 1 || n_coef > d) return HB_ERR_UNSUPPORTED;
    if (env_hook(ENV_NO_MFMA) || env_hook(ENV_NO_FUSED_SMALL) || env_hook(ENV_NO_QUICK) || !prescale_params(ctx)) return HB_ERR_UNSUPPORTED;
    if ((int64_t)d * 16 * 128 * 128 > MM8_BIAS) return HB_ERR_UNSUPPORTED;
    std::vector<uint16_t> xs(pt->xs);
    std::sort(xs.begin(), xs.end());
    double bits_n = 0.0, bits_p = 0.0;
    for (int k = 0; k < d - 1 && k < (int)xs.size(); k++) bits_n += log2(1.0 + xs[xs.size() - 1 - k]);
    const int R = xs.empty() ? 0 : xs.back() - xs.front();
    for (int k = 0; k < d - 1; k++) { const int dist = R - k / 2; if (dist < 1) break; bits_p += log2((double)dist); }
// ... 257 lines not shown
```

honeybadgermpc_amd/csrc/hb_mm8.hpp:

```cpp
#pragma once
#include "hb_common.hpp"

namespace hb {

typedef int v4i __attribute__((ext_vector_type(4)));

constexpr int MM8_NC = 47;
constexpr int MM8_CW = 13;
constexpr int MM8_FOLD_ROW = 272;
constexpr int MM8_FOLD_Q = 8 * MM8_FOLD_ROW / 16;
constexpr int MM8_BIAS = 5800000;
constexpr int MM8_NCP = 39;
constexpr int MM8_BIAS_PACK = MM8_BIAS / 2;

struct BarrettParams {
    uint32_t pneg[8];
    uint32_t c384[8];
    uint32_t mu;
};

struct Mm8Matrix {
    int n_out, d, nkb, n_rt;
    bool skip01;
    int4 *a8;
    uint32_t *crow;
    uint32_t *zero;
    BarrettParams bp;
};

struct Mm8Shared {
    BarrettParams bp;
    uint32_t c80r[9], biasmod[9];
    uint32_t biasmod_pm[9], biasmod_ps[9];
    uint32_t ms_c80[9], ms_bias[9];
    uint8_t fold_host[MM8_FOLD_Q * 16];
    v4i *fold_dev;
};
int mm8_shared(hb_ctx *ctx, const Mm8Shared **out, hipStream_t s);
int64_t mm8_trimmed_grid(int64_t n_units, int64_t blocks);
void mm8_shared_free(hb_ctx *ctx);

}
```

Before: 9.862 billion.

## Pre-bias element bytes in LDS with interleaved granule layout to drop in-phase XORs

Adds pre-biased MFMA phase variants (Mm8PhaseB / Mm8PhasePackedB) that expect the element buffer to already hold bytes XORed with 0x80808080, stored in an interleaved granule layout. In the plain mm8 kernel a prebias pass runs on the next buffer after the current unit. In the fused kernel the bias is applied at the point the elements are stored to LDS. This removes the per-phase v_xor instructions and frees some reserved VGPRs from the inline asm. The cost is an extra LDS read-modify-write pass in k_mm8 and a changed LDS load layout. A generator-side symbolic checker verifies that the new schedules are equivalent to the old ones, and an env switch can turn the path off.

After: 10.04 billion (median of 6 runs). 1.02x the previous value.

```diff
diff --git a/honeybadgermpc_amd/csrc/gen_mm8.py b/honeybadgermpc_amd/csrc/gen_mm8.py
--- a/honeybadgermpc_amd/csrc/gen_mm8.py
+++ b/honeybadgermpc_amd/csrc/gen_mm8.py
@@ -1,5 +1,6 @@
 #!/usr/bin/env python3
 import os
+import re
 
 NC = 47
 MAXKB = 4
@@ -136,6 +137,241 @@
     return L, ncol
 
 
+CLOBBER_LO_B = 196
+
+
+def lds_loads_b(kb, xs_op, as_op, packed=False):
+    a0, a1 = ABUF[kb & 1]
+    out = []
+    for j in range(4):
+        r = f(0, 2 * j, 0)
+        out.append(f"ds_read_b128 v[{r}:{r + 3}], {xs_op} offset:{(kb * 4 + j) * 1024}")
+    out.append(f"ds_read_b128 v[{a0}:{a0 + 3}], {as_op} offset:{(kb * 2) * 1024}")
+    if not packed:
+        out.append(f"ds_read_b128 v[{a1}:{a1 + 3}], {as_op} offset:{(kb * 2 + 1) * 1024}")
+    return out
+
+
+def asm_half_b(half, nkb, skip=False, packed=False):
+    assert not skip or nkb >= 2
+    assert not (skip and packed)
+    cols = packed_columns(half) if packed else half_columns(half)
+    pos = {c: i for i, c in enumerate(cols)}
+    ncol = len(cols)
+    xs_op, as_op, bias = f"%{ncol}", f"%{ncol + 1}", f"%{ncol + 2}"
+    rho0 = HALF_RHOS[half][0]
+    L = []
+    for s in range(2):
+        for k in (-2, 8):
+            for e in (0, 1):
+                L.append(f"v_mov_b32 v{f(s, k, e)}, 0")
+    for e in (0, 1):
+        L.append(f"v_mov_b32 v{f(0, -1, e)}, 0")
+    groups = [(kb, rho) for kb in range(nkb) for rho in HALF_RHOS[half]]
+
+    def fetch(kb):
+        ops = lds_loads_b(kb, xs_op, as_op, packed)
+        return ops[:5] if skip and kb == 0 else ops
+
+    def prep(gi):
+        kb, rho = groups[gi]
+        s = gi & 1
+        ops = []
+        if rho == rho0:
+            assert s == 0
+            ops.append("s_waitcnt lgkmcnt(0)")
+            if rho != 0:
+                for e in (0, 1):
+                    ops.append(f"v_alignbyte_b32 v{f(0, -1, e)}, v{f(0, 0, e)}, 0, {rho}")
+                    for k in range(0, 8):
+                        ops.append(f"v_alignbyte_b32 v{f(0, k, e)}, v{f(0, k + 1, e)}, v{f(0, k, e)}, {rho}")
+        else:
+            assert s == 1
+            for e in (0, 1):
+                for k in range(-1, 8):
+                    ops.append(f"v_alignbyte_b32 v{f(1, k, e)}, v{f(0, k + 1, e)}, v{f(0, k, e)}, 1")
+        return ops
+
+    started = set()
+
+    def mfmas(gi):
+        kb, rho = groups[gi]
+        s = gi & 1
+        out = []
+        for q in windows(rho):
+            r = f(s, q, 0)
+            assert r % 2 == 0
+            for grp in ((0,) if packed else (0, 1)):
+                if skip and kb == 0 and grp == 1:
+                    continue
+                c = 4 * q + rho + 7 + 8 * grp
+                ab = ABUF[kb & 1][grp]
+                cin = f"%{pos[c]}"
+                if c not in started:
+                    assert kb == 0 or (skip and kb == 1)
+                    cin = bias
+                    started.add(c)
+                out.append(f"v_mfma_i32_16x16x64_i8 %{pos[c]}, v[{ab}:{ab + 3}], v[{r}:{r + 3}], {cin}")
+        return out
+
+    L += fetch(0) + prep(0) + ["s_nop 1"]
+    for gi in range(len(groups)):
+        nxt = gi + 1 < len(groups)
+        kb, rho = groups[gi]
+        mm = mfmas(gi)
+        if not nxt:
+            L += mm
+        elif rho == rho0:
+            L += interleave(mm, prep(gi + 1)) + ["s_nop 0"]
+        else:
+            hold = len(mm) - 2 if rho0 == 0 else len(mm) // 2
+            L += fetch(kb + 1) + mm[:hold] + interleave(mm[hold:], prep(gi + 1)) + ["s_nop 0"]
+    assert started == set(cols)
+    L += ["s_nop 7", "s_nop 7"]
+    return L, ncol
+
+
+def check_phase(lines, half, nkb, skip, packed, prebiased):
+    cols = packed_columns(half) if packed else half_columns(half)
+    ncol = len(cols)
+    reg = {}
+    pending = {}
+    valu_age = {}
+    done = set()
+    n_mfma = 0
+
+    def outside(k, rho):
+        return 4 * k + rho + 3 < 0 or 4 * k + rho >= 32
+
+    def tick(n):
+        for r in list(valu_age):
+            valu_age[r] += n
+            if valu_age[r] > 8:
+                del valu_age[r]
+
+    def rd(r):
+        assert r not in pending, f"v{r} read while its LDS read is in flight"
+        return reg.get(r)
+
+    def wr(r, v):
+        assert r not in pending, f"v{r} written while its LDS read is in flight"
+        assert CLOBBER_LO_B <= r <= CLOBBER_HI if prebiased else CLOBBER_LO <= r <= CLOBBER_HI, f"v{r} outside the reserved range"
+        reg[r] = v
+        valu_age[r] = 0
+
+    def num(tok):
+        return int(tok.strip().rstrip(",").lstrip("v"))
+
+    for ln in lines:
+        t = ln.replace(",", " ").split()
+        op = t[0]
+        if op == "s_nop":
+            tick(int(t[1]) + 1)
+            continue
+        if op == "s_waitcnt":
+            assert t[1] == "lgkmcnt(0)"
+            for r, v in pending.items():
+                reg[r] = v
+            pending.clear()
+            tick(1)
+            continue
+        tick(1)
+        if op == "v_mov_b32":
+            assert t[2] == "0"
+            wr(num(t[1]), "z")
+        elif op == "v_xor_b32":
+            assert not prebiased and t[2] == "0x80808080"
+            v = rd(num(t[3]))
+            assert v is not None and v != "z"
+            wr(num(t[1]), v)
+        elif op == "v_alignbyte_b32":
+            d, n = num(t[1]), int(t[4])
+            hi = rd(num(t[2]))
+            lo = "z" if t[3] == "0" else rd(num(t[3]))
+            assert hi is not None and lo is not None, ln
+            if hi == "z" and lo == "z":
+                wr(d, "z")
+                continue
+            ref = lo if lo != "z" else hi
+            _, kb, k, rho, e = ref
+            if lo == "z":
+                k -= 1
+            assert lo == ("x", kb, k, rho, e) or (lo == "z" and outside(k, rho)), ln
+            assert hi == ("x", kb, k + 1, rho, e) or (hi == "z" and outside(k + 1, rho)), ln
+            assert rho + n <= 3
+            wr(d, ("x", kb, k, rho + n, e))
+        elif op == "ds_read_b128":
+            m = re.match(r"v\[(\d+):(\d+)\]", t[1])
+            lo_r, hi_r = int(m.group(1)), int(m.group(2))
+            assert hi_r == lo_r + 3 and (CLOBBER_LO_B if prebiased else CLOBBER_LO) <= lo_r and hi_r <= CLOBBER_HI
+            slot, rem = divmod(int(t[3].split(":")[1]), 1024)
+            assert rem == 0
+            for i in range(4):
+                if t[2] == f"%{ncol}":
+                    if prebiased:
+                        kb, j = divmod(slot, 4)
+                        v = ("x", kb, 2 * j + (i >> 1), 0, i & 1)
+                    else:
+                        kb, eh = divmod(slot, 4)
+                        v = ("x", kb, 4 * (eh & 1) + i, 0, eh >> 1)
+                else:
+                    assert t[2] == f"%{ncol + 1}"
+                    v = ("a", slot >> 1, slot & 1, i)
+                assert lo_r + i not in pending
+                pending[lo_r + i] = v
+                reg.pop(lo_r + i, None)
+                valu_age.pop(lo_r + i, None)
+        elif op == "v_mfma_i32_16x16x64_i8":
+            n_mfma += 1
+            acc = int(t[1].lstrip("%"))
+            ma, mb = re.match(r"v\[(\d+):(\d+)\]", t[2]), re.match(r"v\[(\d+):(\d+)\]", t[3])
+            a0, b0 = int(ma.group(1)), int(mb.group(1))
+            for r in list(range(a0, a0 + 4)) + list(range(b0, b0 + 4)):
+                assert valu_age.get(r, 99) > 2, f"v{r}: VALU write {valu_age[r]} wait states before the MFMA that reads it"
+            av = [rd(a0 + i) for i in range(4)]
+            assert av[0] is not None and av[0][0] == "a"
+            _, kb, grp, _ = av[0]
+            assert av == [("a", kb, grp, i) for i in range(4)], ln
+            bv = [rd(b0 + i) for i in range(4)]
+            ref = next(v for v in bv if v not in (None, "z"))
+            _, kbx, k, rho, e = ref
+            q = k - bv.index(ref) // 2
+            for i in range(4):
+                kk, ee = q + (i >> 1), i & 1
+                assert bv[i] == ("x", kb, kk, rho, ee) or (bv[i] == "z" and outside(kk, rho)), (ln, bv)
+            assert kbx == kb and rho in HALF_RHOS[half]
+            c = 4 * q + rho + 7 + 8 * grp
+            assert not packed or grp == 0
+            assert cols[acc] == c, ln
+            cin = t[4]
+            first = not any(dc == c for dc, _, _ in done)
+            assert cin == (f"%{ncol + 2}" if first else f"%{acc}"), ln
+            assert (c, kb, grp) not in done
+            done.add((c, kb, grp))
+        else:
+            raise AssertionError(ln)
+    assert not pending
+    want = set()
+    for rho in HALF_RHOS[half]:
+        for q in windows(rho):
+            for grp in ((0,) if packed else (0, 1)):
+                for kb in range(nkb):
+                    if not (skip and kb == 0 and grp == 1):
+                        want.add((4 * q + rho + 7 + 8 * grp, kb, grp))
+    assert done == want and n_mfma == len(want)
+    assert lines[-2:] == ["s_nop 7", "s_nop 7"]
+    return n_mfma, {c for c, _, _ in done}
+
+
+def variants():
+    out = []
+    for nkb, skip in [(k, False) for k in range(1, MAXKB + 1)] + [(k, True) for k in range(2, MAXKB + 1)]:
+        out += [(nkb, half, skip, False) for half in range(2)]
+    for nkb in range(1, MAXKB + 1):
+        out += [(nkb, half, False, True) for half in range(2)]
+    return out
+
+
 def emit():
     out = ["// GENERATED by gen_mm8.py -- do not edit", ""]
     out.append("// column held by accumulator i of each half (half 0: rho in {0,1}; half 1: rho in {2,3})")
@@ -148,6 +384,7 @@
     for nkb, skip in [(k, False) for k in range(1, MAXKB + 1)] + [(k, True) for k in range(2, MAXKB + 1)]:
         for half in range(2):
             lines, ncol = asm_half(half, nkb, skip)
+            check_phase(lines, half, nkb, skip, False, False)
             out.append(f"template <> struct Mm8Phase<{nkb}, {half}, {'true' if skip else 'false'}> {{")
             out.append("    static __device__ __forceinline__ void run(v4i (&acc)[24], uint32_t xs_addr, uint32_t as_addr, v4i biasv) {")
             out.append("        asm volatile(")
@@ -165,6 +402,7 @@
     for nkb in range(1, MAXKB + 1):
         for half in range(2):
             lines, ncol = asm_half(half, nkb, packed=True)
+            check_phase(lines, half, nkb, False, True, False)
             assert sum("v_mfma" in ln for ln in lines) == len(windows(HALF_RHOS[half][0]) + windows(HALF_RHOS[half][1])) * nkb
             out.append(f"template <> struct Mm8PhasePacked<{nkb}, {half}> {{")
             out.append("    static __device__ __forceinline__ void run(v4i (&acc)[20], uint32_t xs_addr, uint32_t as_addr, v4i biasv) {")
@@ -177,6 +415,29 @@
             out.append(f'            : {clob}, "memory");')
             out.append("    }")
             out.append("};")
+    out.append("// pre-biased phases: the element buffer holds biased bytes in interleaved granules (gen_mm8.py); accumulators as above")
+    out.append("template <int NKB, int HALF, bool SKIP = false> struct Mm8PhaseB;")
+    out.append("template <int NKB, int HALF> struct Mm8PhasePackedB;")
+    clob_b = ", ".join(f'"v{r}"' for r in range(CLOBBER_LO_B, CLOBBER_HI + 1))
+    for nkb, half, skip, packed in variants():
+        lines, ncol = asm_half_b(half, nkb, skip, packed)
+        old_lines, _ = asm_half(half, nkb, skip, packed)
+        assert check_phase(lines, half, nkb, skip, packed, True) == check_phase(old_lines, half, nkb, skip, packed, False)
+        assert not any("0x80808080" in ln or "v_xor" in ln for ln in lines)
+        if packed:
+            out.append(f"template <> struct Mm8PhasePackedB<{nkb}, {half}> {{")
+        else:
+            out.append(f"template <> struct Mm8PhaseB<{nkb}, {half}, {'true' if skip else 'false'}> {{")
+        out.append(f"    static __device__ __forceinline__ void run(v4i (&acc)[{20 if packed else 24}], uint32_t xs_addr, uint32_t as_addr, v4i biasv) {{")
+        out.append("        asm volatile(")
+        for ln in lines:
+            out.append(f'            "{ln}\\n\\t"')
+        outs = ", ".join(f'"=&v"(acc[{i}])' for i in range(ncol))
+        out.append(f"            : {outs}")
+        out.append('            : "v"(xs_addr), "v"(as_addr), "v"(biasv)')
+        out.append(f'            : {clob_b}, "memory");')
+        out.append("    }")
+        out.append("};")
     return "\n".join(out) + "\n"
 
 
diff --git a/honeybadgermpc_amd/csrc/hb_common.hpp b/honeybadgermpc_amd/csrc/hb_common.hpp
--- a/honeybadgermpc_amd/csrc/hb_common.hpp
+++ b/honeybadgermpc_amd/csrc/hb_common.hpp
@@ -99,6 +99,7 @@
     ENV_MM8W_FLAT,
     ENV_MM8W_RQ,
     ENV_MM8W_TILE16,
+    ENV_MM8_NO_PREBIAS,
     ENV_MM8_NO_SKIP,
     ENV_NO_EVAL_FEW,
     ENV_NO_FUSED_MSCALE,
diff --git a/honeybadgermpc_amd/csrc/hb_core.hip b/honeybadgermpc_amd/csrc/hb_core.hip
--- a/honeybadgermpc_amd/csrc/hb_core.hip
+++ b/honeybadgermpc_amd/csrc/hb_core.hip
@@ -448,7 +448,7 @@
 
 
 namespace hb {
-static const char *const ENV_NAMES[ENV_COUNT] = {"HB_CACHE_CAP", "HB_GAO_PAIR", "HB_MM8W_FLAT", "HB_MM8W_RQ", "HB_MM8W_TILE16", "HB_MM8_NO_SKIP", "HB_NO_EVAL_FEW", "HB_NO_FUSED_MSCALE", "HB_NO_FUSED_PACK", "HB_NO_FUSED_SMALL", "HB_NO_FUSED_VALIDATE", "HB_NO_MFMA", "HB_NO_MFMA_DECODE", "HB_NO_MFMA_WIDE", "HB_NO_NARROW_FAST", "HB_NO_QUICK", "HB_NO_QUICK_PLAN", "HB_NTT_STAGE_LOOP", "HB_PROBE_WGS", "HB_QUICK_NO_CAND", "HB_UPLOAD_MODE", "HB_WB_NO_GAO", "HB_WB_NO_UNIFORM"};
+static const char *const ENV_NAMES[ENV_COUNT] = {"HB_CACHE_CAP", "HB_GAO_PAIR", "HB_MM8W_FLAT", "HB_MM8W_RQ", "HB_MM8W_TILE16", "HB_MM8_NO_PREBIAS", "HB_MM8_NO_SKIP", "HB_NO_EVAL_FEW", "HB_NO_FUSED_MSCALE", "HB_NO_FUSED_PACK", "HB_NO_FUSED_SMALL", "HB_NO_FUSED_VALIDATE", "HB_NO_MFMA", "HB_NO_MFMA_DECODE", "HB_NO_MFMA_WIDE", "HB_NO_NARROW_FAST", "HB_NO_QUICK", "HB_NO_QUICK_PLAN", "HB_NTT_STAGE_LOOP", "HB_PROBE_WGS", "HB_QUICK_NO_CAND", "HB_UPLOAD_MODE", "HB_WB_NO_GAO", "HB_WB_NO_UNIFORM"};
 static std::string g_env_val[ENV_COUNT];
 static bool g_env_set[ENV_COUNT];
 static std::once_flag g_env_once;
diff --git a/honeybadgermpc_amd/csrc/hb_mfma.hip b/honeybadgermpc_amd/csrc/hb_mfma.hip
--- a/honeybadgermpc_amd/csrc/hb_mfma.hip
+++ b/honeybadgermpc_amd/csrc/hb_mfma.hip
@@ -12,7 +12,7 @@
 #else
 #define MM8_T(k) do { } while (0)
 #endif
-template <int NKB, bool CHECK, bool RAGGED, bool SKIP>
+template <int NKB, bool CHECK, bool RAGGED, bool SKIP, bool PB = false>
 __global__ __launch_bounds__(256, 2) void k_mm8(const int4 *__restrict__ a8, const uint32_t *__restrict__ crowd,
                                                 const uint32_t *__restrict__ zero_src,
                                                 const uint32_t *__restrict__ in_pk, int64_t in_sc, int64_t in_sl,
@@ -54,6 +54,41 @@
     const int n_slots = tpw * NKB * 4;
     auto issue_loads = [&](int64_t unit, int buf) {
         const int64_t c_last = (unit * tpw + tpw) * 16 - 1;
+        if constexpr (PB) {
+            static_assert(!PB || !CHECK, "CHECK reads raw elements out of xbuf");
+            const bool fast = fast_dma && c_last < n_chunks && c_last * in_sc + (int64_t)rowmax * in_sl < in_count;
+#pragma nounroll
+            for (int q = wave; q < tpw * NKB; q += 4) {
+                const int t = q / NKB, kb = q - t * NKB;
+                const uint32_t lds_dst = __builtin_amdgcn_readfirstlane(
+                    (uint32_t)(uintptr_t)(__attribute__((address_space(3))) void *)(xbuf + (size_t)buf * bufsz + q * 4 * 64));
+                if (fast) {
+                    const uint64_t sbase = (uint64_t)(uintptr_t)in_pk + (uint64_t)((unit * tpw + t) * 16 * in_sc) * 32;
+                    const uint2 ro = *reinterpret_cast<const uint2 *>(rowoff + 8 * kb + 2 * g);
+                    const uint32_t voff0 = lane_off + ro.x, voff1 = lane_off + ro.y, voff0h = voff0 + 16, voff1h = voff1 + 16;
+                    uint32_t keep;
+                    asm volatile("s_mov_b32 %0, m0\n\ts_mov_b32 m0, %6\n\ts_nop 0\n\tglobal_load_lds_dwordx4 %1, %5\n\t"
+                                 "s_add_u32 m0, m0, 0x400\n\ts_nop 0\n\tglobal_load_lds_dwordx4 %2, %5\n\t"
+                                 "s_add_u32 m0, m0, 0x400\n\ts_nop 0\n\tglobal_load_lds_dwordx4 %3, %5\n\t"
+                                 "s_add_u32 m0, m0, 0x400\n\ts_nop 0\n\tglobal_load_lds_dwordx4 %4, %5\n\ts_mov_b32 m0, %0"
+                                 : "=&s"(keep) : "v"(voff0), "v"(voff0h), "v"(voff1), "v"(voff1h), "s"(sbase), "s"(lds_dst) : "memory", "scc");
+                    continue;
+                }
+                int64_t chunk = (unit * tpw + t) * 16 + n;
+                if (chunk >= n_chunks) chunk = n_chunks - 1;
+#pragma nounroll
+                for (int eh = 0; eh < 4; eh++) {
+                    const int64_t idx = chunk * in_sc + (int64_t)rowl[8 * kb + 2 * g + (eh >> 1)] * in_sl;
+                    const uint4 *src = (idx < in_count) ? reinterpret_cast<const uint4 *>(in_pk) + idx * 2 + (eh & 1)
+                                                        : reinterpret_cast<const uint4 *>(zero_src) + (eh & 1);
+                    const uint32_t dst = lds_dst + eh * 1024;
+                    uint32_t keep;
+                    asm volatile("s_mov_b32 %0, m0\n\ts_mov_b32 m0, %2\n\ts_nop 0\n\tglobal_load_lds_dwordx4 %1, off\n\ts_mov_b32 m0, %0"
+                                 : "=&s"(keep) : "v"(src), "s"(dst) : "memory");
+                }
+            }
+            return;
+        }
         if (fast_dma && c_last < n_chunks && c_last * in_sc + (int64_t)rowmax * in_sl < in_count) {
             for (int s = wave; s < n_slots; s += 4) {
                 const int h = s & 1, e = (s >> 1) & 1, q = s >> 2, t = q / NKB, kb = q - t * NKB;
@@ -80,6 +115,19 @@
             asm volatile("s_mov_b32 %0, m0\n\ts_mov_b32 m0, %2\n\ts_nop 0\n\tglobal_load_lds_dwordx4 %1, off\n\ts_mov_b32 m0, %0"
                          : "=&s"(keep) : "v"(src), "s"(lds_dst) : "memory");
         }
+    };
+    auto prebias = [&](int b) {
+#pragma clang loop vectorize(disable) interleave(disable) unroll(disable)
+        for (int q = wave; q < tpw * NKB; q += 4) {
+            uint4 *p = xbuf + (size_t)b * bufsz + (size_t)q * 4 * 64 + lane;
+            const uint4 a0 = p[0], a1 = p[64], c0 = p[128], c1 = p[192];
+            const uint32_t m = 0x80808080u;
+            p[0] = make_uint4(a0.x ^ m, c0.x ^ m, a0.y ^ m, c0.y ^ m);
+            p[64] = make_uint4(a0.z ^ m, c0.z ^ m, a0.w ^ m, c0.w ^ m);
+            p[128] = make_uint4(a1.x ^ m, c1.x ^ m, a1.y ^ m, c1.y ^ m);
+            p[192] = make_uint4(a1.z ^ m, c1.z ^ m, a1.w ^ m, c1.w ^ m);
+        }
+        asm volatile("s_waitcnt lgkmcnt(0)" ::: "memory");
     };
     const v4i biasv = v4i{MM8_BIAS, MM8_BIAS, MM8_BIAS, MM8_BIAS};
     uint32_t k256 = 256u, k16m = 1u << 24;
@@ -106,6 +154,7 @@
     }
     if (threadIdx.x < MM8_FOLD_Q) foldl[threadIdx.x] = reinterpret_cast<const v4i *>(crowd + (size_t)n_rt * 256)[threadIdx.x];
     asm volatile("s_waitcnt vmcnt(0) lgkmcnt(0)" ::: "memory");
+    if constexpr (PB) { if (unit < n_units) prebias(0); }
     const v4i *fold_lane = reinterpret_cast<const v4i *>(reinterpret_cast<const char *>(foldl) + (g == (n >> 2) ? 16 * n : 256));
     MM8_T(0);
     for (; unit < n_units; unit += gridDim.x, buf ^= 1) {
@@ -144,7 +193,8 @@
                 asm volatile("" ::: "memory");
                 __builtin_amdgcn_sched_barrier(0);
                 __builtin_amdgcn_s_setprio(0);
-                Mm8Phase<NKB, 0, SKIP>::run(acc, xs_addr, as_addr, biasv);
+                if constexpr (PB) Mm8PhaseB<NKB, 0, SKIP>::run(acc, xs_addr, as_addr, biasv);
+                else Mm8Phase<NKB, 0, SKIP>::run(acc, xs_addr, as_addr, biasv);
                 __builtin_amdgcn_s_setprio(2);
                 __builtin_amdgcn_sched_barrier(0);
                 MM8_T(3);
@@ -165,7 +215,8 @@
                 __builtin_amdgcn_sched_barrier(0);
                 MM8_T(4);
                 __builtin_amdgcn_s_setprio(0);
-                Mm8Phase<NKB, 1, SKIP>::run(acc, xs_addr, as_addr, biasv);
+                if constexpr (PB) Mm8PhaseB<NKB, 1, SKIP>::run(acc, xs_addr, as_addr, biasv);
+                else Mm8Phase<NKB, 1, SKIP>::run(acc, xs_addr, as_addr, biasv);
                 __builtin_amdgcn_s_setprio(2);
                 __builtin_amdgcn_sched_barrier(0);
                 MM8_T(5);
@@ -271,6 +322,8 @@
             }
             MM8_T(7);
         }
+        if constexpr (PB) { if (unit + gridDim.x < n_units) prebias(buf ^ 1); }
+        MM8_T(6);
     }
 #ifdef HB_MM8_TIMING
     if (lane == 0 && blockIdx.x < 512) for (int k = 0; k < 8; k++) g_mm8_t[(blockIdx.x * 4 + wave) * 8 + k] = tacc[k];
@@ -536,7 +589,7 @@
         }
     }
     Mm8Matrix *m = new Mm8Matrix();
-    m->n_out = n_out; m->d = d; m->nkb = nkb; m->n_rt = n_rt; m->skip01 = skip01; m->a8 = nullptr; m->crow = nullptr; m->zero = nullptr;
+    m->n_out = n_out; m->d = d; m->nkb = nkb; m->n_rt = n_rt; m->skip01 = skip01; m->prebias = !env_hook(ENV_MM8_NO_PREBIAS); m->a8 = nullptr; m->crow = nullptr; m->zero = nullptr;
     m->bp = bpar;
     {
         Big pn(9, 0); pn[8] = 1;
@@ -572,14 +625,15 @@
     const size_t lds = mm8_lds_bytes(m->n_rt, m->nkb, tpw);
     const bool check = check_mask_dev != nullptr;
     const bool ragged = !check && (m->n_out % 16) >= 1 && (m->n_out % 16) <= 8;
-#define MM8_LAUNCH_(NKB, CHK, RG, SK)                                                                                 \
+#define MM8_LAUNCH_(NKB, CHK, RG, SK) do { if (!(CHK) && m->prebias) MM8_LAUNCH__(NKB, CHK, RG, SK, !(CHK)); else MM8_LAUNCH__(NKB, CHK, RG, SK, false); } while (0)
+#define MM8_LAUNCH__(NKB, CHK, RG, SK, PB)                                                                                 \
     do {                                                                                                          \
         static std::atomic<unsigned long long> attr_done{0};                                                                               \
         if (!((attr_done.load() >> (ctx->device & 63)) & 1ull)) {                                                                                         \
-            HB_HIP(ctx, hipFuncSetAttribute(reinterpret_cast<const void *>(k_mm8<NKB, CHK, RG, SK>), hipFuncAttributeMaxDynamicSharedMemorySize, 80 * 1024)); \
+            HB_HIP(ctx, hipFuncSetAttribute(reinterpret_cast<const void *>(k_mm8<NKB, CHK, RG, SK, PB>), hipFuncAttributeMaxDynamicSharedMemorySize, 80 * 1024)); \
             attr_done.fetch_or(1ull << (ctx->device & 63));                                                                                     \
         }                                                                                                         \
-        hipLaunchKernelGGL((k_mm8<NKB, CHK, RG, SK>), dim3((unsigned)blocks), dim3(256), lds, s, m->a8, m->crow, m->zero, in, iv.stride_c, \
+        hipLaunchKernelGGL((k_mm8<NKB, CHK, RG, SK, PB>), dim3((unsigned)blocks), dim3(256), lds, s, m->a8, m->crow, m->zero, in, iv.stride_c, \
                            iv.stride_l, in_rows_dev, in_count, m->d, out, ov.stride_c, ov.stride_l, out_count,   \
                            check_mask_dev, check_rows_dev, mismatch_dev, copy_dst, cpv.stride_c, cpv.stride_l, copy_count, copy_rows,         \
                            m->n_out, m->n_rt, tpw, C, n_units, m->bp);             \
@@ -596,6 +650,7 @@
 #undef MM8_LAUNCH
 #undef MM8_LAUNCH_SK
 #undef MM8_LAUNCH_
+#undef MM8_LAUNCH__
     HB_LAUNCH_CHECK(ctx);
     return HB_OK;
 }
diff --git a/honeybadgermpc_amd/csrc/hb_mfma_fused.hip b/honeybadgermpc_amd/csrc/hb_mfma_fused.hip
--- a/honeybadgermpc_amd/csrc/hb_mfma_fused.hip
+++ b/honeybadgermpc_amd/csrc/hb_mfma_fused.hip
@@ -272,8 +272,20 @@
     for (int i = threadIdx.x; i < (8 * NKB - d) * 256; i += NT) {
         const int l = d + (i >> 8), b = (i >> 7) & 1, t = (i >> 5) & 3, h = (i >> 4) & 1, c = i & 15;
         const int kb = l >> 3, gg = (l & 7) >> 1, e = l & 1;
-        xbuf[(size_t)b * bufsz + (size_t)((((t * NKB + kb) * 2 + e) * 2 + h) * 64) + (c + 16 * gg)] = make_uint4(0, 0, 0, 0);
-    }
+        if constexpr (MSC) {
+            uint32_t *gr = reinterpret_cast<uint32_t *>(xbuf + (size_t)b * bufsz + (size_t)(((t * NKB + kb) * 4 + 2 * h) * 64) + (c + 16 * gg)) + e;
+            gr[0] = 0; gr[2] = 0; gr[256] = 0; gr[258] = 0;
+        } else
+            xbuf[(size_t)b * bufsz + (size_t)((((t * NKB + kb) * 2 + e) * 2 + h) * 64) + (c + 16 * gg)] = make_uint4(0, 0, 0, 0);
+    }
+    auto put_biased = [&](uint4 *dst, int t, int kb, int gg, int e, const uint32_t (&w)[NW]) __attribute__((always_inline)) {
+        uint32_t *gr = reinterpret_cast<uint32_t *>(dst + (size_t)((t * NKB + kb) * 4) * 64 + (n + 16 * gg)) + e;
+#pragma unroll
+        for (int j = 0; j < 4; j++) {
+            gr[256 * j] = w[2 * j] ^ 0x80808080u;
+            gr[256 * j + 2] = w[2 * j + 1] ^ 0x80808080u;
+        }
+    };
     const int n_pairs = FS_TPW * n_rt;
     const uint32_t my_terms = (uint32_t)__builtin_amdgcn_readfirstlane((int)split.terms[wave]);
 
@@ -399,9 +411,12 @@
                 for (int k = 0; k < NW; k++) w[k] = ok ? (take ? u[k] : w[k]) : 0u;
             }
             const int kb = l >> 3, gg = (l & 7) >> 1, e = l & 1;
-            uint4 *slot = dst + (size_t)(((t * NKB + kb) * 2 + e) * 2) * 64 + (n + 16 * gg);
-            slot[0] = make_uint4(w[0], w[1], w[2], w[3]);
-            slot[64] = make_uint4(w[4], w[5], w[6], w[7]);
+            if constexpr (MSC) put_biased(dst, t, kb, gg, e, w);
+            else {
+                uint4 *slot = dst + (size_t)(((t * NKB + kb) * 2 + e) * 2) * 64 + (n + 16 * gg);
+                slot[0] = make_uint4(w[0], w[1], w[2], w[3]);
+                slot[64] = make_uint4(w[4], w[5], w[6], w[7]);
+            }
 #pragma unroll
             for (int k = 0; k < NW; k++) xw[k] = xn[k];
             ok = okn;
@@ -446,10 +461,7 @@
 #pragma unroll
                         for (int k = 0; k < NW; k++) w[k] = okf[j] ? w[k] : 0u;
                     }
-                    const int gg = (l & 7) >> 1, e = l & 1;
-                    uint4 *slot = xbuf + (size_t)(((t * NKB + j) * 2 + e) * 2) * 64 + (n + 16 * gg);
-                    slot[0] = make_uint4(w[0], w[1], w[2], w[3]);
-                    slot[64] = make_uint4(w[4], w[5], w[6], w[7]);
+                    put_biased(xbuf, t, j, (l & 7) >> 1, l & 1, w);
                 }
                 __builtin_amdgcn_sched_barrier(0);
             }
@@ -534,7 +546,8 @@
                     asm volatile("" ::: "memory");
                     __builtin_amdgcn_sched_barrier(0);
                     __builtin_amdgcn_s_setprio(0);
-                    Mm8PhasePacked<NKB, 0>::run(acc, xs_addr, as_addr, biaspv);
+                    if constexpr (MSC) Mm8PhasePackedB<NKB, 0>::run(acc, xs_addr, as_addr, biaspv);
+                    else Mm8PhasePacked<NKB, 0>::run(acc, xs_addr, as_addr, biaspv);
                     __builtin_amdgcn_s_setprio(2);
                     __builtin_amdgcn_sched_barrier(0);
                     FS_T(3);
@@ -554,7 +567,8 @@
                     __builtin_amdgcn_sched_barrier(0);
                     FS_T(4);
                     __builtin_amdgcn_s_setprio(0);
-                    Mm8PhasePacked<NKB, 1>::run(acc, xs_addr, as_addr, biaspv);
+                    if constexpr (MSC) Mm8PhasePackedB<NKB, 1>::run(acc, xs_addr, as_addr, biaspv);
+                    else Mm8PhasePacked<NKB, 1>::run(acc, xs_addr, as_addr, biaspv);
                     __builtin_amdgcn_s_setprio(2);
                     __builtin_amdgcn_sched_barrier(0);
                     FS_T(5);
@@ -596,7 +610,8 @@
                 asm volatile("" ::: "memory");
                 __builtin_amdgcn_sched_barrier(0);
                 __builtin_amdgcn_s_setprio(0);
-                Mm8Phase<NKB, 0, false>::run(acc, xs_addr, as_addr, biasv);
+                if constexpr (MSC) Mm8PhaseB<NKB, 0, false>::run(acc, xs_addr, as_addr, biasv);
+                else Mm8Phase<NKB, 0, false>::run(acc, xs_addr, as_addr, biasv);
                 __builtin_amdgcn_s_setprio(2);
                 __builtin_amdgcn_sched_barrier(0);
                 FS_T(3);
@@ -617,7 +632,8 @@
                 __builtin_amdgcn_sched_barrier(0);
                 FS_T(4);
                 __builtin_amdgcn_s_setprio(0);
-                Mm8Phase<NKB, 1, false>::run(acc, xs_addr, as_addr, biasv);
+                if constexpr (MSC) Mm8PhaseB<NKB, 1, false>::run(acc, xs_addr, as_addr, biasv);
+                else Mm8Phase<NKB, 1, false>::run(acc, xs_addr, as_addr, biasv);
                 __builtin_amdgcn_s_setprio(2);
                 __builtin_amdgcn_sched_barrier(0);
                 FS_T(5);
diff --git a/honeybadgermpc_amd/csrc/hb_mm8.hpp b/honeybadgermpc_amd/csrc/hb_mm8.hpp
--- a/honeybadgermpc_amd/csrc/hb_mm8.hpp
+++ b/honeybadgermpc_amd/csrc/hb_mm8.hpp
@@ -22,6 +22,7 @@
 struct Mm8Matrix {
     int n_out, d, nkb, n_rt;
     bool skip01;
+    bool prebias;
     int4 *a8;
     uint32_t *crow;
     uint32_t *zero;
```
